# kalj/dealii-cuda

Hardware: AMD Instinct MI355X
Metric: DoFs/s on 1305x Laplace vmult (bmop), p=4 3D uniform (higher is better)
Workload: dtype f64; 1 GPU; bmop: DEGREE_FE=4, DIMENSION=3, MATRIX_FREE_UNIFORM_MESH, hyper_cube(-1,1), 54^3 cells, 10218313 DoFs, 1 z-slab(s); cells_per_dir=54, n_dofs=10218313, n_cells=157464, parallelism=slab1, dof_numbering=caller's (lexicographic), finite=True, clock_ramp_steps=2000

## Files before the change

dealii-cuda_amd/csrc/mfgpu_api.hip:

```cpp
#include <hip/hip_runtime.h>

#include <type_traits>

#include <algorithm>
#include <cmath>
#include <cstdlib>
#include <cstring>
#include <memory>
#include <string>
#include <vector>

#include "mfgpu_kernels.h"

using namespace mfgpu;

struct EventTimer {
  std::vector<Event> ev;
  size_t used = 0;
  double ms = 0.0;
  int begin(hipStream_t st) {
    if (used + 2 > ev.size()) {
      Event e0, e1;
      int rc;
      if ((rc = e0.create(hipEventDefault)) || (rc = e1.create(hipEventDefault))) return rc;
      ev.push_back(std::move(e0));
      ev.push_back(std::move(e1));
    }
    HIP_TRY(hipEventRecord(ev[used].get(), st));
    return 0;
  }
  int end(hipStream_t st) {
    HIP_TRY(hipEventRecord(ev[used + 1].get(), st));
    used += 2;
    return 0;
  }
  int drain(double *total) {
    for (size_t i = 0; i + 1 < used; i += 2) {
      float t = 0.f;
      HIP_TRY(hipEventElapsedTime(&t, ev[i].get(), ev[i + 1].get()));
      ms += t;
    }
    used = 0;
    *total = ms;
    return 0;
  }
  void reset() {
    used = 0;
    ms = 0.0;
  }
};

struct mfgpu_handle {
  Plan plan;
  int dim = 0, n = 0, nd = 0, number_type = MFGPU_F64;
  bool hn = false;
  std::vector<double> S, Dt;
  std::vector<double> sv, sg;
  DeviceArray<uint32_t> d_batch_cell_off, d_batch_dof_off, d_bdofs;
  DeviceArray<uint8_t> d_bflags;
  DeviceArray<uint16_t> d_lmap;
  DeviceArray<uint16_t> d_lmapx;
  DeviceArray<uint16_t> d_perm;
  DeviceArray<uint32_t> d_bdofsp, d_idxp;
  DeviceArray<uint32_t> d_shtab;
  bool shared_records = false;
  size_t record_bytes = 0;
  DeviceArray<uint32_t> d_hnrec;
  DeviceArray<uint32_t> d_hn_slot;
  DeviceArray<void> d_coefp;
  DeviceArray<void> d_coef;
  DeviceArray<void> d_mass, d_massp;
  DeviceArray<uint32_t> d_cmask, d_orphans;
  DeviceArray<void> d_hnw;
  DeviceArray<uint32_t> d_constrained;
  uint32_t n_constrained = 0;
  DeviceArray<void> d_tabsd;
  DeviceArray<void> d_tab2;
  bool twopass = true;
  DeviceArray<uint32_t> d_batch_nint, d_halo_off;
  std::vector<uint32_t> seg_end;
  std::vector<DeviceArray<uint32_t>> d_p2arr, d_p2tiles;
  std::vector<uint32_t> n_p2tiles;
  DeviceArray<uint32_t> d_p2rec, d_p2tab;
  bool p2_shared = false, p2_reverse = false, no_shared_records = false;
  Stream side;
  std::vector<Event> ev_seg;
  Event ev_side;
  bool side_pending = false;
  DeviceArray<void> d_halo;
  DeviceArray<unsigned long long> d_stamps;
  size_t lds = 0, device_bytes = 0;
  PlaneKernel planes = PlaneKernel::none;
  BatchKernel batches = BatchKernel::none;
  enum { kPlain, kMasked, kBatch };
  CellKernel<double> kernels_f64[3];
  CellKernel<float> kernels_f32[3];
  template <typename T>
  CellKernel<T> &kernel(int which) {
    if constexpr (std::is_same<T, double>::value) return kernels_f64[which];
    else return kernels_f32[which];
  }
  uint32_t n_cus = 0, max_workgroups = 0;
  bool prof = false;
  EventTimer t_cells;
  EventTimer t_pass2;
  uint64_t prof_vmults = 0;
};

namespace {

template <typename T>
hipError_t bind_kernel(const mfgpu_handle *h, PlaneKernel pk, BatchKernel bk, bool hn, bool sh, CellKernel<T> *k) {
  const Plan &P = h->plan;
  const auto bind = pk == PlaneKernel::planes3 ? p_bind<T> : pk == PlaneKernel::planes4 ? q_bind<T>
                    : bk == BatchKernel::batches ? apply_bind<T> : bk == BatchKernel::x ? x_bind<T>
                    : bk == BatchKernel::g ? g_bind<T> : bk == BatchKernel::g2 ? g2_bind<T> : nullptr;
  if (!bind) return hipErrorInvalidValue;
  return bind(P.dim, P.n, hn, h->twopass, sh, h->d_mass.get() != nullptr, P.max_batch_dofs, k);
}

template <typename T>
int launch_bound(mfgpu_handle *h, int which, const ApplyArgs<T> &a, uint32_t nbat, hipStream_t st) {
  const CellKernel<T> &k = h->kernel<T>(which);
  if (!k.launch[0]) {
    set_error("cell-loop kernel not bound");
    return MFGPU_EINVAL;
  }
  uint32_t grid = (uint32_t)(k.per_cu < 1 ? 1 : k.per_cu) * h->n_cus;
  if (h->max_workgroups && h->max_workgroups < grid) grid = h->max_workgroups;
  HIP_TRY(k.launch[a.add != 0](a, h->S.data(), h->Dt.data(), k.lds, nbat < grid ? nbat : grid, st));
  return 0;
}

int check_symmetrize(int n, std::vector<double> &S, std::vector<double> &Dt) {
  const int p = n - 1;
  double err = 0, mag = 0;
  for (int r = 0; r < n; ++r)
    for (int c = 0; c < n; ++c) {
      const double s1 = S[r * n + c], s2 = S[(p - r) * n + (p - c)];
      const double d1 = Dt[r * n + c], d2 = -Dt[(p - r) * n + (p - c)];
      err = std::fmax(err, std::fmax(std::fabs(s1 - s2), std::fabs(d1 - d2)));
      mag = std::fmax(mag, std::fmax(std::fabs(s1), std::fabs(d1)));
    }
  if (err > 1e-10 * mag) {
    set_error("shape tables are not symmetric about the cell midpoint (unsupported)");
    return MFGPU_EUNSUPPORTED;
  }
  for (int r = 0; r < n; ++r)
    for (int c = 0; c < n; ++c) {
      const int r2 = p - r, c2 = p - c;
      if (r * n + c < r2 * n + c2) {
        const double s = 0.5 * (S[r * n + c] + S[r2 * n + c2]);
        S[r * n + c] = S[r2 * n + c2] = s;
        const double d = 0.5 * (Dt[r * n + c] - Dt[r2 * n + c2]);
        Dt[r * n + c] = d;
        Dt[r2 * n + c2] = -d;
      } else if (r == r2 && c == c2) {
        Dt[r * n + c] = 0.0;
      }
    }
  return 0;
}

int upload_pass2(mfgpu_handle *h, const uint32_t *priority, uint32_t n_priority) {
  const Plan &P = h->plan;
  std::vector<uint8_t> prio(P.n_dofs, 0);
  for (uint32_t i = 0; i < n_priority; ++i) {
    if (priority[i] >= P.n_dofs) {
      set_error("priority dof out of range");
      return MFGPU_EINVAL;
    }
    prio[priority[i]] = 1;
  }
  const size_t ng = 1 + h->seg_end.size();
  const bool shared = P.sh_p2_use && !h->no_shared_records && n_priority == 0 && ng == 2;
  std::vector<std::vector<uint32_t>> sd(ng), so(ng, std::vector<uint32_t>(1, 0u)), si(ng);
  auto add = [&](uint32_t dof, const uint32_t *slots, uint32_t k, size_t seg) {
    const size_t g = prio[dof & 0x7fffffffu] ? 0 : 1 + seg;
    sd[g].push_back(dof);
    si[g].insert(si[g].end(), slots, slots + k);
    so[g].push_back((uint32_t)si[g].size());
  };
  for (size_t i = 0; i < P.sdofs.size(); ++i) {
    size_t seg = 0;
    if (shared && P.s_off[i + 1] > P.s_off[i]) continue;
    if (P.s_off[i + 1] > P.s_off[i]) {
      const uint32_t slot = P.s_idx[P.s_off[i + 1] - 1];
      const uint32_t batch = (uint32_t)(std::upper_bound(P.halo_off.begin(), P.halo_off.end(), slot) - P.halo_off.begin()) - 1;
      seg = (size_t)(std::upper_bound(h->seg_end.begin(), h->seg_end.end(), batch) - h->seg_end.begin());
      if (seg >= h->seg_end.size()) seg = h->seg_end.size() - 1;
    }
    add(P.sdofs[i], P.s_idx.data() + P.s_off[i], P.s_off[i + 1] - P.s_off[i], seg);
  }
  const uint32_t zero_slot = P.halo_off.empty() ? 0u : P.halo_off.back();
  for (uint32_t orph : P.orphans) add(orph, &zero_slot, 1, 0);
  std::vector<DeviceArray<uint32_t>> d_arr(ng), d_tiles(ng);
  std::vector<uint32_t> n_tiles(ng, 0u);
  const bool reverse = (size_t)P.halo_off.back() * esize(h->number_type) <= ((size_t)256 << 20);
  DeviceArray<uint32_t> d_rec, d_tab;
  if (shared) {
    int rc;
    if ((rc = d_rec.upload(P.sh_p2rec.data(), P.sh_p2rec.size()))) return rc;
    if ((rc = d_tab.upload(P.sh_p2tab.data(), P.sh_p2tab.size()))) return rc;
  }
  for (size_t g = 0; g < ng; ++g) {
    std::vector<uint32_t> arr, tiles;
    build_pass2_classes(sd[g], so[g], si[g], arr, tiles);
    n_tiles[g] = (uint32_t)(tiles.size() / 4);
    if (reverse) {
      const size_t nt = tiles.size() / 4;
      for (size_t a = 0, b = nt ? nt - 1 : 0; a < b; ++a, --b)
        for (int w = 0; w < 4; ++w) std::swap(tiles[4 * a + w], tiles[4 * b + w]);
    }
    int rc;
    if ((rc = d_arr[g].upload(arr.data(), arr.size()))) return rc;
    if ((rc = d_tiles[g].upload(tiles.data(), tiles.size()))) return rc;
  }
  h->d_p2arr = std::move(d_arr);
  h->d_p2tiles = std::move(d_tiles);
  h->n_p2tiles = std::move(n_tiles);
  h->d_p2rec = std::move(d_rec);
  h->d_p2tab = std::move(d_tab);
  h->p2_shared = shared;
  h->p2_reverse = reverse;
  return 0;
}

template <typename T>
int create_arrays(mfgpu_handle *h, const mfgpu_desc &d) {
  const Plan &P = h->plan;
  const size_t ncell = P.n_cells, nd = (size_t)P.nd;
  size_t &acct = h->device_bytes;
  auto up = [&](auto &arr, const void *src, size_t n) {
    const int rc = arr.upload(src, n);
    acct += arr.bytes();
    return rc;
  };
  int rc;
  if ((rc = up(h->d_batch_cell_off, P.batch_cell_off.data(), P.batch_cell_off.size()))) return rc;
  if ((rc = up(h->d_batch_dof_off, P.batch_dof_off.data(), P.batch_dof_off.size()))) return rc;
  if ((rc = up(h->d_bdofs, P.bdofs.data(), P.bdofs.size()))) return rc;
  if ((rc = up(h->d_bflags, P.bflags.data(), P.bflags.size()))) return rc;
  if ((rc = up(h->d_lmap, P.lmap.data(), P.lmap.size()))) return rc;
  const bool general = h->batches == BatchKernel::g || h->batches == BatchKernel::g2;
  if (h->batches == BatchKernel::x && !h->hn) {
    const int n = P.n, n2 = n * n, PP = n2, CH = 256 / PP, ndl = n2 * n;
    std::vector<uint16_t> perm(512, 0xffff);
    for (int layout = 0; layout < 2; ++layout) {
      uint16_t *lanes = perm.data() + 256 * layout;
      std::vector<int> fill(32, 0), overflow;
      for (int q = 0; q < CH * PP; ++q) {
        const int cell = q / PP, pen = q % PP, a = pen % n, b = pen / n;
        const int base = cell * ndl + (layout == 0 ? a + n2 * b : a + n * b);
        const int r = base & 31;
        if (fill[r] < 8) lanes[32 * fill[r]++ + r] = (uint16_t)q;
        else overflow.push_back(q);
      }
      for (int l = 255; l >= 0 && !overflow.empty(); --l)
        if (lanes[l] == 0xffff) {
          lanes[l] = (uint16_t)overflow.back();
          overflow.pop_back();
        }
    }
    if ((rc = up(h->d_perm, perm.data(), perm.size()))) return rc;
  }
  if (h->batches == BatchKernel::x || general) {
    const size_t n = (size_t)P.n, np = (n + 1) & ~(size_t)1, runs = P.lmap.size() / n;
    std::vector<uint16_t> lx(runs * np, 0);
    for (size_t r = 0; r < runs; ++r)
      for (size_t i = 0; i < n; ++i) lx[r * np + i] = P.lmap[r * n + i];
    if ((rc = up(h->d_lmapx, lx.data(), lx.size()))) return rc;
  }
  if (h->batches == BatchKernel::g2) {
    std::vector<T> sd(2 * (size_t)P.n * P.n);
    for (int i = 0; i < P.n * P.n; ++i) {
      sd[i] = (T)h->S[i];
      sd[P.n * P.n + i] = (T)h->Dt[i];
    }
    if ((rc = up(h->d_tabsd, sd.data(), sd.size() * sizeof(T)))) return rc;
  }
  if (h->planes != PlaneKernel::none) {
    if ((rc = build_plane_records(h->plan, d.constraint_mask))) return rc;
    if (!P.pr_hn.empty()) {
      if ((rc = up(h->d_hnrec, P.pr_hn.data(), P.pr_hn.size()))) return rc;
      if ((rc = up(h->d_hn_slot, P.pr_hn_slot.data(), P.pr_hn_slot.size()))) return rc;
    }
    h->shared_records = P.sh_use && !(d.flags & MFGPU_NO_SHARED_RECORDS) &&
                        kernel_exists(h->planes, P.n, d.number_type, false, true, d.mass_coefficient != nullptr);
    const std::vector<uint32_t> &rd = h->shared_records ? P.sh_dofs : P.pr_dofs;
    const std::vector<uint32_t> &rx = h->shared_records ? P.sh_idx : P.pr_idx;
    if ((rc = up(h->d_bdofsp, rd.data(), rd.size()))) return rc;
    if ((rc = up(h->d_idxp, rx.data(), rx.size()))) return rc;
    if (h->shared_records && (rc = up(h->d_shtab, P.sh_batch.data(), P.sh_batch.size()))) return rc;
    h->record_bytes = h->d_bdofsp.bytes() + h->d_idxp.bytes() + h->d_shtab.bytes();
  }
  if ((rc = up(h->d_orphans, P.orphans.data(), P.orphans.size()))) return rc;
  if (h->twopass) {
    if ((rc = up(h->d_batch_nint, P.batch_nint.data(), P.batch_nint.size()))) return rc;
    if ((rc = up(h->d_halo_off, P.halo_off.data(), P.halo_off.size()))) return rc;
    if (h->planes != PlaneKernel::none && (uint64_t)P.halo_off.back() >= (1ull << 29)) {
      set_error("halo buffer too large for 32-bit byte offsets");
      return MFGPU_EUNSUPPORTED;
    }
    const size_t hb = ((size_t)P.halo_off.back() + 1) * sizeof(T);
    if ((rc = h->d_halo.alloc(hb, true))) return rc;
    acct += hb;
  }
  if (h->hn) {
    std::vector<uint32_t> cm(ncell);
    for (size_t i = 0; i < ncell; ++i) cm[i] = d.constraint_mask[P.cell_order[i]];
    if ((rc = up(h->d_cmask, cm.data(), ncell))) return rc;
    std::vector<T> w((size_t)h->n * h->n);
    for (size_t i = 0; i < w.size(); ++i) w[i] = (T)d.constraint_weights[i];
    if ((rc = up(h->d_hnw, w.data(), w.size() * sizeof(T)))) return rc;
  }
  DeviceArray<T> metric;
  if ((rc = fold_coefficient<T>(metric, d.coefficient, d.quadrature_points, d.JxW, d.inv_jac, P.cell_order.data(), P.dim,
                                (uint32_t)ncell, (uint32_t)nd, general)))
    return rc;
  h->d_coef = std::move(metric);
  acct += h->d_coef.bytes();
  if (d.mass_coefficient) {
    DeviceArray<T> mass;
    if ((rc = fold_mass<T>(mass, d.mass_coefficient, d.JxW, P.cell_order.data(), (uint32_t)ncell, (uint32_t)nd))) return rc;
    h->d_mass = std::move(mass);
    acct += h->d_mass.bytes();
  }
  if (h->planes != PlaneKernel::none) {
    const int n = P.n, NT = p_cells_per_wave(n) * n;
    const size_t nbat = P.n_plane_batches, total = nbat * (size_t)(n * n) * NT;
    const size_t ncell_p = P.batch_cell_off[nbat];
    std::vector<uint32_t> cb(ncell_p), cp(ncell_p);
    for (size_t b = 0; b < nbat; ++b)
      for (uint32_t c = P.batch_cell_off[b]; c < P.batch_cell_off[b + 1]; ++c) {
        cb[c] = (uint32_t)b;
        cp[c] = c - P.batch_cell_off[b];
      }
    DeviceArray<uint32_t> t_cb, t_cp;
    if ((rc = t_cb.upload(cb.data(), ncell_p))) return rc;
    if ((rc = t_cp.upload(cp.data(), ncell_p))) return rc;
    if ((rc = h->d_coefp.alloc(total * sizeof(T), true))) return rc;
    acct += h->d_coefp.bytes();
    HIP_TRY(relayout_coef_launch<T>(h->d_coefp.as<T>(), h->d_coef.as<const T>(), t_cb.get(), t_cp.get(), ncell_p * nd, n,
                                    nullptr));
    if (d.mass_coefficient) {
      if ((rc = h->d_massp.alloc(total * sizeof(T), true))) return rc;
      acct += h->d_massp.bytes();
      HIP_TRY(relayout_coef_launch<T>(h->d_massp.as<T>(), h->d_mass.as<const T>(), t_cb.get(), t_cp.get(), ncell_p * nd,
                                      n, nullptr));
    }
    HIP_TRY(hipDeviceSynchronize());
  }
  int dev = 0;
  hipDeviceProp_t prop;
  HIP_TRY(hipGetDevice(&dev));
  HIP_TRY(hipGetDeviceProperties(&prop, dev));
  h->n_cus = (uint32_t)prop.multiProcessorCount;
  h->max_workgroups = d.max_workgroups;
  if (h->planes != PlaneKernel::none) {
    CellKernel<T> &plain = h->kernel<T>(mfgpu_handle::kPlain), &masked = h->kernel<T>(mfgpu_handle::kMasked);
    HIP_TRY(bind_kernel<T>(h, h->planes, BatchKernel::none, false, h->shared_records, &plain));
    h->lds = plain.lds;
    if (P.n_plain_plane_batches < P.n_plane_batches) {
      HIP_TRY(bind_kernel<T>(h, h->planes, BatchKernel::none, true, false, &masked));
      h->lds = std::max(h->lds, masked.lds);
    }
  }
  if (h->batches == BatchKernel::none) return 0;
  CellKernel<T> &batch = h->kernel<T>(mfgpu_handle::kBatch);
  const hipError_t bind_batch_family = bind_kernel<T>(h, PlaneKernel::none, h->batches, h->hn, false, &batch);
  h->lds = batch.lds;
  if (h->lds > 160 * 1024) {
    set_error("batch needs more than 160 KiB of LDS; lower max_dofs_per_batch");
    return MFGPU_EINVAL;
  }
  HIP_TRY(bind_batch_family);
  return 0;
}

void choose_segments(mfgpu_handle *h, uint32_t request) {
  const Plan &P = h->plan;
  const uint32_t nb = (uint32_t)(P.batch_cell_off.size() - 1);
  h->seg_end.assign(1, nb);
  if (!h->twopass || nb < 2 || request == 1) return;
  const uint32_t npl = P.n_plane_batches, nplain = P.n_plain_plane_batches;
  std::vector<uint32_t> cuts;
  if (npl > 0 && npl < nb) cuts.push_back(npl);
  if (nplain > 0 && nplain < npl) cuts.push_back(nplain);
  if (request > 1) {
    for (uint32_t i = 1; i < request; ++i) cuts.push_back((uint32_t)((uint64_t)nb * i / request));
  }
  if (request == 0 && !P.pr_hn.empty() && nplain == 0 && P.n == 5) cuts.push_back(nb / 2);
  std::sort(cuts.begin(), cuts.end());
  h->seg_end.clear();
  for (uint32_t c : cuts)
    if (c > 0 && c < nb && (h->seg_end.empty() || h->seg_end.back() != c)) h->seg_end.push_back(c);
  h->seg_end.push_back(nb);
}

template <typename T>
int create_typed(mfgpu_handle *h, const mfgpu_desc &d) {
  int rc = create_arrays<T>(h, d);
  if (rc) return rc;
  choose_segments(h, d.cell_loop_segments);
  if (!h->twopass) return 0;
  if (h->seg_end.size() > 1) {
    int prio_least = 0, prio_greatest = 0;
    HIP_TRY(hipDeviceGetStreamPriorityRange(&prio_least, &prio_greatest));
    if ((rc = h->side.create(hipStreamNonBlocking, prio_least))) return rc;
    if ((rc = h->ev_side.create(hipEventDisableTiming))) return rc;
    h->ev_seg.resize(h->seg_end.size() - 1);
    for (Event &e : h->ev_seg)
      if ((rc = e.create(hipEventDisableTiming))) return rc;
  }
  return upload_pass2(h, nullptr, 0);
}

template <typename T>
int launch_pass2_group(mfgpu_handle *h, size_t group, void *dst, const void *src, hipStream_t st, int add) {
  if (h->p2_shared && group == 1)
    HIP_TRY(reduce_owner_batches_launch<T>((T *)dst, (const T *)src, h->d_halo.as<const T>(), h->d_p2rec.get(),
                                           h->d_p2tab.get(), (uint32_t)(h->plan.batch_cell_off.size() - 1),
                                           (uint32_t)p_hs(h->plan.n) * 64u, h->p2_reverse ? 1 : 0, add, st));
  HIP_TRY(reduce_classes_launch<T>((T *)dst, (const T *)src, h->d_halo.as<const T>(), h->d_p2arr[group].get(),
                                   h->d_p2tiles[group].get(), h->n_p2tiles[group], add, st));
  return 0;
}

template <typename T>
int vmult_pass2(mfgpu_handle *h, int phase, void *dst, const void *src, hipStream_t st, int add) {
  if (!h->twopass) return 0;
  if (phase == 0) return launch_pass2_group<T>(h, 0, dst, src, st, add);
  int rc = launch_pass2_group<T>(h, h->seg_end.size(), dst, src, st, add);
  if (!rc && h->side_pending) {
    HIP_TRY(hipStreamWaitEvent(st, h->ev_side.get(), 0));
    h->side_pending = false;
  }
  return rc;
}

template <typename T>
int launch_cells(mfgpu_handle *h, ApplyArgs<T> a, uint32_t b0, uint32_t b1, hipStream_t st) {
  const Plan &P = h->plan;
  const uint32_t npl = P.n_plane_batches, nplain = P.n_plain_plane_batches;
  if (b0 < nplain) {
    a.batch0 = b0;
    a.batch_end = b1 < nplain ? b1 : nplain;
    if (const int rc = launch_bound<T>(h, mfgpu_handle::kPlain, a, a.batch_end - a.batch0, st)) return rc;
    b0 = a.batch_end;
  }
  if (b0 < npl && b0 < b1) {
    a.batch0 = b0;
    a.batch_end = b1 < npl ? b1 : npl;
    if (const int rc = launch_bound<T>(h, mfgpu_handle::kMasked, a, a.batch_end - a.batch0, st)) return rc;
    b0 = a.batch_end;
  }
  if (b0 >= b1) return 0;
  a.batch0 = b0;
  a.batch_end = b1;
  return launch_bound<T>(h, mfgpu_handle::kBatch, a, b1 - b0, st);
}

template <typename T>
ApplyArgs<T> make_args(mfgpu_handle *h, void *dst, const void *src, int add) {
  const Plan &P = h->plan;
  ApplyArgs<T> a;
  a.batch_cell_off = h->d_batch_cell_off.get();
  a.batch_dof_off = h->d_batch_dof_off.get();
  a.bdofs = h->d_bdofs.get();
  a.bflags = h->d_bflags.get();
  a.lmap = h->d_lmap.get();
  a.lmapx = h->d_lmapx.get();
  a.perm = h->d_perm.get();
  a.bdofsp = h->d_bdofsp.get();
  a.idxp = h->d_idxp.get();
  a.shtab = h->shared_records ? h->d_shtab.get() : nullptr;
  a.hnrec = h->d_hnrec.get();
  a.hn_slot = h->d_hn_slot.get();
  a.coefp = h->d_coefp.as<const T>();
  a.coef = h->d_coef.as<const T>();
  a.mass = h->d_mass.as<const T>();
  a.massp = h->d_massp.as<const T>();
  a.cmask = h->d_cmask.get();
  a.hn_weights = h->d_hnw.as<const T>();
  a.tabS = h->d_tabsd.as<const T>();
  a.tabDt = a.tabS ? a.tabS + (size_t)P.n * P.n : nullptr;
  a.batch_nint = h->d_batch_nint.get();
  a.halo_off = h->d_halo_off.get();
  a.halo = h->d_halo.as<T>();
  a.dst = (T *)dst;
  a.src = (const T *)src;
  a.nb_max = P.max_batch_dofs;
  a.add = add;
  a.stamps = h->d_stamps.get();
  a.dbg = 0;
  return a;
}

template <typename T>
int vmult_main(mfgpu_handle *h, void *dst, const void *src, hipStream_t st, int add) {
  const Plan &P = h->plan;
  ApplyArgs<T> a = make_args<T>(h, dst, src, add);
  int rc;
  if (h->prof && (rc = h->t_cells.begin(st))) return rc;
  if (h->twopass) {
    const size_t nseg = h->seg_end.size();
    if (h->side_pending) {
      HIP_TRY(hipStreamWaitEvent(st, h->ev_side.get(), 0));
      h->side_pending = false;
    }
    for (size_t s = 0; s < nseg; ++s) {
      if ((rc = launch_cells<T>(h, a, s ? h->seg_end[s - 1] : 0u, h->seg_end[s], st))) return rc;
      if (s + 1 < nseg) {
        HIP_TRY(hipEventRecord(h->ev_seg[s].get(), st));
        HIP_TRY(hipStreamWaitEvent(h->side.get(), h->ev_seg[s].get(), 0));
        if ((rc = launch_pass2_group<T>(h, 1 + s, dst, src, h->side.get(), add))) return rc;
      }
    }
    if (nseg > 1) {
      HIP_TRY(hipEventRecord(h->ev_side.get(), h->side.get()));
      h->side_pending = true;
    }
  } else {
    for (size_t c = 0; c + 1 < P.color_batch_off.size(); ++c) {
      if (P.color_batch_off[c + 1] == P.color_batch_off[c]) continue;
      if ((rc = launch_cells<T>(h, a, P.color_batch_off[c], P.color_batch_off[c + 1], st))) return rc;
    }
  }
  if (h->prof && (rc = h->t_cells.end(st))) return rc;
  if (!h->twopass)
    HIP_TRY(orphan_launch<T>((T *)dst, (const T *)src, h->d_orphans.get(), (uint32_t)P.orphans.size(), add, st));
  if (h->prof) h->prof_vmults++;
  return 0;
}

template <typename T>
int vmult_typed(mfgpu_handle *h, void *dst, const void *src, hipStream_t st, int add) {
  int rc = vmult_main<T>(h, dst, src, st, add);
  if (rc) return rc;
  const bool timed = h->prof && h->twopass;
  if (timed && (rc = h->t_pass2.begin(st))) return rc;
  rc = vmult_pass2<T>(h, 0, dst, src, st, add);
  if (!rc) rc = vmult_pass2<T>(h, 1, dst, src, st, add);
  if (!rc && timed) rc = h->t_pass2.end(st);
  return rc;
}

}

namespace {
template <typename T>
int inverse_diagonal_typed(mfgpu_handle *h, void *diag, hipStream_t st) {
  const Plan &P = h->plan;
  const bool general = h->batches == BatchKernel::g || h->batches == BatchKernel::g2;
  if (!h->d_tab2.get()) {
    const int nn = h->n * h->n;
    std::vector<T> t2(2 * (size_t)nn);
    for (int i = 0; i < nn; ++i) {
      t2[i] = (T)(general ? h->sv[i] : h->sv[i] * h->sv[i]);
      t2[nn + i] = (T)(general ? h->sg[i] : h->sg[i] * h->sg[i]);
    }
    if (const int rc = h->d_tab2.upload(t2.data(), t2.size() * sizeof(T))) return rc;
    h->device_bytes += h->d_tab2.bytes();
  }
  HIP_TRY(fill_launch<T>((T *)diag, P.n_dofs, T(0), st));
  const uint32_t nb = (uint32_t)(P.batch_cell_off.size() - 1), *cell_off = h->d_batch_cell_off.get();
  const uint32_t *dof_off = h->d_batch_dof_off.get(), *bdofs = h->d_bdofs.get(), *cmask = h->d_cmask.get();
  const uint16_t *lmap = h->d_lmap.get();
  const T *coef = h->d_coef.as<const T>(), *hnw = h->d_hnw.as<const T>(), *tab2 = h->d_tab2.as<const T>();
  if (h->batches == BatchKernel::g2)
    HIP_TRY(diag_general2_launch<T>(P.n, (T *)diag, nb, cell_off, dof_off, bdofs, lmap, coef, cmask, hnw, tab2, st));
  else if (h->batches == BatchKernel::g)
    HIP_TRY(diag_general_launch<T>(P.n, (T *)diag, nb, cell_off, dof_off, bdofs, lmap, coef, cmask, hnw, tab2, st));
  else
    HIP_TRY(diag_launch<T>(P.dim, P.n, (T *)diag, nb, cell_off, dof_off, bdofs, lmap, coef, cmask, hnw, tab2, st));
  if (h->d_mass.get())
    HIP_TRY(diag_mass_launch<T>(P.dim, P.n, (T *)diag, nb, cell_off, dof_off, bdofs, lmap, h->d_mass.as<const T>(), cmask,
                                hnw, tab2, !general, st));
  HIP_TRY(set_values_launch<T>((T *)diag, h->d_constrained.get(), h->n_constrained, T(1), st));
  HIP_TRY(vec_map_launch<T>(4, (T *)diag, nullptr, T(0), T(0), P.n_dofs, st));
  return 0;
}
}


namespace {
int vec_map(int op, void *v, const void *w, double s, double a, size_t n, int nt, void *stream) {
  if ((!v && n) || (!w && n && op <= 3)) {
    set_error("null vector");
    return MFGPU_EINVAL;
  }
  if (nt == MFGPU_F32)
    HIP_TRY(vec_map_launch<float>(op, (float *)v, (const float *)w, (float)s, (float)a, n, (hipStream_t)stream));
  else if (nt == MFGPU_F64)
    HIP_TRY(vec_map_launch<double>(op, (double *)v, (const double *)w, s, a, n, (hipStream_t)stream));
  else
    return MFGPU_EINVAL;
  return 0;
}
int vec_reduce(int op, void *v, const void *x, const void *w, double a, size_t n, int nt, void *stream, double *out) {
  if (!out || (n && (!v || (op != 2 && !w) || (op == 1 && !x)))) {
    set_error("null argument");
    return MFGPU_EINVAL;
  }
  if (nt == MFGPU_F32)
    HIP_TRY(vec_reduce_launch<float>(op, (float *)v, (const float *)x, (const float *)w, (float)a, n, (hipStream_t)stream, out));
  else if (nt == MFGPU_F64)
    HIP_TRY(vec_reduce_launch<double>(op, (double *)v, (const double *)x, (const double *)w, a, n, (hipStream_t)stream, out));
  else
    return MFGPU_EINVAL;
  return 0;
}
}


namespace mfgpu {
int handle_number_type(const mfgpu_handle *h) { return h->number_type; }
int handle_set_priority_dofs(mfgpu_handle *h, const uint32_t *ids, uint32_t n) {
  return h->twopass ? upload_pass2(h, ids, n) : 0;
}
int handle_n_batches(const mfgpu_handle *h) { return (int)h->plan.batch_cell_off.size() - 1; }
bool handle_ranged_ok(const mfgpu_handle *h) { return h->twopass && h->seg_end.size() == 1; }
int handle_batches_touching(const mfgpu_handle *h, const uint32_t *ids, uint32_t n, std::vector<uint8_t> &flags) {
  const Plan &P = h->plan;
  std::vector<uint8_t> mark(P.n_dofs, 0);
  for (uint32_t i = 0; i < n; ++i) {
    if (ids[i] >= P.n_dofs) {
      set_error("interface dof out of range");
      return MFGPU_EINVAL;
    }
    mark[ids[i]] = 1;
  }
  const size_t nb = P.batch_cell_off.size() - 1;
  flags.assign(nb, 0);
  for (size_t b = 0; b < nb; ++b)
    for (uint32_t t = P.batch_dof_off[b]; t < P.batch_dof_off[b + 1]; ++t)
      if (mark[P.bdofs[t] & 0x7fffffffu]) {
        flags[b] = 1;
        break;
      }
  return 0;
}
int handle_cells_range(mfgpu_handle *h, uint32_t b0, uint32_t b1, void *dst, const void *src, void *stream, int add) {
  if (b0 >= b1) return 0;
  hipStream_t st = (hipStream_t)stream;
  if (h->number_type == MFGPU_F64) return launch_cells<double>(h, make_args<double>(h, dst, src, add), b0, b1, st);
  return launch_cells<float>(h, make_args<float>(h, dst, src, add), b0, b1, st);
}
int handle_cells_two_ranges(mfgpu_handle *h, uint32_t b0, uint32_t b1, uint32_t c0, uint32_t c1, void *dst,
                            const void *src, void *stream, int add) {
  const uint32_t nplain = h->plan.n_plain_plane_batches, npl = h->plan.n_plane_batches;
  const bool plain = c1 <= nplain, masked = b0 >= nplain && c1 <= npl;
  if (b0 >= b1 || c0 >= c1 || b1 > c0 || !(plain || masked)) {
    const int rc = handle_cells_range(h, b0, b1, dst, src, stream, add);
    return rc ? rc : handle_cells_range(h, c0, c1, dst, src, stream, add);
  }
  hipStream_t st = (hipStream_t)stream;
  auto run = [&](auto a) -> int {
    a.batch0 = b0;
    a.batch_end = c1;
    a.hole0 = b1;
    a.hole_len = c0 - b1;
    using T = typename std::remove_const<typename std::remove_pointer<decltype(a.src)>::type>::type;
    return launch_bound<T>(h, plain ? mfgpu_handle::kPlain : mfgpu_handle::kMasked, a, (b1 - b0) + (c1 - c0), st);
  };
  return h->number_type == MFGPU_F64 ? run(make_args<double>(h, dst, src, add)) : run(make_args<float>(h, dst, src, add));
}
int handle_pass2_group(mfgpu_handle *h, int group, void *dst, const void *src, void *stream, int add) {
  if (!h->twopass) return 0;
  hipStream_t st = (hipStream_t)stream;
  return h->number_type == MFGPU_F64 ? launch_pass2_group<double>(h, (size_t)group, dst, src, st, add)
                                     : launch_pass2_group<float>(h, (size_t)group, dst, src, st, add);
}
int handle_vmult_phase(mfgpu_handle *h, int phase, void *dst, const void *src, void *stream, int add) {
  hipStream_t st = (hipStream_t)stream;
  if (h->number_type == MFGPU_F64)
    return phase == 0 ? vmult_main<double>(h, dst, src, st, add) : vmult_pass2<double>(h, phase - 1, dst, src, st, add);
  return phase == 0 ? vmult_main<float>(h, dst, src, st, add) : vmult_pass2<float>(h, phase - 1, dst, src, st, add);
}
}

extern "C" {

int mfgpu_create(const mfgpu_desc *desc, mfgpu_handle **out) {
  if (!desc || !out) {
    set_error("null argument");
    return MFGPU_EINVAL;
  }
  const mfgpu_desc &d = *desc;
  if (!valid_number_type(d.number_type)) {
    set_error("number_type must be MFGPU_F64 or MFGPU_F32");
    return MFGPU_EINVAL;
  }
  const bool general = !(d.flags & MFGPU_UNIFORM_J0);
  if (general && (d.flags & MFGPU_COLORED_SCATTER)) {
    set_error("the general-Jacobian path (no MFGPU_UNIFORM_J0) is implemented in two-pass scatter mode only");
    return MFGPU_EUNSUPPORTED;
  }
  if (!d.JxW || !d.inv_jac || !d.shape_values || !d.shape_gradients ||
      (!d.coefficient && !d.quadrature_points)) {
    set_error("JxW, inv_jac, shape tables and coefficient (or quadrature_points) are required");
    return MFGPU_EINVAL;
  }
  const bool hn = (d.flags & MFGPU_HANGING_NODES) != 0;
  if (hn && (!d.constraint_mask || !d.constraint_weights)) {
    set_error("MFGPU_HANGING_NODES needs constraint_mask and constraint_weights");
    return MFGPU_EINVAL;
  }
  std::unique_ptr<mfgpu_handle, decltype(&mfgpu_destroy)> h(new mfgpu_handle(), mfgpu_destroy);
  int rc = choose_kernel_and_plan(d, h->planes, h->batches, h->plan);
  if (rc) return rc;
  h->dim = d.dim;
  h->n = d.degree + 1;
  h->nd = h->plan.nd;
  h->number_type = d.number_type;
  h->hn = hn;
  h->twopass = !(d.flags & MFGPU_COLORED_SCATTER);
  h->no_shared_records = (d.flags & MFGPU_NO_SHARED_RECORDS) != 0;
  const int nn = h->n * h->n;
  std::vector<double> sv(nn), sg(nn);
  for (int i = 0; i < nn; ++i) {
    sv[i] = d.number_type == MFGPU_F64 ? ((const double *)d.shape_values)[i] : ((const float *)d.shape_values)[i];
    sg[i] = d.number_type == MFGPU_F64 ? ((const double *)d.shape_gradients)[i] : ((const float *)d.shape_gradients)[i];
  }
  h->sv = sv;
  h->sg = sg;
  rc = derive_tables(h->n, sv.data(), sg.data(), h->S, h->Dt);
  if (!rc) rc = check_symmetrize(h->n, h->S, h->Dt);
  if (!rc) rc = d.number_type == MFGPU_F64 ? create_typed<double>(h.get(), d) : create_typed<float>(h.get(), d);
  if (!rc && d.n_constrained) {
    h->n_constrained = d.n_constrained;
    rc = h->d_constrained.upload(d.constrained_dofs, d.n_constrained);
    h->device_bytes += h->d_constrained.bytes();
  }
  if (rc) return rc;
  *out = h.release();
  return 0;
}

void mfgpu_destroy(mfgpu_handle *h) {
  if (!h) return;
  if (h->side.get()) hipStreamSynchronize(h->side.get());
  delete h;
}

int mfgpu_vmult(mfgpu_handle *h, void *dst, const void *src, void *stream) {
  if (!h || !dst || !src) {
    set_error("null argument");
    return MFGPU_EINVAL;
  }
  if (dst == src) {
    set_error("vmult: dst and src must not alias");
    return MFGPU_EINVAL;
  }
  return h->number_type == MFGPU_F64 ? vmult_typed<double>(h, dst, src, (hipStream_t)stream, 0)
                                     : vmult_typed<float>(h, dst, src, (hipStream_t)stream, 0);
}

int mfgpu_vmult_add(mfgpu_handle *h, void *dst, const void *src, void *stream) {
  if (!h || !dst || !src) {
    set_error("null argument");
    return MFGPU_EINVAL;
  }
  if (dst == src) {
    set_error("vmult_add: dst and src must not alias");
    return MFGPU_EINVAL;
  }
  return h->number_type == MFGPU_F64 ? vmult_typed<double>(h, dst, src, (hipStream_t)stream, 1)
                                     : vmult_typed<float>(h, dst, src, (hipStream_t)stream, 1);
}

uint32_t mfgpu_n_dofs(const mfgpu_handle *h) { return h ? h->plan.n_dofs : 0; }

size_t mfgpu_memory_consumption(const mfgpu_handle *h) { return h ? h->device_bytes : 0; }

int mfgpu_plan_stats(const mfgpu_handle *h, uint64_t s[8]) {
  if (!h || !s) return MFGPU_EINVAL;
  const Plan &P = h->plan;
  s[0] = P.batch_cell_off.size() - 1;
  s[1] = P.color_batch_off.size() - 1;
  s[2] = P.bdofs.size();
  s[3] = P.max_batch_dofs;
  s[4] = P.max_batch_cells;
  s[5] = P.orphans.size();
  s[6] = P.n_first;
  s[7] = P.n_add;
  if (h->twopass) {
    const uint32_t nb = (uint32_t)s[0], npl = P.n_plane_batches, nplain = P.n_plain_plane_batches;
    const uint32_t edge[4] = {0u, nplain, npl, nb};
    s[1] = 0;
    for (size_t g = 0; g < h->seg_end.size(); ++g) {
      const uint32_t s0 = g ? h->seg_end[g - 1] : 0u, s1 = h->seg_end[g];
      for (int f = 0; f < 3; ++f)
        if (std::max(s0, edge[f]) < std::min(s1, edge[f + 1])) ++s[1];
    }
    s[6] = P.sdofs.size();
    s[7] = P.halo_off.back();
  }
  return 0;
}

int mfgpu_record_stats(const mfgpu_handle *h, uint64_t s[4]) {
  if (!h || !s) return MFGPU_EINVAL;
  const Plan &P = h->plan;
  const size_t n = (size_t)P.n, nb = (size_t)p_kgu((int)n) * 64, nx = ((n * n + 1) / 2) * (p_cells_per_wave((int)n) * n);
  const bool planes = h->planes != PlaneKernel::none;
  s[0] = (h->shared_records ? 1 : 0) | (h->p2_shared ? 2 : 0);
  s[1] = planes ? P.sh_dofs.size() / nb : 0;
  s[2] = planes ? P.sh_idx.size() / nx : 0;
  s[3] = h->record_bytes;
  return 0;
}

const char *mfgpu_kernel_name(const mfgpu_handle *h) {
  if (!h) return "";
  const bool x = h->batches == BatchKernel::x;
  switch (h->planes) {
    case PlaneKernel::planes3: return x ? "apply_planes3+apply_batches_x" : "apply_planes3";
    case PlaneKernel::planes4: return x ? "apply_planes4+apply_batches_x" : "apply_planes4";
    default: break;
  }
  switch (h->batches) {
    case BatchKernel::x: return "apply_batches_x";
    case BatchKernel::g: return "apply_batches_g";
    case BatchKernel::g2: return "apply_batches_g2";
    default: return "apply_batches";
  }
}

int mfgpu_profile_enable(mfgpu_handle *h, int on) {
  if (!h) return MFGPU_EINVAL;
  h->prof = on != 0;
  h->t_cells.reset();
  h->t_pass2.reset();
  h->prof_vmults = 0;
  return 0;
}

int mfgpu_profile_read_pass2(mfgpu_handle *h, double *ms) {
  if (!h || !ms) return MFGPU_EINVAL;
  HIP_TRY(hipDeviceSynchronize());
  return h->t_pass2.drain(ms);
}

int mfgpu_profile_read(mfgpu_handle *h, double *ms, uint64_t *nv) {
  if (!h || !ms || !nv) return MFGPU_EINVAL;
  HIP_TRY(hipDeviceSynchronize());
  if (const int rc = h->t_cells.drain(ms)) return rc;
  *nv = h->prof_vmults;
  return 0;
}

#ifdef MFGPU_STAMPS
int mfgpu_debug_stamps(mfgpu_handle *h, unsigned long long *out, size_t n_batches) {
  if (!h) return MFGPU_EINVAL;
  const size_t nbt = h->plan.batch_cell_off.size() - 1;
  if (!h->d_stamps.get()) return h->d_stamps.alloc(2 * nbt * 16, true);
  if (out && n_batches == nbt) {
    HIP_TRY(hipDeviceSynchronize());
    HIP_TRY(hipMemcpy(out, h->d_stamps.get(), 2 * nbt * 16 * sizeof(unsigned long long), hipMemcpyDeviceToHost));
  }
  return 0;
}
#endif


int mfgpu_compute_inverse_diagonal(mfgpu_handle *h, void *inv_diag, void *stream) {
  if (!h || !inv_diag) {
    set_error("null argument");
    return MFGPU_EINVAL;
  }
  return h->number_type == MFGPU_F64 ? inverse_diagonal_typed<double>(h, inv_diag, (hipStream_t)stream)
                                     : inverse_diagonal_typed<float>(h, inv_diag, (hipStream_t)stream);
}

int mfgpu_set_constrained_values(mfgpu_handle *h, void *vec, double value, void *stream) {
  if (!h || !vec) {
    set_error("null argument");
    return MFGPU_EINVAL;
  }
  if (h->number_type == MFGPU_F64)
    HIP_TRY(set_values_launch<double>((double *)vec, h->d_constrained.get(), h->n_constrained, value, (hipStream_t)stream));
  else
    HIP_TRY(set_values_launch<float>((float *)vec, h->d_constrained.get(), h->n_constrained, (float)value,
                                     (hipStream_t)stream));
  return 0;
}

int mfgpu_vec_sadd(void *v, double s, double a, const void *w, size_t n, int nt, void *stream) {
  return vec_map(0, v, w, s, a, n, nt, stream);
}
int mfgpu_vec_equ(void *v, double a, const void *w, size_t n, int nt, void *stream) {
  return vec_map(1, v, w, 0.0, a, n, nt, stream);
}
int mfgpu_vec_scale(void *v, const void *w, size_t n, int nt, void *stream) {
  return vec_map(2, v, w, 0.0, 0.0, n, nt, stream);
}
int mfgpu_vec_divide(void *v, const void *w, size_t n, int nt, void *stream) {
  return vec_map(3, v, w, 0.0, 0.0, n, nt, stream);
}
int mfgpu_vec_invert(void *v, size_t n, int nt, void *stream) { return vec_map(4, v, nullptr, 0.0, 0.0, n, nt, stream); }
int mfgpu_vec_mul(void *v, double a, size_t n, int nt, void *stream) {
  return vec_map(5, v, nullptr, 0.0, a, n, nt, stream);
}
int mfgpu_vec_dot(const void *v, const void *w, size_t n, int nt, void *stream, double *result) {
  return vec_reduce(0, const_cast<void *>(v), nullptr, w, 0.0, n, nt, stream, result);
}
int mfgpu_vec_l2_norm(const void *v, size_t n, int nt, void *stream, double *result) {
  int rc = vec_reduce(0, const_cast<void *>(v), nullptr, v, 0.0, n, nt, stream, result);
  if (!rc) *result = std::sqrt(*result);
  return rc;
}
int mfgpu_vec_add_and_dot(void *v, double a, const void *x, const void *w, size_t n, int nt, void *stream,
                          double *result) {
  return vec_reduce(1, v, x, w, a, n, nt, stream, result);
}
int mfgpu_vec_all_zero(const void *v, size_t n, int nt, void *stream, int *result) {
  if (!result) return MFGPU_EINVAL;
  double cnt = 0.0;
  int rc = vec_reduce(2, const_cast<void *>(v), nullptr, nullptr, 0.0, n, nt, stream, &cnt);
  if (!rc) *result = cnt == 0.0;
  return rc;
}

int mfgpu_vec_alloc(void **dev, size_t n, int nt) {
  if (!dev) return MFGPU_EINVAL;
  *dev = nullptr;
  if (n == 0) return 0;
  HIP_TRY(hipMalloc(dev, n * esize(nt)));
  HIP_TRY(hipMemset(*dev, 0, n * esize(nt)));
  return 0;
}
int mfgpu_vec_free(void *dev) {
  if (dev) HIP_TRY(hipFree(dev));
  return 0;
}
int mfgpu_vec_fill(void *dev, size_t n, int nt, double value, void *stream) {
  if (!dev && n) return MFGPU_EINVAL;
  if (nt == MFGPU_F32)
    HIP_TRY(fill_launch<float>((float *)dev, n, (float)value, (hipStream_t)stream));
  else
    HIP_TRY(fill_launch<double>((double *)dev, n, value, (hipStream_t)stream));
  return 0;
}
int mfgpu_vec_from_host(void *dev, const void *host, size_t n, int nt) {
  if (n) HIP_TRY(hipMemcpy(dev, host, n * esize(nt), hipMemcpyHostToDevice));
  return 0;
}
int mfgpu_vec_to_host(void *host, const void *dev, size_t n, int nt) {
  if (n) HIP_TRY(hipMemcpy(host, dev, n * esize(nt), hipMemcpyDeviceToHost));
  return 0;
}
int mfgpu_device_synchronize(void) {
  HIP_TRY(hipDeviceSynchronize());
  return 0;
}
int mfgpu_device_memory_info(size_t *free_bytes, size_t *total_bytes) {
  if (!free_bytes || !total_bytes) return MFGPU_EINVAL;
  HIP_TRY(hipMemGetInfo(free_bytes, total_bytes));
  return 0;
}

}
```

dealii-cuda_amd/csrc/mfgpu_internal.h:

```cpp
#ifndef MFGPU_INTERNAL_H
#define MFGPU_INTERNAL_H

#include <cstdint>
#include <string>
#include <vector>

#include "../../include/mfgpu.h"

namespace mfgpu {

void set_error(const std::string &msg);

inline int ipow(int a, int e) {
  int r = 1;
  for (int i = 0; i < e; ++i) r *= a;
  return r;
}

constexpr int p_cells_per_wave(int n) { return 64 / n; }
constexpr int p_ji(int n) { return n == 3 ? 2 : n == 4 ? 5 : n == 5 ? 9 : n == 6 ? 14 : 23; }
constexpr int p_hs(int n) { return n == 3 ? 3 : n == 4 ? 6 : n == 5 ? 9 : n == 6 ? 14 : 18; }
constexpr int p_kgu(int n) { return p_ji(n) + p_hs(n); }
constexpr int p_cell_stride(int n) {
  int s = n * n * n;
  while ((s & 31) != (n & 31)) ++s;
  return s;
}

constexpr int q_plane_stride(int n) { return n >= 6 ? 65 : n == 5 ? 33 : n == 4 ? 17 : 33; }
constexpr int q_cell_stride(int n) { return n * q_plane_stride(n); }
constexpr int p_priv_max(int n) { return n >= 5 ? 384 : n == 4 ? 256 : 192; }
constexpr int kHnOpRounds = 2;
constexpr int p_hn_rows(int n) { return p_priv_max(n) / 64 + 3 * kHnOpRounds * 3 + 2; }

template <typename T>
constexpr size_t q_region_doubles(int n) {
  const size_t t = ((size_t)(p_cells_per_wave(n) + 1) * q_cell_stride(n) * sizeof(T) + 7) / 8;
  const size_t u = (size_t)p_kgu(n) * 64 + p_priv_max(n);
  return t > u ? t : u;
}
template <typename T>
constexpr size_t q_lds_bytes(int n, bool hn) {
  return (q_region_doubles<T>(n) + (hn ? (size_t)n * n : 0)) * 8;
}

constexpr uint8_t kFlagConstrained = 1;
constexpr uint8_t kFlagAdd = 2;

struct Plan {
  int dim = 0, degree = 0, n = 0, nd = 0;
  uint32_t n_dofs = 0, n_cells = 0;
  std::vector<uint32_t> cell_order;
  std::vector<uint32_t> batch_cell_off;
  std::vector<uint32_t> batch_dof_off;
  std::vector<uint32_t> color_batch_off;
  std::vector<uint32_t> bdofs;
  std::vector<uint8_t> bflags;
  std::vector<uint16_t> lmap;
  std::vector<uint32_t> orphans;
  std::vector<uint32_t> batch_nint;
  std::vector<uint32_t> halo_off;
  std::vector<uint32_t> sdofs;
  std::vector<uint32_t> s_off;
  std::vector<uint32_t> s_idx;
  std::vector<uint32_t> chunks;
  std::vector<uint32_t> gstarts;
  uint32_t max_batch_dofs = 0, max_batch_cells = 0;
  uint32_t n_plane_batches = 0;
  uint32_t n_plain_plane_batches = 0;
  std::vector<uint32_t> pr_dofs, pr_idx, pr_hn, pr_hn_slot;
  std::vector<uint32_t> sh_dofs, sh_idx, sh_batch;
  bool sh_use = false;
  std::vector<uint32_t> sh_p2rec, sh_p2tab;
  bool sh_p2_use = false;
  uint64_t n_first = 0, n_add = 0;
};

struct PlanLimits {
  uint32_t max_cells = 0, max_dofs = 0;
  uint32_t interior_max = 0, shared_max = 0, halo_stride = 0;
  bool segregate_masked = false;
  bool masked_planes = false;
  uint32_t private_max = 0;
};

int build_plan(const mfgpu_desc &d, Plan &plan, uint32_t max_chunks = 3, const PlanLimits *limits = nullptr);

struct HnLine {
  uint16_t node[8];
};
void hn_cell_lines(unsigned mask, int n, std::vector<HnLine> (&lines)[3], std::vector<uint16_t> &nodes);

enum class PlaneKernel : uint8_t { none, planes3, planes4 };
enum class BatchKernel : uint8_t { none, batches, x, g, g2 };
int choose_kernel_and_plan(const mfgpu_desc &d, PlaneKernel &pk, BatchKernel &bk, Plan &plan);

constexpr bool planes4_wide(int n) { return n >= 6; }
constexpr bool kernel_exists(PlaneKernel k, int n, int number_type, bool hn, bool sh, bool mass) {
  switch (k) {
    case PlaneKernel::planes3: return n >= 3 && n <= 5 && !(sh && hn);
    case PlaneKernel::planes4:
      return planes4_wide(n) ? n <= 7 && !hn && !sh && !mass
                             : n >= 3 && !sh && !(mass && n == 5 && number_type == MFGPU_F64);
    default: return false;
  }
}
constexpr bool kernel_exists(BatchKernel k, int n, int , bool , bool sh, bool ) {
  return k != BatchKernel::none && n >= 2 && n <= 7 && !sh;
}
int build_plane_records(Plan &plan, const uint32_t *constraint_mask);
constexpr int kShBatchWords = 4;
constexpr double kShareMaxFraction = 0.5;
void share_plane_records(Plan &plan);
constexpr int kP2Header = 16, kP2MaxK = 12, kP2SlotBits = 12;
void share_pass2_records(Plan &plan);

int derive_tables(int n, const double *shape_values, const double *shape_gradients,
                  std::vector<double> &S, std::vector<double> &Dt);

int handle_number_type(const mfgpu_handle *h);
int handle_set_priority_dofs(mfgpu_handle *h, const uint32_t *ids, uint32_t n);
int handle_vmult_phase(mfgpu_handle *h, int phase, void *dst, const void *src, void *stream, int add);
int handle_n_batches(const mfgpu_handle *h);
bool handle_ranged_ok(const mfgpu_handle *h);
int handle_batches_touching(const mfgpu_handle *h, const uint32_t *ids, uint32_t n, std::vector<uint8_t> &flags);
int handle_cells_range(mfgpu_handle *h, uint32_t b0, uint32_t b1, void *dst, const void *src, void *stream, int add);
int handle_cells_two_ranges(mfgpu_handle *h, uint32_t b0, uint32_t b1, uint32_t c0, uint32_t c1, void *dst,
                            const void *src, void *stream, int add);
int handle_pass2_group(mfgpu_handle *h, int group, void *dst, const void *src, void *stream, int add);

}

struct mfgpu_plan {
  mfgpu::Plan plan;
};

#endif
```

dealii-cuda_amd/csrc/mfgpu_kernels.h:

```cpp
#ifndef MFGPU_KERNELS_H
#define MFGPU_KERNELS_H

#include <hip/hip_runtime.h>

#include <type_traits>

#include "mfgpu_device.h"
#include "mfgpu_internal.h"

namespace mfgpu {

template <typename T>
struct ApplyArgs {
  const uint32_t *batch_cell_off;
  const uint32_t *batch_dof_off;
  const uint32_t *bdofs;
  const uint8_t *bflags;
  const uint16_t *lmap;
  const uint16_t *lmapx;
  const uint16_t *perm;
  const uint32_t *bdofsp;
  const uint32_t *idxp;
  const T *coefp;
  const uint32_t *hnrec;
  const uint32_t *hn_slot;
  const T *coef;
  const uint32_t *cmask;
  const T *hn_weights;
  const T *tabS, *tabDt;
  const uint32_t *batch_nint;
  const uint32_t *halo_off;
  T *halo;
  T *dst;
  const T *src;
  uint32_t batch0;
  uint32_t batch_end;
  uint32_t hole0 = 0xffffffffu, hole_len = 0;
  uint32_t nb_max;
  int add;
  unsigned long long *stamps;
  int dbg;
  const uint32_t *shtab = nullptr;
  const T *mass = nullptr;
  const T *massp = nullptr;
};

template <typename T, int n>
struct Tables {
  T S[((n + 1) / 2) * n];
  T Dt[((n + 1) / 2) * n];
};

template <typename T, int n>
inline Tables<T, n> make_tables(const double *S, const double *Dt) {
  Tables<T, n> tab;
  for (int i = 0; i < ((n + 1) / 2) * n; ++i) {
    tab.S[i] = (T)S[i];
    tab.Dt[i] = (T)Dt[i];
  }
  return tab;
}

template <typename T>
struct CellKernel {
  size_t lds = 0;
  int per_cu = 0;
  hipError_t (*launch[2])(const ApplyArgs<T> &a, const double *S, const double *Dt, size_t lds, uint32_t grid,
                          hipStream_t st) = {nullptr, nullptr};
};

template <typename T, int Block, auto K, auto MakeTab>
hipError_t launch_cell_kernel(const ApplyArgs<T> &a, const double *S, const double *Dt, size_t lds, uint32_t grid,
                              hipStream_t st) {
  if constexpr (std::is_null_pointer_v<decltype(MakeTab)>)
    hipLaunchKernelGGL(K, dim3(grid), dim3(Block), lds, st, a);
  else
    hipLaunchKernelGGL(K, dim3(grid), dim3(Block), lds, st, a, MakeTab(S, Dt));
  return hipGetLastError();
}

template <typename T, int Block, auto K0, auto K1, auto MakeTab>
hipError_t bind_cell_kernel(size_t lds, CellKernel<T> *k) {
  k->lds = lds;
  for (const void *f : {(const void *)K1, (const void *)K0})
    if (const hipError_t e = hipFuncSetAttribute(f, hipFuncAttributeMaxDynamicSharedMemorySize, (int)lds)) return e;
  k->launch[0] = launch_cell_kernel<T, Block, K0, MakeTab>;
  k->launch[1] = launch_cell_kernel<T, Block, K1, MakeTab>;
  return hipOccupancyMaxActiveBlocksPerMultiprocessor(&k->per_cu, (const void *)K0, Block, lds);
}

template <typename F>
hipError_t dispatch_flags(F &&f) { return f(); }
template <typename F, typename... B>
hipError_t dispatch_flags(F &&f, bool flag, B... rest) {
  return dispatch_flags(
      [&](auto... c) { return flag ? f(std::true_type{}, c...) : f(std::false_type{}, c...); }, rest...);
}
template <typename F, typename... B>
hipError_t dispatch_instantiation(int n, F &&f, B... flags) {
  auto at = [&](auto N) { return dispatch_flags([&](auto... c) { return f(N, c...); }, flags...); };
  switch (n) {
    case 2: return at(std::integral_constant<int, 2>{});
    case 3: return at(std::integral_constant<int, 3>{});
    case 4: return at(std::integral_constant<int, 4>{});
    case 5: return at(std::integral_constant<int, 5>{});
    case 6: return at(std::integral_constant<int, 6>{});
    case 7: return at(std::integral_constant<int, 7>{});
    default: return hipErrorInvalidValue;
  }
}
template <typename T>
constexpr int number_type_of = sizeof(T) == 8 ? MFGPU_F64 : MFGPU_F32;

#define MFGPU_CELL_LOOP_FAMILY(F)                                                                              \
  template <typename T>                                                                                        \
  hipError_t F##_bind(int dim, int n, bool hn, bool twopass, bool sh, bool mass, uint32_t nb_max, CellKernel<T> *k);
MFGPU_CELL_LOOP_FAMILY(apply)
MFGPU_CELL_LOOP_FAMILY(x)
MFGPU_CELL_LOOP_FAMILY(g)
MFGPU_CELL_LOOP_FAMILY(g2)
MFGPU_CELL_LOOP_FAMILY(p)
MFGPU_CELL_LOOP_FAMILY(q)
#undef MFGPU_CELL_LOOP_FAMILY

void build_pass2_classes(const std::vector<uint32_t> &sdofs, const std::vector<uint32_t> &s_off,
                         const std::vector<uint32_t> &s_idx, std::vector<uint32_t> &arr, std::vector<uint32_t> &tiles);
template <typename T>
hipError_t reduce_classes_launch(T *dst, const T *src, const T *halo, const uint32_t *arr, const uint32_t *tiles,
                                 uint32_t n_tiles, int add, hipStream_t st);
template <typename T>
hipError_t reduce_owner_batches_launch(T *dst, const T *src, const T *halo, const uint32_t *rec, const uint32_t *tab,
                                       uint32_t n_batches, uint32_t hstride, int reverse, int add, hipStream_t st);
template <typename T>
hipError_t relayout_coef_launch(T *out, const T *in, const uint32_t *cell_batch, const uint32_t *cell_pos,
                                size_t total, int n, hipStream_t st);
template <typename T>
hipError_t fold_general_launch(T *M, const T *coef, const T *jxw, const T *jinv, const uint32_t *order,
                               uint32_t n_cells, uint32_t nd, hipStream_t st);
template <typename T>
hipError_t fold_general2_launch(T *M, const T *coef, const T *jxw, const T *jinv, const uint32_t *order,
                                uint32_t n_cells, uint32_t nd, hipStream_t st);
template <typename T>
hipError_t orphan_launch(T *dst, const T *src, const uint32_t *orph, uint32_t n, int add, hipStream_t st);
template <typename T>
hipError_t coefficient_launch(T *coef, const T *qpts, size_t nq, int dim, hipStream_t st);
template <typename T>
hipError_t fold_launch(T *c, const T *coef, const T *jxw, const T *j0, const uint32_t *order,
                       uint32_t n_cells, uint32_t nd, hipStream_t st);
template <typename T>
hipError_t fill_launch(T *v, size_t n, T a, hipStream_t st);
template <typename T>
int fold_mass(DeviceArray<T> &out, const void *mass_coefficient, const void *JxW, const uint32_t *cell_order,
              uint32_t n_cells, uint32_t nd);
template <typename T>
int fold_coefficient(DeviceArray<T> &out, const void *coefficient, const void *quadrature_points, const void *JxW,
                     const void *inv_jac, const uint32_t *cell_order, int dim, uint32_t n_cells, uint32_t nd,
                     bool general);

template <typename T>
hipError_t diag_launch(int dim, int n, T *diag, uint32_t n_batches, const uint32_t *batch_cell_off,
                       const uint32_t *batch_dof_off, const uint32_t *bdofs, const uint16_t *lmap, const T *coef,
                       const uint32_t *cmask, const T *hn_weights, const T *tab2, hipStream_t st);
template <typename T>
hipError_t diag_general_launch(int n, T *diag, uint32_t n_batches, const uint32_t *batch_cell_off,
                               const uint32_t *batch_dof_off, const uint32_t *bdofs, const uint16_t *lmap,
                               const T *metric, const uint32_t *cmask, const T *hn_weights, const T *tab,
                               hipStream_t st);
template <typename T>
hipError_t diag_general2_launch(int n, T *diag, uint32_t n_batches, const uint32_t *batch_cell_off,
                                const uint32_t *batch_dof_off, const uint32_t *bdofs, const uint16_t *lmap,
                                const T *metric, const uint32_t *cmask, const T *hn_weights, const T *tab,
                                hipStream_t st);
template <typename T>
hipError_t diag_mass_launch(int dim, int n, T *diag, uint32_t n_batches, const uint32_t *batch_cell_off,
                            const uint32_t *batch_dof_off, const uint32_t *bdofs, const uint16_t *lmap, const T *mass,
                            const uint32_t *cmask, const T *hn_weights, const T *tab, bool squared, hipStream_t st);
template <typename T>
hipError_t set_values_launch(T *v, const uint32_t *idx, uint32_t n, T value, hipStream_t st);
template <typename T>
hipError_t vec_map_launch(int op, T *v, const T *w, T s, T a, size_t n, hipStream_t st);
template <typename T>
hipError_t vec_reduce_launch(int op, T *v, const T *x, const T *w, T a, size_t n, hipStream_t st, double *out);

}
#endif
```

dealii-cuda_amd/csrc/mfgpu_kernels_p.hip:

```cpp
#include <hip/hip_runtime.h>

#include "mfgpu_cell.h"
#include "mfgpu_kernels.h"
#include "mfgpu_planes.h"

namespace mfgpu {

#define MFGPU_PIN_VMEM() __builtin_amdgcn_sched_barrier(0x380)

template <int n, typename T, bool ADD, bool HN, bool SH = false, bool MASS = false>
__global__ void __launch_bounds__(64) __attribute__((amdgpu_waves_per_eu(1, 1)))
apply_planes3(const ApplyArgs<T> A, const TablesEO<T, n> tab) {
  constexpr int n2 = n * n;
  constexpr int CW = p_cells_per_wave(n);
  constexpr int NT = CW * n;
  constexpr int KGU = p_kgu(n);
  constexpr int JI = p_ji(n);
  constexpr int HS = KGU - JI;
  constexpr int SA = p_cell_stride(n);
  constexpr int NIW = (n2 + 1) / 2;
  extern __shared__ __attribute__((aligned(16))) unsigned char smem_raw[];
  constexpr int PRIV = HN ? p_priv_max(n) : 0;
  double *ua = reinterpret_cast<double *>(smem_raw);
  T *Aw = reinterpret_cast<T *>(ua + KGU * 64 + PRIV + (HN ? n2 : 0));
  T *Bw = Aw + (CW + 1) * SA;
  double *Wl = ua + KGU * 64 + PRIV;

  const int lane = threadIdx.x;
  if (HN) {
    if (lane < n2) Wl[lane] = (double)A.hn_weights[lane];
  }
  const int lc = lane / n, k = lane - lc * n;
  const bool lane_on = lane < NT;
  const int tk = lane_on ? lane : NT - 1;

  uint32_t b, bstride, bend;
  {
    const uint32_t nbt = A.batch_end - A.batch0 - A.hole_len, G = gridDim.x;
    if (G >= 8 && nbt >= G) {
      const uint32_t xcd = blockIdx.x & 7u, slot = blockIdx.x >> 3;
      const uint32_t q = G >> 3, rem = G & 7u;
      const uint32_t wlo = xcd * q + (xcd < rem ? xcd : rem);
      const uint32_t w = q + (xcd < rem ? 1u : 0u);
      b = A.batch0 + (uint32_t)((uint64_t)nbt * wlo / G) + slot;
      bend = A.batch0 + (uint32_t)((uint64_t)nbt * (wlo + w) / G);
      bstride = w;
    } else {
      b = A.batch0 + blockIdx.x;
      bend = A.batch_end - A.hole_len;
      bstride = G;
    }
  }
  if (b >= bend) return;
  const uint32_t hole0 = A.hole0, hole_len = A.hole_len;
  auto next_of = [&](uint32_t x) {
    const uint32_t l = (x >= hole0 ? x - hole_len : x) + bstride;
    return l < bend ? (l >= hole0 ? l + hole_len : l) : x;
  };
  if (b >= hole0) b += hole_len;
  static_assert(kernel_exists(PlaneKernel::planes3, n, number_type_of<T>, HN, SH, MASS), "no such instantiation");
  struct Meta {
    uint32_t base, drec, irec;
  };
  auto meta_request = [&](uint32_t bb) -> uint32_t {
    return A.shtab[(size_t)bb * kShBatchWords + (lane & (kShBatchWords - 1))];
  };
  auto meta_of = [&](uint32_t v) -> Meta {
    return Meta{(uint32_t)__builtin_amdgcn_readlane((int)v, 0), (uint32_t)__builtin_amdgcn_readlane((int)v, 1),
                (uint32_t)__builtin_amdgcn_readlane((int)v, 2)};
  };

  auto load_dofs = [&](uint32_t rec, uint32_t (&g)[KGU]) {
    const uint32_t *p = A.bdofsp + (size_t)rec * (KGU * 64) + lane;
#pragma unroll
    for (int j = 0; j < KGU; ++j) g[j] = SH ? p[j * 64] : nt_load(p + j * 64);
  };
  auto src_at = [&](uint32_t base, uint32_t g) -> T {
    const T *const sp = SH ? A.src + base : A.src;
    return *reinterpret_cast<const T *>(reinterpret_cast<const char *>(sp) + (uint32_t)(g * (uint32_t)sizeof(T)));
  };
  auto dst_at = [&](uint32_t base, uint32_t g) -> T * {
    T *const dp = SH ? A.dst + base : A.dst;
    return reinterpret_cast<T *>(reinterpret_cast<char *>(dp) + (uint32_t)(g * (uint32_t)sizeof(T)));
  };
  auto load_ix = [&](uint32_t rec, uint32_t (&ix)[NIW]) {
    const uint32_t *p = A.idxp + (size_t)rec * (NIW * NT) + tk;
#pragma unroll
    for (int w = 0; w < NIW; ++w) ix[w] = SH ? p[w * NT] : nt_load(p + w * NT);
  };
  auto stage_src = [&](const uint32_t (&g)[KGU], const T (&sv)[KGU]) {
#pragma unroll
    for (int j = 0; j < KGU; ++j) {
      double v = (double)sv[j];
      if (j >= JI) {
        const unsigned long long keep = (unsigned long long)(long long)~((int)g[j] >> 31);
        v = __longlong_as_double((long long)((unsigned long long)__double_as_longlong(v) & keep));
      }
      ua[lane + j * 64] = v;
    }
  };
  auto ixb = [&](const uint32_t (&ix)[NIW], int i) -> uint32_t {
    return (i & 1) ? (ix[i >> 1] >> 16) : (ix[i >> 1] & 0xffffu);
  };
  auto scatter_slot = [&](int j, uint32_t bb, uint32_t base, uint32_t g, T r, T oldv) {
    if (j < JI) {
      *dst_at(base, g) = ADD ? oldv + r : r;
    } else {
      T *const hp = A.halo + (size_t)bb * (HS * 64) + lane;
      hp[(j - JI) * 64] = r;
    }
  };

  uint32_t b1 = next_of(b), b2 = next_of(b1);
  uint32_t Gp[KGU], Gc[KGU], Gn[KGU], Gnn[KGU];
  uint32_t IXc[NIW], IXn[NIW];
  constexpr int CR = PRIV / 64, HROWS = HN ? p_hn_rows(n) : 1;
  uint32_t Hc[HROWS], Hn[HROWS];
  auto load_hn = [&](uint32_t bb, uint32_t (&H)[HROWS]) {
    const uint32_t slot = A.hn_slot[bb];
    if (slot != 0xffffffffu) {
      const uint32_t *p = A.hnrec + (size_t)slot * (HROWS * 64) + lane;
#pragma unroll
      for (int w = 0; w < HROWS; ++w) H[w] = nt_load(p + w * 64);
    } else {
#pragma unroll
      for (int w = 0; w < HROWS; ++w) H[w] = 0u;
    }
  };
  T Cc[n2];
  T Mm[MASS ? n2 : 1];
  T SVn[KGU], R[KGU], old[KGU];
  Meta Mp{0u, 0u, 0u}, Mc = Mp, M1 = Mp, M2 = Mp;
  uint32_t Mv = 0u;
  if (SH) {
    Mc = meta_of(meta_request(b));
    M1 = meta_of(meta_request(b1));
    M2 = meta_of(meta_request(b2));
    Mp = Mc;
  }
  load_dofs(SH ? Mc.drec : b, Gc);
  load_dofs(SH ? M1.drec : b1, Gn);
  load_ix(SH ? Mc.irec : b, IXc);
  if (HN) load_hn(b, Hc);
  constexpr uint32_t kDummyIx = 8u * (uint32_t)(KGU * 64 - 1) * 0x10001u;
#pragma unroll
  for (int w = 0; w < NIW; ++w) IXc[w] = lane_on ? IXc[w] : kDummyIx;
  {
    const T *p = A.coefp + (size_t)b * (n2 * NT) + tk;
#pragma unroll
    for (int r = 0; r < n2; ++r) Cc[r] = nt_load(p + r * NT);
  }
  if (MASS) {
    const T *p = A.massp + (size_t)b * (n2 * NT) + tk;
#pragma unroll
    for (int r = 0; r < n2; ++r) Mm[r] = nt_load(p + r * NT);
  }
#pragma unroll
  for (int j = 0; j < KGU; ++j) {
    SVn[j] = src_at(Mc.base, Gc[j]);
    Gp[j] = Gc[j];
    R[j] = T(0);
    old[j] = T(0);
  }
  stage_src(Gc, SVn);
  WaveSync::sync();

  const int pxy = lc * SA + n2 * k;
  const int pyz = lc * SA + k;
  uint32_t bp = b;

  while (true) {
    const bool has_next = b1 != b;
    constexpr int kH2 = HN ? HROWS - 2 : 0, kH1 = HN ? HROWS - 1 : 0;
    const uint32_t hn_ncopy = HN ? (uint32_t)__builtin_amdgcn_readfirstlane(Hc[kH2] & 0xffffu) : 0u;
    auto hn_count = [&](int dir) -> uint32_t {
      const uint32_t w = dir == 0 ? Hc[kH2] >> 16 : dir == 1 ? Hc[kH1] & 0xffffu : Hc[kH1] >> 16;
      return (uint32_t)__builtin_amdgcn_readfirstlane(w);
    };
    auto hn_pass = [&](int dir, bool transposed, const double (&Wr)[n2]) {
      const uint32_t count = hn_count(dir);
#pragma unroll
      for (int r = 0; r < kHnOpRounds; ++r) {
        if ((uint32_t)(r * 64) >= count) break;
        const bool on = (uint32_t)(r * 64 + lane) < count;
        const uint32_t *ww = &Hc[CR + (dir * kHnOpRounds + r) * 3];
        double v[n], o[n];
        uint32_t pos[n];
#pragma unroll
        for (int t = 0; t < n; ++t) {
          pos[t] = on ? (ww[t >> 1] >> (16 * (t & 1))) & 0xffffu : (uint32_t)(KGU * 64 + PRIV - 1);
          v[t] = ua[pos[t]];
        }
#pragma unroll
        for (int i = 0; i < n; ++i) {
          double acc = 0.0;
#pragma unroll
          for (int k2 = 0; k2 < n; ++k2) acc = fma(transposed ? Wr[k2 * n + i] : Wr[i * n + k2], v[k2], acc);
          o[i] = acc;
        }
        if (on) {
#pragma unroll
          for (int i = 0; i < n; ++i) ua[pos[i]] = o[i];
        }
      }
    };
    if (HN && hn_ncopy) {
      double Wr[n2];
#pragma unroll
      for (int i = 0; i < n2; ++i) Wr[i] = Wl[i];
      double cv[CR > 0 ? CR : 1];
#pragma unroll
      for (int r = 0; r < CR; ++r) cv[r] = (uint32_t)(r * 64 + lane) < hn_ncopy ? ua[Hc[r] & 0xffffu] : 0.0;
#pragma unroll
      for (int r = 0; r < CR; ++r)
        if ((uint32_t)(r * 64 + lane) < hn_ncopy) ua[Hc[r] >> 16] = cv[r];
      WaveSync::sync();
      hn_pass(0, false, Wr);
      WaveSync::sync();
      hn_pass(1, false, Wr);
      WaveSync::sync();
      hn_pass(2, false, Wr);
      WaveSync::sync();
    }
    STAMP(0);
    RSTAMP(8);
    WGSTAMP(10);
    load_dofs(SH ? M2.drec : b2, Gnn);
    load_ix(SH ? M1.irec : b1, IXn);
    if (SH) Mv = meta_request(next_of(b2));
    if (HN) load_hn(b1, Hn);
    if (ADD) {
#pragma unroll
      for (int j = 0; j < JI; ++j) old[j] = *dst_at(Mp.base, Gp[j]);
    }
    STAMP(1);
    auto hookA = [&](int) {};
    auto hookB = [&](int s) {
      MFGPU_PIN_VMEM();
#pragma unroll
      for (int j = (KGU * s) / (5 * n); j < (KGU * (s + 1)) / (5 * n); ++j)
        scatter_slot(j, bp, Mp.base, Gp[j], R[j], old[j]);
#pragma unroll
      for (int j = (KGU * s) / (5 * n); j < (KGU * (s + 1)) / (5 * n); ++j)
        SVn[j] = src_at(M1.base, Gn[j]);
      MFGPU_PIN_VMEM();
    };
    const T *const cnext = A.coefp + (size_t)b1 * (n2 * NT) + tk;
    const T *const mnext = MASS ? A.massp + (size_t)b1 * (n2 * NT) + tk : nullptr;
    auto hookC = [&](int s) {
      MFGPU_PIN_VMEM();
#pragma unroll
      for (int r = (n2 * s) / (2 * n); r < (n2 * (s + 1)) / (2 * n); ++r)
        Cc[r] = nt_load(cnext + r * NT);
      if (MASS) {
#pragma unroll
        for (int r = (n2 * s) / (2 * n); r < (n2 * (s + 1)) / (2 * n); ++r)
          Mm[r] = nt_load(mnext + r * NT);
      }
      MFGPU_PIN_VMEM();
    };

    {
      T u[n2];
#pragma unroll
      for (int x = 0; x < n; ++x)
#pragma unroll
        for (int y = 0; y < n; ++y)
          u[x + n * y] = (T) * reinterpret_cast<const double *>(reinterpret_cast<const char *>(ua) + ixb(IXc, x + n * y));
#pragma unroll
      for (int x = 0; x < n; ++x) {
        T in[n], out[n];
        get_line<n, 1>(u, x, in);
        eo_apply<n, 0>(tab, in, out);
        set_line<n, 1>(u, x, out);
        hookA(x);
      }
#pragma unroll
      for (int y = 0; y < n; ++y) {
        T in[n], a[n], bb[n];
        get_line<n, 0>(u, y, in);
        eo_apply<n, 0>(tab, in, a);
        eo_apply<n, 2>(tab, a, bb);
#pragma unroll
        for (int x = 0; x < n; ++x) {
          Aw[pxy + x + n * y] = a[x];
          Bw[pxy + x + n * y] = bb[x];
        }
        hookA(n + y);
      }
    }
    WaveSync::sync();
    STAMP(2);
#pragma unroll
    for (int j = 0; j < KGU + PRIV / 64; ++j) ua[lane + j * 64] = 0.0;

    {
      T nx[n];
#pragma unroll
      for (int z = 0; z < n; ++z) nx[z] = Bw[pyz + n2 * z];
#pragma unroll
      for (int y = 0; y < n; ++y) {
        T in[n], g[n], o[n];
#pragma unroll
        for (int z = 0; z < n; ++z) in[z] = nx[z];
#pragma unroll
        for (int z = 0; z < n; ++z) nx[z] = y + 1 < n ? Bw[pyz + n * (y + 1) + n2 * z] : Aw[pyz + n2 * z];
        eo_apply<n, 0>(tab, in, g);
#pragma unroll
        for (int z = 0; z < n; ++z) g[z] *= Cc[y + n * z];
        eo_apply<n, 1>(tab, g, o);
#pragma unroll
        for (int z = 0; z < n; ++z) Bw[pyz + n * y + n2 * z] = o[z];
        hookB(y);
      }
      T v[n2], r[n2];
#pragma unroll
      for (int y = 0; y < n; ++y) {
        T in[n], o[n];
#pragma unroll
        for (int z = 0; z < n; ++z) in[z] = nx[z];
        if (y + 1 < n) {
#pragma unroll
          for (int z = 0; z < n; ++z) nx[z] = Aw[pyz + n * (y + 1) + n2 * z];
        }
        eo_apply<n, 0>(tab, in, o);
        set_line<n, 1>(v, y, o);
        hookB(n + y);
      }
#pragma unroll
      for (int y = 0; y < n; ++y) {
        T in[n], g[n], o[n];
        get_line<n, 1>(v, y, in);
        eo_apply<n, 2>(tab, in, g);
#pragma unroll
        for (int z = 0; z < n; ++z) g[z] *= Cc[y + n * z];
        eo_apply<n, 3>(tab, g, o);
        set_line<n, 1>(r, y, o);
        hookB(2 * n + y);
      }
#pragma unroll
      for (int z = 0; z < n; ++z) {
        T in[n], g[n], o[n];
        get_line<n, 0>(v, z, in);
        eo_apply<n, 2>(tab, in, g);
#pragma unroll
        for (int y = 0; y < n; ++y) g[y] *= Cc[y + n * z];
        eo_apply<n, 3>(tab, g, o);
#pragma unroll
        for (int y = 0; y < n; ++y) r[y + n * z] += MASS ? fma(Mm[y + n * z], in[y], o[y]) : o[y];
        hookB(3 * n + z);
      }
#pragma unroll
      for (int y = 0; y < n; ++y) {
        T in[n], o[n];
        get_line<n, 1>(r, y, in);
        eo_apply<n, 1>(tab, in, o);
#pragma unroll
        for (int z = 0; z < n; ++z) Aw[pyz + n * y + n2 * z] = o[z];
        hookB(4 * n + y);
      }
    }
    WaveSync::sync();
    STAMP(3);

    {
      T o[n2];
      T nr[n], nt[n];
#pragma unroll
      for (int x = 0; x < n; ++x) {
        nr[x] = Aw[pxy + x];
        nt[x] = Bw[pxy + x];
      }
#pragma unroll
      for (int y = 0; y < n; ++y) {
        T rp[n], tp[n], w[n], ol[n];
#pragma unroll
        for (int x = 0; x < n; ++x) {
          rp[x] = nr[x];
          tp[x] = nt[x];
        }
        if (y + 1 < n) {
#pragma unroll
          for (int x = 0; x < n; ++x) {
            nr[x] = Aw[pxy + x + n * (y + 1)];
            nt[x] = Bw[pxy + x + n * (y + 1)];
          }
        }
        eo_apply<n, 3>(tab, tp, w);
#pragma unroll
        for (int x = 0; x < n; ++x) w[x] += rp[x];
        eo_apply<n, 1>(tab, w, ol);
        set_line<n, 0>(o, y, ol);
        hookC(y);
      }
#pragma unroll
      for (int x = 0; x < n; ++x) {
        T in[n], out[n];
        get_line<n, 1>(o, x, in);
        eo_apply<n, 1>(tab, in, out);
#pragma unroll
        for (int y = 0; y < n; ++y)
          lds_add(reinterpret_cast<double *>(reinterpret_cast<char *>(ua) + ixb(IXc, x + n * y)), (double)out[y]);
        hookC(n + x);
      }
    }
    WaveSync::sync();
    STAMP(4);

    if (HN && hn_ncopy) {
      double Wr[n2];
#pragma unroll
      for (int i = 0; i < n2; ++i) Wr[i] = Wl[i];
      hn_pass(2, true, Wr);
      WaveSync::sync();
      hn_pass(1, true, Wr);
      WaveSync::sync();
      hn_pass(0, true, Wr);
      WaveSync::sync();
      double cv[CR > 0 ? CR : 1];
#pragma unroll
      for (int r = 0; r < CR; ++r) cv[r] = (uint32_t)(r * 64 + lane) < hn_ncopy ? ua[Hc[r] >> 16] : 0.0;
#pragma unroll
      for (int r = 0; r < CR; ++r)
        if ((uint32_t)(r * 64 + lane) < hn_ncopy) lds_add(ua + (Hc[r] & 0xffffu), cv[r]);
      WaveSync::sync();
    }
#pragma unroll
    for (int j = 0; j < KGU; ++j) R[j] = (T)ua[lane + j * 64];
    WaveSync::sync();
    STAMP(5);
    stage_src(Gn, SVn);
    STAMP(6);
    bp = b;
    if (SH) Mp = Mc;
#pragma unroll
    for (int j = 0; j < KGU; ++j) Gp[j] = Gc[j];
    STAMP(7);
    RSTAMP(9);
    if (!has_next) break;
    WaveSync::sync();
    b = b1;
    b1 = b2;
    b2 = next_of(b2);
    if (SH) {
      Mc = M1;
      M1 = M2;
      M2 = meta_of(Mv);
    }
#pragma unroll
    for (int j = 0; j < KGU; ++j) {
      Gc[j] = Gn[j];
      Gn[j] = Gnn[j];
    }
#pragma unroll
    for (int w = 0; w < NIW; ++w) IXc[w] = lane_on ? IXn[w] : kDummyIx;
    if (HN) {
#pragma unroll
      for (int w = 0; w < HROWS; ++w) Hc[w] = Hn[w];
    }
  }
  if (ADD) {
#pragma unroll
    for (int j = 0; j < JI; ++j) old[j] = *dst_at(Mp.base, Gp[j]);
  }
#pragma unroll
  for (int j = 0; j < KGU; ++j) scatter_slot(j, bp, Mp.base, Gp[j], R[j], old[j]);
}

template <int n, typename T>
static size_t p_lds_bytes(bool hn) {
  return ((size_t)p_kgu(n) * 64 + (hn ? (size_t)p_priv_max(n) + n * n : 0)) * sizeof(double) +
         (size_t)2 * (p_cells_per_wave(n) + 1) * p_cell_stride(n) * sizeof(T);
}

template <typename T>
hipError_t p_bind(int, int n, bool hn, bool, bool sh, bool mass, uint32_t, CellKernel<T> *k) {
  return dispatch_instantiation(n, [&](auto N, auto HN, auto SH, auto MASS) {
    constexpr int n_ = N;
    if constexpr (kernel_exists(PlaneKernel::planes3, n_, number_type_of<T>, HN, SH, MASS))
      return bind_cell_kernel<T, 64, apply_planes3<n_, T, false, HN, SH, MASS>, apply_planes3<n_, T, true, HN, SH, MASS>,
                              make_tables_eo<T, n_>>(p_lds_bytes<n_, T>(HN), k);
    else
      return hipErrorInvalidValue;
  }, hn, sh, mass);
}
template hipError_t p_bind<double>(int, int, bool, bool, bool, bool, uint32_t, CellKernel<double> *);
template hipError_t p_bind<float>(int, int, bool, bool, bool, bool, uint32_t, CellKernel<float> *);

template <typename T>
__global__ void relayout_coef_kernel(T *out, const T *in, const uint32_t *cell_batch, const uint32_t *cell_pos,
                                     size_t total, int n) {
  const size_t i = (size_t)blockIdx.x * blockDim.x + threadIdx.x;
  if (i >= total) return;
  const int n2 = n * n, nd = n2 * n, NT = (64 / n) * n;
  const size_t cell = i / nd;
  const int q = (int)(i - cell * nd);
  const int x = q % n, r = q / n;
  out[((size_t)cell_batch[cell] * n2 + r) * NT + cell_pos[cell] * n + x] = in[i];
}

template <typename T>
hipError_t relayout_coef_launch(T *out, const T *in, const uint32_t *cell_batch, const uint32_t *cell_pos,
                                size_t total, int n, hipStream_t st) {
  if (total == 0) return hipSuccess;
  hipLaunchKernelGGL(relayout_coef_kernel<T>, dim3((unsigned)((total + 255) / 256)), dim3(256), 0, st, out, in,
                     cell_batch, cell_pos, total, n);
  return hipGetLastError();
}
template hipError_t relayout_coef_launch<double>(double *, const double *, const uint32_t *, const uint32_t *, size_t,
                                                 int, hipStream_t);
template hipError_t relayout_coef_launch<float>(float *, const float *, const uint32_t *, const uint32_t *, size_t, int,
                                                hipStream_t);

}
```

dealii-cuda_amd/csrc/mfgpu_plan.cpp:

```cpp
#include <algorithm>
#include <cassert>
#include <cmath>
#include <cstring>
#include <numeric>
#include <unordered_map>

#include "mfgpu_internal.h"

namespace mfgpu {

static thread_local std::string g_err;
void set_error(const std::string &msg) { g_err = msg; }
const char *last_error() { return g_err.c_str(); }

int derive_tables(int n, const double *sv, const double *sg, std::vector<double> &S,
                  std::vector<double> &Dt) {
  std::vector<long double> A(n * n), B(n * n);
  for (int i = 0; i < n * n; ++i) {
    A[i] = sv[i];
    B[i] = sg[i];
  }
  for (int c = 0; c < n; ++c) {
    int piv = c;
    for (int r = c + 1; r < n; ++r)
// ... 419 lines not shown
      std::vector<uint32_t> second(batches[b].begin() + half, batches[b].end());
      batches[b].resize(half);
      batches.insert(batches.begin() + b + 1, std::move(second));
      batch_masked.insert(batch_masked.begin() + b + 1, batch_masked[b]);
    }
  }

  std::vector<uint64_t> dof_colors(N, 0);
  std::vector<uint32_t> bcolor(nb, 0);
  uint32_t ncolors = 0;
  for (uint32_t b = 0; b < nb; ++b) {
    uint64_t forbidden = 0;
    for (uint32_t g : bd[b]) forbidden |= dof_colors[g];
    uint32_t c = 0;
    while (c < 64 && (forbidden >> c) & 1) ++c;
    if (c >= 64) {
      set_error("more than 64 batch colours needed");
      return MFGPU_EUNSUPPORTED;
    }
    bcolor[b] = c;
    ncolors = std::max(ncolors, c + 1);
    for (uint32_t g : bd[b]) dof_colors[g] |= (1ull << c);
  }
  const bool colored = (d.flags & MFGPU_COLORED_SCATTER) != 0;
  std::vector<uint32_t> order(nb);
  std::iota(order.begin(), order.end(), 0u);
  if (colored) {
    std::stable_sort(order.begin(), order.end(),
                     [&](uint32_t a, uint32_t b2) { return bcolor[a] < bcolor[b2]; });
    P.color_batch_off.assign(ncolors + 1, 0);
    for (uint32_t b = 0; b < nb; ++b) P.color_batch_off[bcolor[b] + 1]++;
    for (uint32_t c = 0; c < ncolors; ++c) P.color_batch_off[c + 1] += P.color_batch_off[c];
  } else {
    P.color_batch_off.assign({0u, nb});
  }

  std::vector<uint32_t> rank_of(nb);
  for (uint32_t k = 0; k < nb; ++k) rank_of[order[k]] = k;
  std::vector<uint32_t> shared_ids;
  for (uint32_t g = 0; g < N; ++g)
    if (shared_flag[g]) shared_ids.push_back(g);
  const size_t ns = shared_ids.size();
  std::vector<uint32_t> sid(N, NONE), t_off(ns + 1, 0);
  for (size_t i = 0; i < ns; ++i) {
    sid[shared_ids[i]] = (uint32_t)i;
    t_off[i + 1] = t_off[i] + ntouch[shared_ids[i]];
  }
  std::vector<uint32_t> touchers(t_off[ns]);
  {
    std::vector<uint32_t> fill(t_off.begin(), t_off.end() - 1);
    for (uint32_t k = 0; k < nb; ++k)
      for (size_t t = nint[order[k]]; t < bd[order[k]].size(); ++t) touchers[fill[sid[bd[order[k]][t]]]++] = k;
  }
  auto seq_less = [&](uint32_t a, uint32_t b2) {
    const uint32_t la = t_off[a + 1] - t_off[a], lb = t_off[b2 + 1] - t_off[b2];
    const uint32_t *pa = &touchers[t_off[a]], *pb = &touchers[t_off[b2]];
    for (uint32_t i = 0; i < la && i < lb; ++i)
      if (pa[i] != pb[i]) return pa[i] < pb[i];
    if (la != lb) return la < lb;
    return a < b2;
  };
  auto same_group = [&](uint32_t a, uint32_t b2) {
    const uint32_t la = t_off[a + 1] - t_off[a], lb = t_off[b2 + 1] - t_off[b2];
    return la == lb && std::equal(&touchers[t_off[a]], &touchers[t_off[a]] + la, &touchers[t_off[b2]]);
  };
  std::vector<uint32_t> sorder(ns);
  std::iota(sorder.begin(), sorder.end(), 0u);
  std::sort(sorder.begin(), sorder.end(), seq_less);
  std::vector<uint32_t> spos(N, NONE);
  for (size_t i = 0; i < ns; ++i) spos[shared_ids[sorder[i]]] = (uint32_t)i;
  for (uint32_t b = 0; b < nb; ++b)
    std::sort(bd[b].begin() + nint[b], bd[b].end(), [&](uint32_t x, uint32_t y) { return spos[x] < spos[y]; });

  P.cell_order.clear();
  P.cell_order.reserve(nc);
  P.batch_cell_off.assign(1, 0);
  P.batch_dof_off.assign(1, 0);
  P.bdofs.clear();
  P.bflags.clear();
  P.lmap.assign((size_t)nc * nd, 0);
  std::vector<uint8_t> touched(N, 0);
  std::vector<uint16_t> pos_in_batch(N, 0);
  P.max_batch_dofs = P.max_batch_cells = 0;
  P.n_first = P.n_add = 0;
  P.batch_nint.clear();
  P.halo_off.assign(1, 0);
  for (uint32_t k = 0; k < nb; ++k) {
    const uint32_t b = order[k];
    const std::vector<uint32_t> &v = bd[b];
    P.batch_nint.push_back(nint[b]);
    P.halo_off.push_back(P.halo_off.back() +
                         (interior_max && (!batch_masked[b] || masked_planes) ? limits->halo_stride
                                                                              : (uint32_t)(v.size() - nint[b])));
    for (uint32_t g : v) {
      uint8_t f = 0;
      if (constrained[g]) f |= kFlagConstrained;
      if (touched[g]) {
        f |= kFlagAdd;
        ++P.n_add;
      } else {
        touched[g] = 1;
        ++P.n_first;
      }
      P.bdofs.push_back(g | (constrained[g] ? 0x80000000u : 0u));
      P.bflags.push_back(f);
    }
    for (size_t t = 0; t < v.size(); ++t) pos_in_batch[v[t]] = (uint16_t)t;
    for (uint32_t c : batches[b]) {
      const size_t pos = P.cell_order.size();
      P.cell_order.push_back(c);
      for (uint32_t i = 0; i < nd; ++i) P.lmap[pos * nd + i] = pos_in_batch[l2g[(uint64_t)c * nd + i]];
    }
    P.batch_cell_off.push_back((uint32_t)P.cell_order.size());
    P.batch_dof_off.push_back((uint32_t)P.bdofs.size());
    P.max_batch_dofs = std::max<uint32_t>(P.max_batch_dofs, (uint32_t)v.size());
    P.max_batch_cells = std::max<uint32_t>(P.max_batch_cells, (uint32_t)batches[b].size());
  }
  P.n_plane_batches = P.n_plain_plane_batches = 0;
  if (interior_max) {
    for (uint32_t k = 0; k < nb; ++k) {
      P.n_plain_plane_batches += batch_masked[order[k]] ? 0u : 1u;
      P.n_plane_batches += (batch_masked[order[k]] && !masked_planes) ? 0u : 1u;
    }
    if (masked_planes && P.n_plain_plane_batches < P.n_plane_batches) P.n_plain_plane_batches = 0;
  }
  P.orphans.clear();
  for (uint32_t g = 0; g < N; ++g)
    if (!touched[g]) P.orphans.push_back(g | (constrained[g] ? 0x80000000u : 0u));
  {
    P.sdofs.resize(ns);
    for (size_t i = 0; i < ns; ++i) {
      const uint32_t g = shared_ids[sorder[i]];
      P.sdofs[i] = g | (constrained[g] ? 0x80000000u : 0u);
    }
    P.s_off.assign(ns + 1, 0);
    for (size_t i = 0; i < ns; ++i) P.s_off[i + 1] = P.s_off[i] + ntouch[P.sdofs[i] & 0x7fffffffu];
    P.s_idx.assign(P.s_off[ns], 0);
    std::vector<uint32_t> fill(P.s_off.begin(), P.s_off.end() - 1);
    for (uint32_t k = 0; k < nb; ++k) {
      const uint32_t ni = P.batch_nint[k];
      const uint32_t d0 = P.batch_dof_off[k], d1 = P.batch_dof_off[k + 1];
      for (uint32_t t = d0 + ni; t < d1; ++t) {
        const uint32_t g = P.bdofs[t] & 0x7fffffffu;
        P.s_idx[fill[spos[g]]++] = P.halo_off[k] + (t - d0 - ni);
      }
    }
    P.chunks.clear();
    P.gstarts.clear();
    for (size_t i = 0; i < ns;) {
      size_t j = i + 1;
      while (j < ns && same_group(sorder[i], sorder[j])) ++j;
      const uint32_t k = P.s_off[i + 1] - P.s_off[i], tstart = (uint32_t)P.gstarts.size();
      for (uint32_t t = 0; t < k; ++t) P.gstarts.push_back(P.s_idx[P.s_off[i] + t]);
      for (size_t o = i; o < j; o += 64) {
        const uint32_t cnt = (uint32_t)std::min<size_t>(64, j - o);
        P.chunks.push_back((uint32_t)o);
        P.chunks.push_back(cnt | (k << 16));
        P.chunks.push_back(tstart);
        P.chunks.push_back((uint32_t)(o - i));
      }
      i = j;
    }
  }
  return 0;
}

int build_plane_records(Plan &P, const uint32_t *constraint_mask) {
  const int n = P.n, n2 = n * n, NT = p_cells_per_wave(n) * n, NIW = (n2 + 1) / 2;
  const int JI = p_ji(n) * 64, NB = p_kgu(n) * 64;
  const size_t nbat = P.n_plane_batches;
  const uint32_t dummy = 8u * (uint32_t)(NB - 1);
  std::vector<uint32_t> &bd = P.pr_dofs, &ix = P.pr_idx;
  bd.assign((size_t)NB * nbat, 0u);
  ix.assign((size_t)NIW * NT * nbat, dummy | (dummy << 16));
  std::vector<uint32_t> slot_of;
  const int HROWS = p_hn_rows(n), CR = p_priv_max(n) / 64;
  std::vector<uint32_t> &hnrec = P.pr_hn;
  hnrec.clear();
  P.pr_hn_slot.assign(nbat, 0xffffffffu);
  std::vector<HnLine> lines[3];
  std::vector<uint16_t> pnodes;
  std::vector<uint32_t> priv_pos((size_t)P.nd);
  for (size_t b = 0; b < nbat; ++b) {
    const uint32_t c0 = P.batch_cell_off[b], nc = P.batch_cell_off[b + 1] - c0;
    const uint32_t d0 = P.batch_dof_off[b], nbd = P.batch_dof_off[b + 1] - d0, ni = P.batch_nint[b];
    if ((int)nc * n > NT || (int)ni > JI || (int)(nbd - ni) >= NB - JI || nbd == ni) {
      set_error("internal: batch does not fit the plane kernel's dof-list slots");
      return MFGPU_EINVAL;
    }
    slot_of.assign(nbd, 0u);
    for (uint32_t t = 0; t < nbd; ++t) slot_of[t] = t < ni ? t : (uint32_t)JI + (t - ni);
    for (int t = 0; t < NB; ++t) {
      uint32_t src_t;
      if (t < JI) src_t = (uint32_t)t < ni ? (uint32_t)t : ni;
      else src_t = std::min<uint32_t>(ni + (uint32_t)(t - JI), nbd - 1);
      bd[b * NB + t] = P.bdofs[d0 + src_t];
    }
    bool hnb = false;
    if (constraint_mask && b >= P.n_plain_plane_batches)
      for (uint32_t c = 0; c < nc; ++c) hnb = hnb || constraint_mask[P.cell_order[c0 + c]] != 0;
    uint32_t next_priv = (uint32_t)NB;
    std::vector<uint32_t> copies, ops_d[3];
    for (uint32_t c = 0; c < nc; ++c) {
      const unsigned mask = hnb ? constraint_mask[P.cell_order[c0 + c]] : 0u;
      std::fill(priv_pos.begin(), priv_pos.end(), 0xffffffffu);
      if (mask) {
        hn_cell_lines(mask, n, lines, pnodes);
        for (uint16_t node : pnodes) {
          if (next_priv >= (uint32_t)NB + (uint32_t)p_priv_max(n)) {
            set_error("internal: batch exceeds the plane kernel's private hanging-node entries");
            return MFGPU_EINVAL;
          }
          priv_pos[node] = next_priv;
          copies.push_back((next_priv << 16) | slot_of[P.lmap[(size_t)(c0 + c) * P.nd + node]]);
          ++next_priv;
        }
        for (int dir = 0; dir < 3; ++dir)
          for (const HnLine &L : lines[dir]) {
            uint32_t w[3] = {0u, 0u, 0u};
            for (int t = 0; t < n; ++t) w[t >> 1] |= priv_pos[L.node[t]] << (16 * (t & 1));
            ops_d[dir].insert(ops_d[dir].end(), w, w + 3);
          }
      }
      for (int k = 0; k < n; ++k)
        for (int i = 0; i < n2; ++i) {
          const int node = i + n2 * k;
          const uint32_t pos = priv_pos[node] != 0xffffffffu ? priv_pos[node] : slot_of[P.lmap[(size_t)(c0 + c) * P.nd + node]];
          const uint32_t off = 8u * pos;
          uint32_t &w = ix[(b * NIW + i / 2) * NT + c * n + k];
          w = (i & 1) ? ((w & 0xffffu) | (off << 16)) : ((w & 0xffff0000u) | off);
        }
    }
    if (hnb) {
      P.pr_hn_slot[b] = (uint32_t)(hnrec.size() / ((size_t)HROWS * 64));
      hnrec.resize(hnrec.size() + (size_t)HROWS * 64, 0u);
      uint32_t *rec = hnrec.data() + (size_t)P.pr_hn_slot[b] * HROWS * 64;
      for (size_t e = 0; e < copies.size(); ++e) rec[e] = copies[e];
      for (int dir = 0; dir < 3; ++dir) {
        const size_t nops = ops_d[dir].size() / 3;
        if (nops > (size_t)kHnOpRounds * 64) {
          set_error("internal: more hanging-node lines in a batch than the plane kernel's record holds");
          return MFGPU_EINVAL;
        }
        for (size_t e = 0; e < nops; ++e)
          for (int w = 0; w < 3; ++w)
            rec[(size_t)(CR + (dir * kHnOpRounds + (int)(e / 64)) * 3 + w) * 64 + e % 64] = ops_d[dir][e * 3 + w];
      }
      const uint32_t h0 = (uint32_t)copies.size() | ((uint32_t)(ops_d[0].size() / 3) << 16);
      const uint32_t h1 = (uint32_t)(ops_d[1].size() / 3) | ((uint32_t)(ops_d[2].size() / 3) << 16);
      for (int l = 0; l < 64; ++l) {
        rec[(size_t)(HROWS - 2) * 64 + l] = h0;
        rec[(size_t)(HROWS - 1) * 64 + l] = h1;
      }
    }
  }
  share_plane_records(P);
  share_pass2_records(P);
  return 0;
}

namespace {
uint64_t hash_words(const uint32_t *w, size_t n) {
  uint64_t h = 1469598103934665603ull;
  for (size_t i = 0; i < n; ++i) h = (h ^ w[i]) * 1099511628211ull;
  return h;
}

uint32_t intern_record(std::vector<uint32_t> &table, std::unordered_multimap<uint64_t, uint32_t> &seen,
                       const uint32_t *rec, size_t len) {
  const uint64_t h = hash_words(rec, len);
  const auto range = seen.equal_range(h);
  for (auto it = range.first; it != range.second; ++it)
    if (!std::memcmp(table.data() + (size_t)it->second * len, rec, len * sizeof(uint32_t))) return it->second;
  const uint32_t id = (uint32_t)(table.size() / len);
  table.insert(table.end(), rec, rec + len);
  seen.emplace(h, id);
  return id;
}
}

void share_plane_records(Plan &P) {
  const int n = P.n, NT = p_cells_per_wave(n) * n, NIW = (n * n + 1) / 2;
  const size_t NB = (size_t)p_kgu(n) * 64, NX = (size_t)NIW * NT, nbat = P.n_plane_batches;
  P.sh_dofs.clear();
  P.sh_idx.clear();
  P.sh_batch.assign(nbat * kShBatchWords, 0u);
  std::unordered_multimap<uint64_t, uint32_t> seen_d, seen_x;
  std::vector<uint32_t> rel(NB);
  for (size_t b = 0; b < nbat; ++b) {
    const uint32_t *g = P.pr_dofs.data() + b * NB;
    uint32_t base = 0x7fffffffu;
    for (size_t t = 0; t < NB; ++t) base = std::min(base, g[t] & 0x7fffffffu);
    for (size_t t = 0; t < NB; ++t) rel[t] = g[t] - base;
    uint32_t *e = P.sh_batch.data() + b * kShBatchWords;
    e[0] = base;
    e[1] = intern_record(P.sh_dofs, seen_d, rel.data(), NB);
    e[2] = intern_record(P.sh_idx, seen_x, P.pr_idx.data() + b * NX, NX);
  }
  const size_t shared = P.sh_dofs.size() + P.sh_idx.size() + P.sh_batch.size();
  const size_t expanded = P.pr_dofs.size() + P.pr_idx.size();
  P.sh_use = nbat > 0 && P.pr_hn.empty() && (double)shared <= kShareMaxFraction * (double)expanded;
}

void share_pass2_records(Plan &P) {
  P.sh_p2rec.clear();
  P.sh_p2tab.clear();
  P.sh_p2_use = false;
  const size_t nb = P.batch_cell_off.size() - 1;
  const uint32_t hs = (uint32_t)p_hs(P.n) * 64u;
  if (nb == 0 || P.n_plane_batches != nb || P.halo_off.size() != nb + 1 || hs > (1u << kP2SlotBits)) return;
  for (size_t b = 0; b <= nb; ++b)
    if (P.halo_off[b] != (uint64_t)b * hs) return;
  std::vector<std::vector<uint32_t>> owned(nb);
  size_t expanded = 0;
  for (size_t i = 0; i < P.sdofs.size(); ++i) {
    const uint32_t k = P.s_off[i + 1] - P.s_off[i];
    expanded += 1 + (k ? k : 1);
    if (k == 0) continue;
    if (k > (uint32_t)kP2MaxK) return;
    const uint32_t owner = P.s_idx[P.s_off[i]] / hs;
    for (uint32_t t = 0; t < k; ++t) {
      const uint32_t tb = P.s_idx[P.s_off[i] + t] / hs;
      if (tb >= nb || tb < owner || tb - owner >= (1u << (32 - kP2SlotBits))) return;
    }
    owned[owner].push_back((uint32_t)i);
  }
  P.sh_p2tab.assign(2 * nb, 0u);
  std::unordered_multimap<uint64_t, std::pair<uint32_t, uint32_t>> seen;
  std::vector<uint32_t> rec;
  for (size_t b = 0; b < nb; ++b) {
    std::vector<uint32_t> &m = owned[b];
    auto k_of = [&](uint32_t i) { return P.s_off[i + 1] - P.s_off[i]; };
    std::stable_sort(m.begin(), m.end(), [&](uint32_t x, uint32_t y) { return k_of(x) > k_of(y); });
    const uint32_t base = P.sh_batch[b * kShBatchWords], ne = (uint32_t)m.size(), kmax = ne ? k_of(m[0]) : 0u;
    auto pad = [](uint32_t x) { return (x + 63u) & ~63u; };
    const uint32_t e0 = pad(ne);
    rec.assign(kP2Header, 0u);
    rec[0] = ne;
    rec[1] = e0;
    rec[2] = kmax;
    rec.resize(kP2Header + 2 * (size_t)e0, 0u);
    for (uint32_t e = 0; e < e0; ++e) rec[kP2Header + e] = e < ne ? P.sdofs[m[e]] - base : 0xffffffffu;
    for (uint32_t e = 0; e < ne; ++e) rec[kP2Header + e0 + e] = k_of(m[e]);
    for (uint32_t t = 0; t < kmax; ++t) {
      uint32_t cnt = 0;
      while (cnt < ne && k_of(m[cnt]) > t) ++cnt;
      rec[3 + t] = (uint32_t)rec.size();
      rec.resize(rec.size() + pad(cnt), 0u);
      for (uint32_t e = 0; e < cnt; ++e) {
        const uint32_t slot = P.s_idx[P.s_off[m[e]] + t], tb = slot / hs;
        rec[rec[3 + t] + e] = ((tb - (uint32_t)b) << kP2SlotBits) | (slot - tb * hs);
      }
    }
    const uint64_t h = hash_words(rec.data(), rec.size());
    uint32_t off = 0xffffffffu;
    const auto range = seen.equal_range(h);
    for (auto it = range.first; it != range.second && off == 0xffffffffu; ++it)
      if (it->second.second == rec.size() &&
          !std::memcmp(P.sh_p2rec.data() + it->second.first, rec.data(), rec.size() * sizeof(uint32_t)))
        off = it->second.first;
    if (off == 0xffffffffu) {
      off = (uint32_t)P.sh_p2rec.size();
      P.sh_p2rec.insert(P.sh_p2rec.end(), rec.begin(), rec.end());
      seen.emplace(h, std::make_pair(off, (uint32_t)rec.size()));
    }
    P.sh_p2tab[2 * b] = base;
    P.sh_p2tab[2 * b + 1] = off;
  }
  const size_t shared = P.sh_p2rec.size() + P.sh_p2tab.size();
  P.sh_p2_use = (double)shared <= kShareMaxFraction * (double)expanded;
}

int choose_kernel_and_plan(const mfgpu_desc &d, PlaneKernel &pk, BatchKernel &bk, Plan &plan) {
  const bool general = !(d.flags & MFGPU_UNIFORM_J0), hn = (d.flags & MFGPU_HANGING_NODES) != 0;
  const bool colored = (d.flags & MFGPU_COLORED_SCATTER) != 0;
  if (d.kernel > MFGPU_KERNEL_PLANES_2W) {
    set_error("unknown mfgpu_desc.kernel");
    return MFGPU_EINVAL;
  }
  const bool pk_ok = d.dim == 3 && !general && !colored && d.degree >= 2 && d.degree <= 6 &&
                     d.n_dofs < (1u << 29);
  const bool xk_ok = d.dim == 3 && !general && !colored;
  const bool want_planes = d.kernel == MFGPU_KERNEL_PLANES || d.kernel == MFGPU_KERNEL_PLANES_2W;
  if ((want_planes && !pk_ok) || (d.kernel == MFGPU_KERNEL_PENCILS_X && !xk_ok) ||
      (d.kernel == MFGPU_KERNEL_PENCILS && general)) {
    set_error("mfgpu_desc.kernel: this kernel family does not cover the description (see include/mfgpu.h)");
    return MFGPU_EUNSUPPORTED;
  }
  const bool planes4 = d.kernel == MFGPU_KERNEL_PLANES_2W || d.degree >= 5 ||
                       (d.kernel == MFGPU_KERNEL_AUTO && d.degree == 3 && d.number_type == MFGPU_F64);
  const PlaneKernel plane_kind = planes4 ? PlaneKernel::planes4 : PlaneKernel::planes3;
  const bool mass = d.mass_coefficient != nullptr;
  auto plane_kernel_exists = [&](bool with_hn) {
    return kernel_exists(plane_kind, d.degree + 1, d.number_type, with_hn, false, mass);
  };
  const bool mass_without_planes = mass && pk_ok && !plane_kernel_exists(false);
  if (mass_without_planes && want_planes) {
    set_error("mfgpu_desc.kernel: this plane kernel has no mass-term instantiation at this degree (apply_planes4w at "
              "p = 5, 6; apply_planes4 at p = 4 in double); use MFGPU_KERNEL_AUTO or MFGPU_KERNEL_PENCILS_X");
    return MFGPU_EUNSUPPORTED;
  }
  bool planes = pk_ok && !mass_without_planes && (want_planes || (d.kernel == MFGPU_KERNEL_AUTO &&
                                     (d.degree >= 4 || (d.degree == 3 && (hn || d.number_type == MFGPU_F64)))));
  bool pencils_x = xk_ok && !planes && d.kernel != MFGPU_KERNEL_PENCILS;
  PlanLimits lim;
  if (planes) {
    lim.max_cells = (uint32_t)p_cells_per_wave(d.degree + 1);
    lim.max_dofs = (uint32_t)p_kgu(d.degree + 1) * 64u - 1u;
    lim.interior_max = (uint32_t)p_ji(d.degree + 1) * 64u;
    lim.halo_stride = (uint32_t)p_hs(d.degree + 1) * 64u;
    lim.shared_max = lim.halo_stride - 1u;
    lim.segregate_masked = hn;
    lim.masked_planes = hn && plane_kernel_exists(true);
    lim.private_max = (uint32_t)p_priv_max(d.degree + 1);
  }
  int rc = build_plan(d, plan, (pencils_x && d.degree == 3) ? 4u : 3u, planes ? &lim : nullptr);
  if (rc == MFGPU_EUNSUPPORTED && planes && d.kernel == MFGPU_KERNEL_AUTO && xk_ok) {
    planes = false;
    pencils_x = true;
    plan = Plan();
    rc = build_plan(d, plan, d.degree == 3 ? 4u : 3u, nullptr);
  }
  if (!rc && planes) {
    const uint32_t nbat = (uint32_t)plan.batch_cell_off.size() - 1;
    pencils_x = plan.n_plane_batches < nbat;
    if (plan.n_plane_batches == 0) planes = false;
  }
  pk = planes ? plane_kind : PlaneKernel::none;
  bk = pencils_x ? BatchKernel::x : general ? (d.dim == 2 ? BatchKernel::g2 : BatchKernel::g)
                                   : planes ? BatchKernel::none : BatchKernel::batches;
  assert(rc || (pk != PlaneKernel::none) == (plan.n_plane_batches > 0));
  return rc;
}

}

extern "C" {

const char *mfgpu_last_error(void) { return mfgpu::last_error(); }

int mfgpu_plan_create(const mfgpu_desc *desc, mfgpu_plan **out) {
  if (!desc || !out) {
    mfgpu::set_error("null argument");
    return MFGPU_EINVAL;
  }
  mfgpu_plan *p = new mfgpu_plan();
  mfgpu::PlaneKernel pk;
  mfgpu::BatchKernel bk;
  mfgpu_desc d = *desc;
  d.mass_coefficient = nullptr;
  int rc = mfgpu::choose_kernel_and_plan(d, pk, bk, p->plan);
  if (!rc && pk != mfgpu::PlaneKernel::none) rc = mfgpu::build_plane_records(p->plan, desc->constraint_mask);
  if (rc) {
    delete p;
    return rc;
  }
  *out = p;
  return 0;
}

void mfgpu_plan_destroy(mfgpu_plan *p) { delete p; }

size_t mfgpu_desc_size(void) { return sizeof(mfgpu_desc); }

int mfgpu_suggest_renumbering(const mfgpu_desc *desc, uint32_t *new_index) {
  if (!desc || !new_index) {
    mfgpu::set_error("null argument");
    return MFGPU_EINVAL;
  }
  mfgpu::Plan P;
  mfgpu::PlaneKernel pk;
  mfgpu::BatchKernel bk;
  mfgpu_desc d = *desc;
  d.mass_coefficient = nullptr;
  int rc = mfgpu::choose_kernel_and_plan(d, pk, bk, P);
  if (rc) return rc;
  const uint32_t NONE = 0xffffffffu;
  std::fill(new_index, new_index + desc->n_dofs, NONE);
  uint32_t next = 0;
  const size_t nb = P.batch_cell_off.size() - 1;
  for (size_t b = 0; b < nb; ++b) {
    const uint32_t d0 = P.batch_dof_off[b];
    const uint32_t ni = P.batch_nint.empty() ? P.batch_dof_off[b + 1] - d0 : P.batch_nint[b];
    for (uint32_t t = 0; t < ni; ++t) {
      const uint32_t g = P.bdofs[d0 + t] & 0x7fffffffu;
      if (new_index[g] == NONE) new_index[g] = next++;
    }
  }
  for (uint32_t e : P.sdofs) {
    const uint32_t g = e & 0x7fffffffu;
    if (new_index[g] == NONE) new_index[g] = next++;
  }
  for (uint32_t g = 0; g < desc->n_dofs; ++g)
    if (new_index[g] == NONE) new_index[g] = next++;
  if (next != desc->n_dofs) {
    mfgpu::set_error("internal: renumbering is not a permutation");
    return MFGPU_EINVAL;
  }
  return 0;
}

int64_t mfgpu_plan_array_u32(const mfgpu_plan *p, int what, const uint32_t **ptr) {
  if (!p || !ptr) return MFGPU_EINVAL;
  const std::vector<uint32_t> *v = nullptr;
  switch (what) {
    case 0: v = &p->plan.batch_cell_off; break;
    case 1: v = &p->plan.batch_dof_off; break;
    case 2: v = &p->plan.color_batch_off; break;
    case 3: v = &p->plan.cell_order; break;
    case 4: v = &p->plan.bdofs; break;
    case 5: v = &p->plan.orphans; break;
    case 6: v = &p->plan.batch_nint; break;
    case 7: v = &p->plan.halo_off; break;
    case 8: v = &p->plan.sdofs; break;
    case 9: v = &p->plan.s_off; break;
    case 10: v = &p->plan.s_idx; break;
    case 11: v = &p->plan.chunks; break;
    case 12: v = &p->plan.gstarts; break;
    case 13: v = &p->plan.pr_dofs; break;
    case 14: v = &p->plan.pr_idx; break;
    case 15: v = &p->plan.pr_hn; break;
    case 16: v = &p->plan.pr_hn_slot; break;
    case 17: v = &p->plan.sh_dofs; break;
    case 18: v = &p->plan.sh_idx; break;
    case 19: v = &p->plan.sh_batch; break;
    case 20: v = &p->plan.sh_p2rec; break;
    case 21: v = &p->plan.sh_p2tab; break;
    default: mfgpu::set_error("bad array id"); return MFGPU_EINVAL;
  }
  *ptr = v->data();
  return (int64_t)v->size();
}

int mfgpu_plan_shares_records(const mfgpu_plan *p) {
  return p ? (p->plan.sh_use ? 1 : 0) | (p->plan.sh_p2_use ? 2 : 0) : 0;
}

int64_t mfgpu_plan_lmap(const mfgpu_plan *p, const uint16_t **ptr) {
  if (!p || !ptr) return MFGPU_EINVAL;
  *ptr = p->plan.lmap.data();
  return (int64_t)p->plan.lmap.size();
}

int64_t mfgpu_plan_bflags(const mfgpu_plan *p, const uint8_t **ptr) {
  if (!p || !ptr) return MFGPU_EINVAL;
  *ptr = p->plan.bflags.data();
  return (int64_t)p->plan.bflags.size();
}

}
```

dealii-cuda_amd/pymfgpu/__init__.py:

```python
from __future__ import annotations

import ctypes as C
import os

import numpy as np

_HERE = os.path.dirname(os.path.abspath(__file__))
LIB_PATH = os.environ.get("MFGPU_LIB") or os.path.join(os.path.dirname(_HERE), "lib", "libmfgpu.so")

F64, F32 = 0, 1
OK, EINVAL = 0, -1
UNIFORM_J0, HANGING_NODES, COLORED_SCATTER, NO_SHARED_RECORDS = 1, 2, 1 << 8, 1 << 9
KERNEL_AUTO, KERNEL_PENCILS, KERNEL_PENCILS_X, KERNEL_PLANES, KERNEL_PLANES_2W = 0, 1, 2, 3, 4


class MfgpuError(RuntimeError):
    pass


class Desc(C.Structure):
    _fields_ = [
        ("dim", C.c_int32), ("degree", C.c_int32), ("number_type", C.c_int32), ("flags", C.c_uint32),
        ("n_dofs", C.c_uint32), ("n_cells", C.c_uint32),
        ("loc2glob", C.c_void_p), ("constraint_mask", C.c_void_p),
        ("JxW", C.c_void_p), ("inv_jac", C.c_void_p), ("coefficient", C.c_void_p),
        ("quadrature_points", C.c_void_p), ("shape_values", C.c_void_p), ("shape_gradients", C.c_void_p),
        ("constraint_weights", C.c_void_p), ("constrained_dofs", C.c_void_p),
        ("n_constrained", C.c_uint32), ("max_cells_per_batch", C.c_uint32), ("max_dofs_per_batch", C.c_uint32),
        ("kernel", C.c_uint32), ("cell_loop_segments", C.c_uint32), ("max_workgroups", C.c_uint32),
        ("mass_coefficient", C.c_void_p),
    ]


SYMBOLS = [
    "mfgpu_create", "mfgpu_vmult", "mfgpu_vmult_add", "mfgpu_n_dofs", "mfgpu_memory_consumption",
    "mfgpu_destroy", "mfgpu_last_error", "mfgpu_plan_stats", "mfgpu_kernel_name", "mfgpu_compute_inverse_diagonal", "mfgpu_set_constrained_values",
    "mfgpu_vec_sadd", "mfgpu_vec_equ", "mfgpu_vec_scale", "mfgpu_vec_divide", "mfgpu_vec_invert", "mfgpu_vec_mul",
    "mfgpu_vec_dot", "mfgpu_vec_l2_norm", "mfgpu_vec_add_and_dot", "mfgpu_vec_all_zero", "mfgpu_profile_enable", "mfgpu_profile_read", "mfgpu_profile_read_pass2",
    "mfgpu_plan_create", "mfgpu_plan_destroy", "mfgpu_plan_array_u32", "mfgpu_plan_lmap", "mfgpu_plan_bflags",
    "mfgpu_plan_shares_records", "mfgpu_record_stats",
    "mfgpu_vec_alloc", "mfgpu_vec_free", "mfgpu_vec_fill", "mfgpu_vec_from_host", "mfgpu_vec_to_host",
    "mfgpu_device_synchronize", "mfgpu_device_memory_info", "mfgpu_mesh_create_uniform", "mfgpu_mesh_create_adaptive", "mfgpu_mesh_create_ball", "mfgpu_mesh_create_from_leaves",
    "mfgpu_mesh_cell_levels", "mfgpu_mesh_destroy",
    "mfgpu_mesh_desc", "mfgpu_mesh_dof_coords", "mfgpu_mesh_interface_dofs",
    "mfgpu_dist_unique_id", "mfgpu_dist_create", "mfgpu_dist_connect_local", "mfgpu_dist_attach", "mfgpu_dist_schedule",
    "mfgpu_vmult_dist_begin", "mfgpu_vmult_dist_end", "mfgpu_vmult_dist", "mfgpu_dist_destroy",
    "mfgpu_transfer_create", "mfgpu_transfer_create_from_meshes", "mfgpu_transfer_prolongate",
    "mfgpu_transfer_restrict_and_add", "mfgpu_transfer_memory_consumption", "mfgpu_transfer_destroy",
    "mfgpu_mesh_transfer_patches", "mfgpu_suggest_renumbering", "mfgpu_mesh_renumber",
    "mfgpu_level_create", "mfgpu_level_operator", "mfgpu_level_vmult_interface_down", "mfgpu_level_vmult_interface_up",
    "mfgpu_level_destroy", "mfgpu_index_pairs_create", "mfgpu_vec_copy_pairs", "mfgpu_index_pairs_destroy",
    "mfgpu_mesh_create_adaptive_mg", "mfgpu_mg_hierarchy_create", "mfgpu_mg_n_levels", "mfgpu_mg_level_mesh",
    "mfgpu_mg_edge_dofs", "mfgpu_mg_copy_pairs", "mfgpu_mg_transfer_arrays", "mfgpu_mg_hierarchy_destroy",
    "mfgpu_integrator_create", "mfgpu_integrator_rhs", "mfgpu_integrator_l2_error", "mfgpu_integrator_error_points",
    "mfgpu_integrator_destroy",
    "mfgpu_vec_convert", "mfgpu_vec_copy_pairs_convert", "mfgpu_vec_chebyshev_start", "mfgpu_vec_chebyshev_update",
    "mfgpu_desc_size",
]

_lib = None


def lib():
    global _lib
    if _lib is None:
        if not os.path.exists(LIB_PATH):
            raise MfgpuError(f"{LIB_PATH} not found: build it with __graft_entry__.build() "
                             "(make -C dealii-cuda_amd); there is no fallback path")
        L = C.CDLL(LIB_PATH)
        L.mfgpu_last_error.restype = C.c_char_p
        L.mfgpu_create.argtypes = [C.POINTER(Desc), C.POINTER(C.c_void_p)]
        L.mfgpu_desc_size.argtypes = []
        L.mfgpu_desc_size.restype = C.c_size_t
        L.mfgpu_vmult.argtypes = [C.c_void_p, C.c_void_p, C.c_void_p, C.c_void_p]
        L.mfgpu_vmult_add.argtypes = [C.c_void_p, C.c_void_p, C.c_void_p, C.c_void_p]
        L.mfgpu_n_dofs.argtypes = [C.c_void_p]
        L.mfgpu_n_dofs.restype = C.c_uint32
        L.mfgpu_memory_consumption.argtypes = [C.c_void_p]
        L.mfgpu_memory_consumption.restype = C.c_size_t
        L.mfgpu_destroy.argtypes = [C.c_void_p]
        L.mfgpu_destroy.restype = None
        L.mfgpu_plan_stats.argtypes = [C.c_void_p, C.POINTER(C.c_uint64)]
        L.mfgpu_device_memory_info.argtypes = [C.POINTER(C.c_size_t), C.POINTER(C.c_size_t)]
        L.mfgpu_kernel_name.argtypes = [C.c_void_p]
        L.mfgpu_kernel_name.restype = C.c_char_p
        L.mfgpu_compute_inverse_diagonal.argtypes = [C.c_void_p, C.c_void_p, C.c_void_p]
        L.mfgpu_set_constrained_values.argtypes = [C.c_void_p, C.c_void_p, C.c_double, C.c_void_p]
        vp, d, z, i = C.c_void_p, C.c_double, C.c_size_t, C.c_int
        L.mfgpu_vec_sadd.argtypes = [vp, d, d, vp, z, i, vp]
        L.mfgpu_vec_equ.argtypes = [vp, d, vp, z, i, vp]
        L.mfgpu_vec_scale.argtypes = [vp, vp, z, i, vp]
        L.mfgpu_vec_divide.argtypes = [vp, vp, z, i, vp]
        L.mfgpu_vec_invert.argtypes = [vp, z, i, vp]
        L.mfgpu_vec_mul.argtypes = [vp, d, z, i, vp]
        L.mfgpu_vec_dot.argtypes = [vp, vp, z, i, vp, C.POINTER(d)]
        L.mfgpu_vec_l2_norm.argtypes = [vp, z, i, vp, C.POINTER(d)]
        L.mfgpu_vec_add_and_dot.argtypes = [vp, d, vp, vp, z, i, vp, C.POINTER(d)]
        L.mfgpu_vec_all_zero.argtypes = [vp, z, i, vp, C.POINTER(i)]
        L.mfgpu_profile_enable.argtypes = [C.c_void_p, C.c_int]
        L.mfgpu_profile_read.argtypes = [C.c_void_p, C.POINTER(C.c_double), C.POINTER(C.c_uint64)]
        L.mfgpu_profile_read_pass2.argtypes = [C.c_void_p, C.POINTER(C.c_double)]
        L.mfgpu_plan_create.argtypes = [C.POINTER(Desc), C.POINTER(C.c_void_p)]
        L.mfgpu_plan_destroy.argtypes = [C.c_void_p]
        L.mfgpu_plan_destroy.restype = None
        L.mfgpu_plan_array_u32.argtypes = [C.c_void_p, C.c_int, C.POINTER(C.c_void_p)]
        L.mfgpu_plan_array_u32.restype = C.c_int64
        L.mfgpu_plan_lmap.argtypes = [C.c_void_p, C.POINTER(C.c_void_p)]
        L.mfgpu_plan_lmap.restype = C.c_int64
        L.mfgpu_plan_bflags.argtypes = [C.c_void_p, C.POINTER(C.c_void_p)]
        L.mfgpu_plan_bflags.restype = C.c_int64
        L.mfgpu_plan_shares_records.argtypes = [C.c_void_p]
        L.mfgpu_record_stats.argtypes = [C.c_void_p, C.POINTER(C.c_uint64)]
        L.mfgpu_vec_alloc.argtypes = [C.POINTER(C.c_void_p), C.c_size_t, C.c_int]
        L.mfgpu_vec_free.argtypes = [C.c_void_p]
        L.mfgpu_vec_fill.argtypes = [C.c_void_p, C.c_size_t, C.c_int, C.c_double, C.c_void_p]
        L.mfgpu_vec_from_host.argtypes = [C.c_void_p, C.c_void_p, C.c_size_t, C.c_int]
        L.mfgpu_vec_to_host.argtypes = [C.c_void_p, C.c_void_p, C.c_size_t, C.c_int]
        L.mfgpu_mesh_create_uniform.argtypes = [C.c_int, C.c_int, C.POINTER(C.c_uint32), C.c_double, C.c_double,
                                                C.c_uint32, C.c_uint32, C.c_int, C.POINTER(C.c_void_p)]
        L.mfgpu_mesh_create_adaptive.argtypes = [C.c_int, C.c_int, C.c_int, C.c_int, C.POINTER(C.c_void_p)]
        L.mfgpu_mesh_create_ball.argtypes = [C.c_int, C.c_int, C.c_int, C.c_int, C.POINTER(C.c_void_p)]
        L.mfgpu_mesh_create_from_leaves.argtypes = [C.c_int, C.c_int, C.c_void_p, C.c_uint32, C.c_int, C.POINTER(C.c_void_p)]
        L.mfgpu_mesh_cell_levels.argtypes = [C.c_void_p, C.POINTER(C.c_void_p)]
        L.mfgpu_mesh_cell_levels.restype = C.c_int64
        L.mfgpu_mesh_destroy.argtypes = [C.c_void_p]
        L.mfgpu_mesh_destroy.restype = None
        L.mfgpu_mesh_desc.argtypes = [C.c_void_p, C.POINTER(Desc)]
        L.mfgpu_mesh_dof_coords.argtypes = [C.c_void_p, C.POINTER(C.c_void_p)]
        L.mfgpu_mesh_dof_coords.restype = C.c_int64
        L.mfgpu_mesh_interface_dofs.argtypes = [C.c_void_p, C.c_int, C.POINTER(C.c_void_p)]
        L.mfgpu_mesh_interface_dofs.restype = C.c_int64
        L.mfgpu_transfer_create.argtypes = [C.c_int, C.c_int, C.c_int, C.c_uint32, C.c_void_p, C.c_void_p, C.c_uint32,
                                            C.c_uint32, C.c_void_p, C.c_uint32, C.c_void_p, C.POINTER(C.c_void_p)]
        L.mfgpu_transfer_create_from_meshes.argtypes = [C.c_void_p, C.c_void_p, C.POINTER(C.c_void_p)]
        L.mfgpu_transfer_prolongate.argtypes = [C.c_void_p, C.c_void_p, C.c_void_p, C.c_void_p]
        L.mfgpu_transfer_restrict_and_add.argtypes = [C.c_void_p, C.c_void_p, C.c_void_p, C.c_void_p]
        L.mfgpu_transfer_memory_consumption.argtypes = [C.c_void_p]
        L.mfgpu_transfer_memory_consumption.restype = C.c_size_t
        L.mfgpu_mesh_transfer_patches.argtypes = [C.c_void_p, C.c_void_p, C.c_void_p, C.c_void_p]
        L.mfgpu_mesh_transfer_patches.restype = C.c_int64
        L.mfgpu_suggest_renumbering.argtypes = [C.POINTER(Desc), C.c_void_p]
        L.mfgpu_mesh_renumber.argtypes = [C.c_void_p, C.c_void_p]
        L.mfgpu_level_create.argtypes = [C.POINTER(Desc), C.c_void_p, C.c_uint32, C.POINTER(C.c_void_p)]
        L.mfgpu_level_operator.argtypes = [C.c_void_p]
        L.mfgpu_level_operator.restype = C.c_void_p
        L.mfgpu_level_vmult_interface_down.argtypes = [C.c_void_p, C.c_void_p, C.c_void_p, C.c_void_p]
        L.mfgpu_level_vmult_interface_up.argtypes = [C.c_void_p, C.c_void_p, C.c_void_p, C.c_void_p]
        L.mfgpu_mesh_create_adaptive_mg.argtypes = [C.c_int, C.c_int, C.c_int, C.c_int, C.POINTER(C.c_void_p)]
        L.mfgpu_mg_hierarchy_create.argtypes = [C.c_void_p, C.POINTER(C.c_void_p)]
        L.mfgpu_mg_n_levels.argtypes = [C.c_void_p]
        L.mfgpu_mg_level_mesh.argtypes = [C.c_void_p, C.c_int]
        L.mfgpu_mg_level_mesh.restype = C.c_void_p
        L.mfgpu_mg_edge_dofs.argtypes = [C.c_void_p, C.c_int, C.POINTER(C.c_void_p)]
        L.mfgpu_mg_edge_dofs.restype = C.c_int64
        L.mfgpu_mg_copy_pairs.argtypes = [C.c_void_p, C.c_int, C.POINTER(C.c_void_p), C.POINTER(C.c_void_p)]
        L.mfgpu_mg_copy_pairs.restype = C.c_int64
        L.mfgpu_mg_transfer_arrays.argtypes = [C.c_void_p, C.c_int, C.POINTER(C.c_void_p), C.POINTER(C.c_void_p)]
        L.mfgpu_mg_transfer_arrays.restype = C.c_int64
        L.mfgpu_mg_hierarchy_destroy.argtypes = [C.c_void_p]
        L.mfgpu_mg_hierarchy_destroy.restype = None
        L.mfgpu_index_pairs_create.argtypes = [C.c_void_p, C.c_void_p, C.c_uint32, C.POINTER(C.c_void_p)]
        L.mfgpu_vec_copy_pairs.argtypes = [C.c_void_p, C.c_void_p, C.c_void_p, C.c_int, C.c_void_p]
        L.mfgpu_index_pairs_destroy.argtypes = [C.c_void_p]
        L.mfgpu_index_pairs_destroy.restype = None
        L.mfgpu_level_destroy.argtypes = [C.c_void_p]
        L.mfgpu_level_destroy.restype = None
        L.mfgpu_transfer_destroy.argtypes = [C.c_void_p]
        L.mfgpu_transfer_destroy.restype = None
        L.mfgpu_integrator_create.argtypes = [C.POINTER(Desc), C.POINTER(C.c_void_p)]
        L.mfgpu_integrator_rhs.argtypes = [C.c_void_p, C.c_void_p, C.c_void_p, C.c_void_p, C.c_void_p]
        L.mfgpu_integrator_l2_error.argtypes = [C.c_void_p, C.c_void_p, C.c_void_p, C.c_void_p, C.c_void_p,
                                                C.POINTER(C.c_double)]
        L.mfgpu_integrator_error_points.argtypes = [C.c_void_p, C.c_void_p, C.c_void_p]
        L.mfgpu_integrator_destroy.argtypes = [C.c_void_p]
        L.mfgpu_integrator_destroy.restype = None
        L.mfgpu_vec_convert.argtypes = [vp, i, vp, i, z, vp]
        L.mfgpu_vec_copy_pairs_convert.argtypes = [vp, vp, i, vp, i, vp]
        L.mfgpu_vec_chebyshev_start.argtypes = [vp, vp, vp, vp, vp, vp, d, i, z, i, vp]
        L.mfgpu_vec_chebyshev_update.argtypes = [vp, vp, vp, vp, vp, d, d, z, i, vp]
        _lib = L
    return _lib


def _check(rc):
    if rc != 0:
        raise MfgpuError(f"mfgpu error {rc}: {lib().mfgpu_last_error().decode()}")


def np_dtype(number_type):
    return np.float64 if number_type == F64 else np.float32


def _view(ptr, count, dtype):
    if count <= 0 or not ptr:
        return np.zeros(0, dtype=dtype)
    buf = (C.c_char * (count * np.dtype(dtype).itemsize)).from_address(ptr)
    return np.frombuffer(buf, dtype=dtype, count=count)


class Mesh:

    def __init__(self, handle, keep=None):
        self._h = handle
        self._keep = keep
        self.desc = Desc()
        _check(lib().mfgpu_mesh_desc(self._h, C.byref(self.desc)))

    @classmethod
    def uniform(cls, dim, degree, n_per_dir, lo=-1.0, hi=1.0, slab=(0, 0), number_type=F64):
        if np.isscalar(n_per_dir):
            n_per_dir = [int(n_per_dir)] * dim
        arr = (C.c_uint32 * 3)(*(list(n_per_dir) + [1] * (3 - len(n_per_dir))))
        h = C.c_void_p()
        _check(lib().mfgpu_mesh_create_uniform(dim, degree, arr, lo, hi, slab[0], slab[1], number_type, C.byref(h)))
        return cls(h)

    @classmethod
    def adaptive(cls, dim, degree, n_ref, number_type=F64):
        h = C.c_void_p()
        _check(lib().mfgpu_mesh_create_adaptive(dim, degree, n_ref, number_type, C.byref(h)))
        return cls(h)

    @classmethod
    def adaptive_mg(cls, dim, degree, n_ref, number_type=F64):
        h = C.c_void_p()
        _check(lib().mfgpu_mesh_create_adaptive_mg(dim, degree, n_ref, number_type, C.byref(h)))
        return cls(h)

    @classmethod
    def ball(cls, dim, degree, n_ref, number_type=F64):
        h = C.c_void_p()
        _check(lib().mfgpu_mesh_create_ball(dim, degree, n_ref, number_type, C.byref(h)))
        return cls(h)

    @classmethod
    def from_leaves(cls, dim, degree, leaves, number_type=F64):
        lv = np.ascontiguousarray(leaves, dtype=np.uint32).reshape(-1, 4)
        h = C.c_void_p()
        _check(lib().mfgpu_mesh_create_from_leaves(dim, degree, lv.ctypes.data, len(lv), number_type, C.byref(h)))
        return cls(h)

    def cell_levels(self):
        p = C.c_void_p()
        cnt = lib().mfgpu_mesh_cell_levels(self._h, C.byref(p))
        return _view(p.value, cnt, np.uint32).reshape(-1, 4).copy()

    def __del__(self):
        if getattr(self, "_h", None) and _lib is not None and getattr(self, "_owner", None) is None:
            _lib.mfgpu_mesh_destroy(self._h)
            self._h = None

    @property
    def n_dofs(self):
        return int(self.desc.n_dofs)

    @property
    def n_cells(self):
        return int(self.desc.n_cells)

    @property
    def nd(self):
        return (self.desc.degree + 1) ** self.desc.dim

    def arrays(self):
        d = self.desc
        dt = np_dtype(d.number_type)
        nd, nc, n = self.nd, d.n_cells, d.degree + 1
        out = dict(
            loc2glob=_view(d.loc2glob, nc * nd, np.uint32).reshape(nc, nd),
            JxW=_view(d.JxW, nc * nd, dt).reshape(nc, nd),
            inv_jac=(_view(d.inv_jac, nc, dt) if d.flags & UNIFORM_J0
                     else _view(d.inv_jac, nc * nd * d.dim * d.dim, dt).reshape(nc, nd, d.dim, d.dim)),
            quadrature_points=_view(d.quadrature_points, nc * nd * d.dim, dt).reshape(nc, nd, d.dim),
            shape_values=_view(d.shape_values, n * n, dt),
            shape_gradients=_view(d.shape_gradients, n * n, dt),
            constraint_weights=_view(d.constraint_weights, n * n, np.float64),
            constrained_dofs=_view(d.constrained_dofs, d.n_constrained, np.uint32),
            constraint_mask=_view(d.constraint_mask, nc, np.uint32) if d.constraint_mask else None,
        )
        return out

    def set_mass_coefficient(self, c):
        if c is None:
            self._mass, self.desc.mass_coefficient = None, None
            return
        self._mass = np.ascontiguousarray(c, dtype=np_dtype(self.desc.number_type)).reshape(-1)
        assert self._mass.size == self.n_cells * self.nd
        self.desc.mass_coefficient = self._mass.ctypes.data

    def dof_coords(self):
        p = C.c_void_p()
        cnt = lib().mfgpu_mesh_dof_coords(self._h, C.byref(p))
        return _view(p.value, cnt, np.float64).reshape(-1, self.desc.dim)

    def suggest_renumbering(self):
        out = np.zeros(self.n_dofs, dtype=np.uint32)
        _check(lib().mfgpu_suggest_renumbering(C.byref(self.desc), out.ctypes.data))
        return out

    def renumber(self, new_index):
        ni = np.ascontiguousarray(new_index, dtype=np.uint32)
        assert ni.size == self.n_dofs
        _check(lib().mfgpu_mesh_renumber(self._h, ni.ctypes.data))
        _check(lib().mfgpu_mesh_desc(self._h, C.byref(self.desc)))

    def transfer_patches(self, fine: "Mesh"):
        p, dim = self.desc.degree, self.desc.dim
        cd = np.zeros((self.n_cells, (p + 1) ** dim), dtype=np.uint32)
        fd = np.zeros((self.n_cells, (2 * p + 1) ** dim), dtype=np.uint32)
        rc = lib().mfgpu_mesh_transfer_patches(self._h, fine._h, cd.ctypes.data, fd.ctypes.data)
        if rc < 0:
            _check(int(rc))
        return cd, fd

    def interface_dofs(self, which):
        p = C.c_void_p()
        cnt = lib().mfgpu_mesh_interface_dofs(self._h, which, C.byref(p))
        return _view(p.value, cnt, np.uint32).copy()


def make_desc(dim, degree, n_dofs, loc2glob, JxW, inv_jac, coefficient, constrained,
              shape_values, shape_gradients, number_type=F64, constraint_mask=None,
              constraint_weights=None, quadrature_points=None, max_cells_per_batch=0, max_dofs_per_batch=0,
              colored=False, kernel=0, cell_loop_segments=0, max_workgroups=0, mass_coefficient=None):
    dt = np_dtype(number_type)
    keep = []

    def ptr(a, dtype):
        if a is None:
            return None
        a = np.ascontiguousarray(a, dtype=dtype)
        keep.append(a)
        return a.ctypes.data

    d = Desc()
    d.dim, d.degree, d.number_type = dim, degree, number_type
    l2g = np.ascontiguousarray(loc2glob, dtype=np.uint32)
    d.n_dofs = int(n_dofs)
    d.n_cells = l2g.size // ((degree + 1) ** dim)
    uniform = np.asarray(inv_jac).size == d.n_cells
    assert uniform or np.asarray(inv_jac).size == l2g.size * dim * dim
    d.flags = ((UNIFORM_J0 if uniform else 0) | (HANGING_NODES if constraint_mask is not None else 0)
               | (COLORED_SCATTER if colored else 0))
    d.loc2glob = ptr(l2g, np.uint32)
    d.constraint_mask = ptr(constraint_mask, np.uint32)
    d.JxW = ptr(JxW, dt)
    d.inv_jac = ptr(inv_jac, dt)
    d.coefficient = ptr(coefficient, dt)
    d.quadrature_points = ptr(quadrature_points, dt)
    d.shape_values = ptr(shape_values, dt)
    d.shape_gradients = ptr(shape_gradients, dt)
    d.constraint_weights = ptr(constraint_weights, np.float64)
    c = np.ascontiguousarray(constrained, dtype=np.uint32)
    d.constrained_dofs = ptr(c, np.uint32)
    d.n_constrained = c.size
    d.max_cells_per_batch = max_cells_per_batch
    d.max_dofs_per_batch = max_dofs_per_batch
    d.kernel = kernel
    d.cell_loop_segments = cell_loop_segments
    d.max_workgroups = max_workgroups
    d.mass_coefficient = ptr(mass_coefficient, dt)
    return d, keep


class Plan:

    def __init__(self, desc: Desc, keep=None):
        self._keep = keep
        self.nd = (desc.degree + 1) ** desc.dim
        h = C.c_void_p()
        _check(lib().mfgpu_plan_create(C.byref(desc), C.byref(h)))
        self._h = h

    def __del__(self):
        if getattr(self, "_h", None) and _lib is not None:
            _lib.mfgpu_plan_destroy(self._h)
            self._h = None

    def _u32(self, what):
        p = C.c_void_p()
        cnt = lib().mfgpu_plan_array_u32(self._h, what, C.byref(p))
        if cnt < 0:
            _check(int(cnt))
        return _view(p.value, cnt, np.uint32).copy()

    batch_cell_off = property(lambda s: s._u32(0))
    batch_dof_off = property(lambda s: s._u32(1))
    color_batch_off = property(lambda s: s._u32(2))
    cell_order = property(lambda s: s._u32(3))
    bdofs = property(lambda s: s._u32(4) & np.uint32(0x7fffffff))
    bdofs_constrained = property(lambda s: (s._u32(4) >> np.uint32(31)).astype(bool))
    orphans = property(lambda s: s._u32(5))
    batch_nint = property(lambda s: s._u32(6))
    halo_off = property(lambda s: s._u32(7))
    sdofs = property(lambda s: s._u32(8))
    s_off = property(lambda s: s._u32(9))
    s_idx = property(lambda s: s._u32(10))
    chunks = property(lambda s: s._u32(11).reshape(-1, 4))
    gstarts = property(lambda s: s._u32(12))
    pr_dofs = property(lambda s: s._u32(13))
    pr_idx = property(lambda s: s._u32(14))
    pr_hn = property(lambda s: s._u32(15))
    pr_hn_slot = property(lambda s: s._u32(16))
    sh_dofs = property(lambda s: s._u32(17))
    sh_idx = property(lambda s: s._u32(18))
    sh_batch = property(lambda s: s._u32(19).reshape(-1, 4))
    shares_records = property(lambda s: bool(lib().mfgpu_plan_shares_records(s._h) & 1))
    sh_p2rec = property(lambda s: s._u32(20))
    sh_p2tab = property(lambda s: s._u32(21).reshape(-1, 2))
    shares_pass2_records = property(lambda s: bool(lib().mfgpu_plan_shares_records(s._h) & 2))

    @property
    def lmap(self):
        p = C.c_void_p()
        cnt = lib().mfgpu_plan_lmap(self._h, C.byref(p))
        return _view(p.value, cnt, np.uint16).reshape(-1, self.nd).copy()

    @property
    def bflags(self):
        p = C.c_void_p()
        cnt = lib().mfgpu_plan_bflags(self._h, C.byref(p))
        return _view(p.value, cnt, np.uint8).copy()


class DeviceVector:

    def __init__(self, n, number_type=F64):
        self.n, self.number_type = int(n), number_type
        p = C.c_void_p()
        _check(lib().mfgpu_vec_alloc(C.byref(p), self.n, number_type))
        self.ptr = p.value

    def __del__(self):
        if getattr(self, "ptr", None) and _lib is not None:
            _lib.mfgpu_vec_free(self.ptr)
            self.ptr = None

    def fill(self, value, stream=None):
        _check(lib().mfgpu_vec_fill(self.ptr, self.n, self.number_type, float(value), stream))

    def from_host(self, a):
        a = np.ascontiguousarray(a, dtype=np_dtype(self.number_type))
        assert a.size == self.n
        _check(lib().mfgpu_vec_from_host(self.ptr, a.ctypes.data, self.n, self.number_type))

    def to_host(self):
        a = np.empty(self.n, dtype=np_dtype(self.number_type))
        _check(lib().mfgpu_vec_to_host(a.ctypes.data, self.ptr, self.n, self.number_type))
        return a

    def swap(self, other):
        self.ptr, other.ptr = other.ptr, self.ptr
        self.n, other.n = other.n, self.n

    def _a(self, other=None):
        if other is not None:
            assert other.n == self.n and other.number_type == self.number_type
        return self.n, self.number_type

    def sadd(self, s, a, w, stream=None):
        _check(lib().mfgpu_vec_sadd(self.ptr, float(s), float(a), w.ptr, *self._a(w), stream))

    def add(self, a, w, stream=None):
        self.sadd(1.0, a, w, stream)

    def equ(self, a, w, stream=None):
        _check(lib().mfgpu_vec_equ(self.ptr, float(a), w.ptr, *self._a(w), stream))

    def scale(self, w, stream=None):
        _check(lib().mfgpu_vec_scale(self.ptr, w.ptr, *self._a(w), stream))

    def divide(self, w, stream=None):
        _check(lib().mfgpu_vec_divide(self.ptr, w.ptr, *self._a(w), stream))

    def invert(self, stream=None):
        _check(lib().mfgpu_vec_invert(self.ptr, *self._a(), stream))

    def mul(self, a, stream=None):
        _check(lib().mfgpu_vec_mul(self.ptr, float(a), *self._a(), stream))

    def dot(self, w, stream=None):
        r = C.c_double()
        _check(lib().mfgpu_vec_dot(self.ptr, w.ptr, *self._a(w), stream, C.byref(r)))
        return r.value

    def l2_norm(self, stream=None):
        r = C.c_double()
        _check(lib().mfgpu_vec_l2_norm(self.ptr, *self._a(), stream, C.byref(r)))
        return r.value

    def add_and_dot(self, a, x, w, stream=None):
        r = C.c_double()
        self._a(x)
        _check(lib().mfgpu_vec_add_and_dot(self.ptr, float(a), x.ptr, w.ptr, *self._a(w), stream, C.byref(r)))
        return r.value

    def all_zero(self, stream=None):
        r = C.c_int()
        _check(lib().mfgpu_vec_all_zero(self.ptr, *self._a(), stream, C.byref(r)))
        return bool(r.value)


class Operator:

    def __init__(self, desc: Desc, keep=None):
        self._keep = keep
        self.number_type = desc.number_type
        h = C.c_void_p()
        _check(lib().mfgpu_create(C.byref(desc), C.byref(h)))
        self._h = h

    def __del__(self):
        self.clear()

    def clear(self):
        if getattr(self, "_h", None) and _lib is not None:
            _lib.mfgpu_destroy(self._h)
            self._h = None

    def n(self):
        return int(lib().mfgpu_n_dofs(self._h))

    m = n

    def vmult(self, dst, src, stream=None):
        _check(lib().mfgpu_vmult(self._h, _ptr(dst), _ptr(src), stream))

    def vmult_add(self, dst, src, stream=None):
        _check(lib().mfgpu_vmult_add(self._h, _ptr(dst), _ptr(src), stream))

    def memory_consumption(self):
        return int(lib().mfgpu_memory_consumption(self._h))

    def plan_stats(self):
        s = (C.c_uint64 * 8)()
        _check(lib().mfgpu_plan_stats(self._h, s))
        keys = ["n_batches", "n_launches", "batch_dofs", "max_batch_dofs", "max_batch_cells", "n_orphans",
                "first_touch_or_shared_dofs", "rmw_adds_or_halo_slots"]
        out = dict(zip(keys, [int(v) for v in s]))
        r = (C.c_uint64 * 4)()
        _check(lib().mfgpu_record_stats(self._h, r))
        out.update(index_records="shared" if r[0] & 1 else "expanded",
                   pass2_records="shared" if r[0] & 2 else "expanded", distinct_dof_records=int(r[1]),
                   distinct_index_records=int(r[2]), index_record_bytes=int(r[3]))
        return out

    def kernel_name(self):
        return lib().mfgpu_kernel_name(self._h).decode()

    def compute_inverse_diagonal(self, inv_diag, stream=None):
        _check(lib().mfgpu_compute_inverse_diagonal(self._h, _ptr(inv_diag), stream))

    def set_constrained_values(self, vec, value, stream=None):
        _check(lib().mfgpu_set_constrained_values(self._h, _ptr(vec), float(value), stream))

    def profile_enable(self, on=True):
        _check(lib().mfgpu_profile_enable(self._h, int(on)))

    def profile_read(self):
        ms, nv = C.c_double(), C.c_uint64()
        _check(lib().mfgpu_profile_read(self._h, C.byref(ms), C.byref(nv)))
        return ms.value, int(nv.value)

    def profile_read_pass2(self):
        ms = C.c_double()
        _check(lib().mfgpu_profile_read_pass2(self._h, C.byref(ms)))
        return ms.value


class Integrator:

    def __init__(self, desc: Desc, keep=None):
        self._keep = keep
        self.dim, self.degree, self.n_cells = int(desc.dim), int(desc.degree), int(desc.n_cells)
        h = C.c_void_p()
        _check(lib().mfgpu_integrator_create(C.byref(desc), C.byref(h)))
        self._h = h

    def __del__(self):
        if getattr(self, "_h", None) and _lib is not None:
            _lib.mfgpu_integrator_destroy(self._h)
            self._h = None

    @property
    def n_error_points(self):
        return (self.degree + 2) ** self.dim

    def rhs(self, dst, f=None, u_b=None, stream=None):
        _check(lib().mfgpu_integrator_rhs(self._h, _ptr(dst), None if f is None else _ptr(f),
                                          None if u_b is None else _ptr(u_b), stream))

    def l2_error(self, u, exact=None, per_cell=None, stream=None):
        r = C.c_double()
        _check(lib().mfgpu_integrator_l2_error(self._h, _ptr(u), None if exact is None else _ptr(exact),
                                               None if per_cell is None else _ptr(per_cell), stream, C.byref(r)))
        return r.value

    def error_points(self):
        v = DeviceVector(self.n_cells * self.n_error_points * self.dim)
        _check(lib().mfgpu_integrator_error_points(self._h, v.ptr, None))
        return v.to_host().reshape(self.n_cells, self.n_error_points, self.dim)


class MgHierarchy:

    def __init__(self, mesh: "Mesh"):
        h = C.c_void_p()
        _check(lib().mfgpu_mg_hierarchy_create(mesh._h, C.byref(h)))
        self._h = h
        self.n_levels = int(lib().mfgpu_mg_n_levels(h))

    def level_mesh(self, level):
        m = Mesh.__new__(Mesh)
        m._owner = self
        m._h = C.c_void_p(lib().mfgpu_mg_level_mesh(self._h, level))
        m.desc = Desc()
        _check(lib().mfgpu_mesh_desc(m._h, C.byref(m.desc)))
        return m

    def edge_dofs(self, level):
        p = C.c_void_p()
        n = lib().mfgpu_mg_edge_dofs(self._h, level, C.byref(p))
        return _view(p.value, n, np.uint32).copy()

    def copy_pairs(self, level):
        a, b = C.c_void_p(), C.c_void_p()
        n = lib().mfgpu_mg_copy_pairs(self._h, level, C.byref(a), C.byref(b))
        return _view(a.value, n, np.uint32).copy(), _view(b.value, n, np.uint32).copy()

    def transfer_arrays(self, level, nd, nfd):
        a, b = C.c_void_p(), C.c_void_p()
        n = lib().mfgpu_mg_transfer_arrays(self._h, level, C.byref(a), C.byref(b))
        return _view(a.value, n * nd, np.uint32).reshape(n, nd).copy(), _view(b.value, n * nfd, np.uint32).reshape(n, nfd).copy()

    def __del__(self):
        if getattr(self, "_h", None) and _lib is not None:
            _lib.mfgpu_mg_hierarchy_destroy(self._h)
            self._h = None


class Level:

    def __init__(self, desc: Desc, edge_dofs, keep=None):
        self._keep = keep
        e = np.ascontiguousarray(edge_dofs, dtype=np.uint32)
        h = C.c_void_p()
        _check(lib().mfgpu_level_create(C.byref(desc), e.ctypes.data if e.size else None, e.size, C.byref(h)))
        self._h = h
        self.number_type = desc.number_type

    def vmult(self, dst, src, stream=None):
        _check(lib().mfgpu_vmult(lib().mfgpu_level_operator(self._h), _ptr(dst), _ptr(src), stream))

    def compute_inverse_diagonal(self, inv_diag, stream=None):
        _check(lib().mfgpu_compute_inverse_diagonal(lib().mfgpu_level_operator(self._h), _ptr(inv_diag), stream))

    def vmult_interface_down(self, dst, src, stream=None):
        _check(lib().mfgpu_level_vmult_interface_down(self._h, _ptr(dst), _ptr(src), stream))

    def vmult_interface_up(self, dst, src, stream=None):
        _check(lib().mfgpu_level_vmult_interface_up(self._h, _ptr(dst), _ptr(src), stream))

    def __del__(self):
        if getattr(self, "_h", None) and _lib is not None:
            _lib.mfgpu_level_destroy(self._h)
            self._h = None


class Transfer:

    def __init__(self, handle):
        self._h = handle

    @classmethod
    def from_arrays(cls, dim, degree, coarse_cell_dofs, fine_patch_dofs, n_coarse_dofs, n_fine_dofs, coarse_dirichlet,
                    number_type=F64, prolongation_1d=None):
        cd = np.ascontiguousarray(coarse_cell_dofs, dtype=np.uint32)
        fd = np.ascontiguousarray(fine_patch_dofs, dtype=np.uint32)
        di = np.ascontiguousarray(coarse_dirichlet, dtype=np.uint32)
        p1 = None if prolongation_1d is None else np.ascontiguousarray(prolongation_1d, dtype=np.float64)
        n_cells = cd.size // ((degree + 1) ** dim)
        assert fd.size == n_cells * (2 * degree + 1) ** dim
        h = C.c_void_p()
        _check(lib().mfgpu_transfer_create(dim, degree, number_type, n_cells, cd.ctypes.data, fd.ctypes.data, n_coarse_dofs,
                                           n_fine_dofs, di.ctypes.data if di.size else None, di.size,
                                           None if p1 is None else p1.ctypes.data, C.byref(h)))
        return cls(h)

    @classmethod
    def from_meshes(cls, coarse: "Mesh", fine: "Mesh"):
        h = C.c_void_p()
        _check(lib().mfgpu_transfer_create_from_meshes(coarse._h, fine._h, C.byref(h)))
        return cls(h)

    def prolongate(self, dst_fine, src_coarse, stream=None):
        _check(lib().mfgpu_transfer_prolongate(self._h, _ptr(dst_fine), _ptr(src_coarse), stream))

    def restrict_and_add(self, dst_coarse, src_fine, stream=None):
        _check(lib().mfgpu_transfer_restrict_and_add(self._h, _ptr(dst_coarse), _ptr(src_fine), stream))

    def memory_consumption(self):
        return int(lib().mfgpu_transfer_memory_consumption(self._h))

    def __del__(self):
        if getattr(self, "_h", None) and _lib is not None:
            _lib.mfgpu_transfer_destroy(self._h)
            self._h = None


def _ptr(v):
    if isinstance(v, DeviceVector):
        return v.ptr
    if hasattr(v, "data_ptr"):
        return v.data_ptr()
    return int(v)


class IndexPairs:

    def __init__(self, dst_idx, src_idx):
        a = np.ascontiguousarray(dst_idx, dtype=np.uint32)
        b = np.ascontiguousarray(src_idx, dtype=np.uint32)
        assert a.size == b.size
        h = C.c_void_p()
        _check(lib().mfgpu_index_pairs_create(a.ctypes.data if a.size else None, b.ctypes.data if b.size else None,
                                              a.size, C.byref(h)))
        self._h = h

    def copy(self, dst, src, number_type=F64, stream=None):
        _check(lib().mfgpu_vec_copy_pairs(self._h, _ptr(dst), _ptr(src), number_type, stream))

    def __del__(self):
        if getattr(self, "_h", None) and _lib is not None:
            _lib.mfgpu_index_pairs_destroy(self._h)
            self._h = None


def vec_convert(dst, dst_type, src, src_type, n, stream=None, check=True):
    rc = lib().mfgpu_vec_convert(_ptr(dst), dst_type, _ptr(src), src_type, n, stream)
    return _check(rc) if check else rc


def copy_pairs_convert(pairs: "IndexPairs", dst, dst_type, src, src_type, stream=None, check=True):
    rc = lib().mfgpu_vec_copy_pairs_convert(pairs._h, _ptr(dst), dst_type, _ptr(src), src_type, stream)
    return _check(rc) if check else rc


def chebyshev_start(x, upd, r, b, t, dinv, f, zero_start, n, number_type, stream=None, check=True):
    rc = lib().mfgpu_vec_chebyshev_start(_ptr(x), _ptr(upd), _ptr(r), _ptr(b), None if t is None else _ptr(t),
                                         _ptr(dinv), float(f), 1 if zero_start else 0, n, number_type, stream)
    return _check(rc) if check else rc


def chebyshev_update(x, upd, r, t, dinv, f1, f2, n, number_type, stream=None, check=True):
    rc = lib().mfgpu_vec_chebyshev_update(_ptr(x), _ptr(upd), _ptr(r), _ptr(t), _ptr(dinv), float(f1), float(f2), n,
                                          number_type, stream)
    return _check(rc) if check else rc


def synchronize():
    _check(lib().mfgpu_device_synchronize())


def device_memory_info():
    f, t = C.c_size_t(), C.c_size_t()
    _check(lib().mfgpu_device_memory_info(C.byref(f), C.byref(t)))
    return f.value, t.value


def dist_unique_id() -> bytes:
    buf = C.create_string_buffer(128)
    _check(lib().mfgpu_dist_unique_id(buf))
    return buf.raw


class Dist:

    def __init__(self, mesh: "Mesh", rank: int, world: int, unique_id=None):
        lo = np.ascontiguousarray(mesh.interface_dofs(0), dtype=np.uint32)
        up = np.ascontiguousarray(mesh.interface_dofs(1), dtype=np.uint32)
        con = np.ascontiguousarray(mesh.arrays()["constrained_dofs"], dtype=np.uint32)
        self._keep = (lo, up, con)
        self.number_type = mesh.desc.number_type
        d = C.c_void_p()
        L = lib()
        L.mfgpu_dist_create.argtypes = [C.c_char_p, C.c_int, C.c_int, C.c_void_p, C.c_uint32, C.c_void_p, C.c_uint32,
                                        C.c_void_p, C.c_uint32, C.c_uint32, C.c_int, C.c_void_p]
        _check(L.mfgpu_dist_create(unique_id, rank, world, lo.ctypes.data if lo.size else None, lo.size,
                                   up.ctypes.data if up.size else None, up.size, con.ctypes.data if con.size else None,
                                   con.size, mesh.n_dofs, self.number_type, C.byref(d)))
        self._d = d
        for f in ("mfgpu_dist_connect_local", "mfgpu_dist_attach"):
            getattr(L, f).argtypes = [C.c_void_p, C.c_void_p]
        L.mfgpu_vmult_dist_begin.argtypes = [C.c_void_p, C.c_void_p, C.c_void_p, C.c_void_p, C.c_void_p]
        L.mfgpu_vmult_dist.argtypes = [C.c_void_p, C.c_void_p, C.c_void_p, C.c_void_p, C.c_void_p]
        L.mfgpu_vmult_dist_end.argtypes = [C.c_void_p, C.c_void_p, C.c_void_p, C.c_void_p]
        L.mfgpu_dist_destroy.argtypes = [C.c_void_p]

    def __del__(self):
        if getattr(self, "_d", None) and _lib is not None:
            _lib.mfgpu_dist_destroy(self._d)
            self._d = None

    def connect_local(self, upper: "Dist"):
        _check(lib().mfgpu_dist_connect_local(self._d, upper._d))

    def attach(self, op: "Operator"):
        _check(lib().mfgpu_dist_attach(self._d, op._h))

    def schedule(self):
        info = (C.c_uint32 * 4)()
        lib().mfgpu_dist_schedule.argtypes = [C.c_void_p, C.c_void_p]
        _check(lib().mfgpu_dist_schedule(self._d, info))
        return bool(info[0]), int(info[1]), int(info[2]), int(info[3])

    def vmult_begin(self, op, dst, src, stream=None):
        _check(lib().mfgpu_vmult_dist_begin(op._h, self._d, _ptr(dst), _ptr(src), stream))

    def vmult_end(self, op, dst, stream=None):
        _check(lib().mfgpu_vmult_dist_end(op._h, self._d, _ptr(dst), stream))

    def vmult(self, op, dst, src, stream=None):
        _check(lib().mfgpu_vmult_dist(op._h, self._d, _ptr(dst), _ptr(src), stream))
```

include/mfgpu.h:

```cpp
#ifndef MFGPU_H
#define MFGPU_H

#include <stddef.h>
#include <stdint.h>

#ifdef __cplusplus
extern "C" {
#endif

#define MFGPU_OK 0
#define MFGPU_EINVAL (-1)
#define MFGPU_EHIP (-2)
#define MFGPU_ENOMEM (-3)
#define MFGPU_EUNSUPPORTED (-4)

#define MFGPU_F64 0
#define MFGPU_F32 1

#define MFGPU_UNIFORM_J0 (1u << 0)
#define MFGPU_HANGING_NODES (1u << 1)

#define MFGPU_COLORED_SCATTER (1u << 8)

#define MFGPU_NO_SHARED_RECORDS (1u << 9)

typedef struct mfgpu_handle mfgpu_handle;

typedef struct mfgpu_desc {
  int32_t dim;
  int32_t degree;
  int32_t number_type;
  uint32_t flags;
  uint32_t n_dofs;
  uint32_t n_cells;
  const uint32_t *loc2glob;
  const uint32_t *constraint_mask;
  const void *JxW;
  const void *inv_jac;
  const void *coefficient;
  const void *quadrature_points;
  const void *shape_values;
  const void *shape_gradients;
  const double *constraint_weights;
  const uint32_t *constrained_dofs;
  uint32_t n_constrained;
  uint32_t max_cells_per_batch;
  uint32_t max_dofs_per_batch;
  uint32_t kernel;
  uint32_t cell_loop_segments;
  uint32_t max_workgroups;
  const void *mass_coefficient;
} mfgpu_desc;

size_t mfgpu_desc_size(void);

#define MFGPU_KERNEL_AUTO 0
#define MFGPU_KERNEL_PENCILS 1
#define MFGPU_KERNEL_PENCILS_X 2
#define MFGPU_KERNEL_PLANES 3
#define MFGPU_KERNEL_PLANES_2W 4


int mfgpu_create(const mfgpu_desc *desc, mfgpu_handle **out);

int mfgpu_vmult(mfgpu_handle *h, void *dst_dev, const void *src_dev, void *stream);

int mfgpu_vmult_add(mfgpu_handle *h, void *dst_dev, const void *src_dev, void *stream);

uint32_t mfgpu_n_dofs(const mfgpu_handle *h);

size_t mfgpu_memory_consumption(const mfgpu_handle *h);

void mfgpu_destroy(mfgpu_handle *h);

const char *mfgpu_last_error(void);

int mfgpu_plan_stats(const mfgpu_handle *h, uint64_t stats[8]);

int mfgpu_record_stats(const mfgpu_handle *h, uint64_t stats[4]);

const char *mfgpu_kernel_name(const mfgpu_handle *h);

int mfgpu_profile_enable(mfgpu_handle *h, int on);
int mfgpu_profile_read(mfgpu_handle *h, double *kernel_ms_total, uint64_t *n_vmults);
int mfgpu_profile_read_pass2(mfgpu_handle *h, double *pass2_ms_total);

typedef struct mfgpu_plan mfgpu_plan;
int mfgpu_plan_create(const mfgpu_desc *desc, mfgpu_plan **out);
void mfgpu_plan_destroy(mfgpu_plan *p);
int64_t mfgpu_plan_array_u32(const mfgpu_plan *p, int what, const uint32_t **ptr);
int mfgpu_plan_shares_records(const mfgpu_plan *p);
int64_t mfgpu_plan_lmap(const mfgpu_plan *p, const uint16_t **ptr);
int64_t mfgpu_plan_bflags(const mfgpu_plan *p, const uint8_t **ptr);

int mfgpu_suggest_renumbering(const mfgpu_desc *desc, uint32_t *new_index );

int mfgpu_compute_inverse_diagonal(mfgpu_handle *h, void *inv_diag, void *stream);
int mfgpu_set_constrained_values(mfgpu_handle *h, void *vec, double value, void *stream);

int mfgpu_vec_sadd(void *v, double s, double a, const void *w, size_t n, int number_type, void *stream);
int mfgpu_vec_equ(void *v, double a, const void *w, size_t n, int number_type, void *stream);
int mfgpu_vec_scale(void *v, const void *w, size_t n, int number_type, void *stream);
int mfgpu_vec_divide(void *v, const void *w, size_t n, int number_type, void *stream);
int mfgpu_vec_invert(void *v, size_t n, int number_type, void *stream);
int mfgpu_vec_mul(void *v, double a, size_t n, int number_type, void *stream);
int mfgpu_vec_dot(const void *v, const void *w, size_t n, int number_type, void *stream, double *result);
int mfgpu_vec_l2_norm(const void *v, size_t n, int number_type, void *stream, double *result);
int mfgpu_vec_add_and_dot(void *v, double a, const void *x, const void *w, size_t n, int number_type,
                          void *stream, double *result);
int mfgpu_vec_all_zero(const void *v, size_t n, int number_type, void *stream, int *result);

int mfgpu_vec_alloc(void **dev, size_t n, int number_type);
int mfgpu_vec_free(void *dev);
int mfgpu_vec_fill(void *dev, size_t n, int number_type, double value, void *stream);
int mfgpu_vec_from_host(void *dev, const void *host, size_t n, int number_type);
int mfgpu_vec_to_host(void *host, const void *dev, size_t n, int number_type);
int mfgpu_device_synchronize(void);
int mfgpu_device_memory_info(size_t *free_bytes, size_t *total_bytes);

typedef struct mfgpu_dist mfgpu_dist;
int mfgpu_dist_unique_id(void *id128);
int mfgpu_dist_create(const void *id128, int rank, int world, const uint32_t *lower_ids, uint32_t n_lower,
                      const uint32_t *upper_ids, uint32_t n_upper, const uint32_t *constrained_dofs,
                      uint32_t n_constrained, uint32_t n_dofs, int number_type, mfgpu_dist **out);
int mfgpu_dist_connect_local(mfgpu_dist *lower_rank, mfgpu_dist *upper_rank);
int mfgpu_dist_attach(mfgpu_dist *d, mfgpu_handle *h);
int mfgpu_dist_schedule(const mfgpu_dist *d, uint32_t info[4]);
int mfgpu_vmult_dist_begin(mfgpu_handle *h, mfgpu_dist *d, void *dst_dev, const void *src_dev, void *stream);
int mfgpu_vmult_dist_end(mfgpu_handle *h, mfgpu_dist *d, void *dst_dev, void *stream);
int mfgpu_vmult_dist(mfgpu_handle *h, mfgpu_dist *d, void *dst_dev, const void *src_dev, void *stream);
void mfgpu_dist_destroy(mfgpu_dist *d);

typedef struct mfgpu_transfer mfgpu_transfer;
int mfgpu_transfer_create(int dim, int degree, int number_type, uint32_t n_coarse_cells,
                          const uint32_t *coarse_cell_dofs ,
                          const uint32_t *fine_patch_dofs  , uint32_t n_coarse_dofs,
                          uint32_t n_fine_dofs, const uint32_t *coarse_dirichlet, uint32_t n_coarse_dirichlet,
                          const double *prolongation_1d ,
                          mfgpu_transfer **out);
int mfgpu_transfer_prolongate(mfgpu_transfer *t, void *dst_fine_dev, const void *src_coarse_dev, void *stream);
int mfgpu_transfer_restrict_and_add(mfgpu_transfer *t, void *dst_coarse_dev, const void *src_fine_dev, void *stream);
size_t mfgpu_transfer_memory_consumption(const mfgpu_transfer *t);
void mfgpu_transfer_destroy(mfgpu_transfer *t);

typedef struct mfgpu_level mfgpu_level;
int mfgpu_level_create(const mfgpu_desc *desc, const uint32_t *edge_dofs, uint32_t n_edge, mfgpu_level **out);
mfgpu_handle *mfgpu_level_operator(mfgpu_level *level);
int mfgpu_level_vmult_interface_down(mfgpu_level *level, void *dst_dev, const void *src_dev, void *stream);
int mfgpu_level_vmult_interface_up(mfgpu_level *level, void *dst_dev, const void *src_dev, void *stream);
void mfgpu_level_destroy(mfgpu_level *level);

typedef struct mfgpu_index_pairs mfgpu_index_pairs;
int mfgpu_index_pairs_create(const uint32_t *dst_idx, const uint32_t *src_idx, uint32_t n, mfgpu_index_pairs **out);
int mfgpu_vec_copy_pairs(const mfgpu_index_pairs *p, void *dst_dev, const void *src_dev, int number_type, void *stream);
void mfgpu_index_pairs_destroy(mfgpu_index_pairs *p);

int mfgpu_vec_convert(void *dst, int dst_type, const void *src, int src_type, size_t n, void *stream);
int mfgpu_vec_copy_pairs_convert(const mfgpu_index_pairs *p, void *dst, int dst_type, const void *src, int src_type,
                                 void *stream);
int mfgpu_vec_chebyshev_start(void *x, void *upd, void *r, const void *b, const void *t, const void *dinv, double f,
                              int zero_start, size_t n, int number_type, void *stream);
int mfgpu_vec_chebyshev_update(void *x, void *upd, void *r, const void *t, const void *dinv, double f1, double f2,
                               size_t n, int number_type, void *stream);

typedef struct mfgpu_integrator mfgpu_integrator;
int mfgpu_integrator_create(const mfgpu_desc *desc, mfgpu_integrator **out);
int mfgpu_integrator_rhs(mfgpu_integrator *it, void *rhs, const void *f_qp, const void *u_b, void *stream);
int mfgpu_integrator_l2_error(mfgpu_integrator *it, const void *u, const void *exact, void *per_cell, void *stream,
                              double *l2);
int mfgpu_integrator_error_points(mfgpu_integrator *it, void *points, void *stream);
void mfgpu_integrator_destroy(mfgpu_integrator *it);

typedef struct mfgpu_mesh mfgpu_mesh;

int mfgpu_mesh_create_uniform(int dim, int degree, const uint32_t *n_per_dir, double lo, double hi,
                              uint32_t slab_begin, uint32_t slab_end, int number_type,
                              mfgpu_mesh **out);
int mfgpu_mesh_create_adaptive(int dim, int degree, int n_ref, int number_type, mfgpu_mesh **out);
int mfgpu_mesh_create_ball(int dim, int degree, int n_ref, int number_type, mfgpu_mesh **out);
int mfgpu_transfer_create_from_meshes(const mfgpu_mesh *coarse, const mfgpu_mesh *fine, mfgpu_transfer **out);
int64_t mfgpu_mesh_transfer_patches(const mfgpu_mesh *coarse, const mfgpu_mesh *fine, uint32_t *coarse_cell_dofs,
                                    uint32_t *fine_patch_dofs);
int mfgpu_mesh_renumber(mfgpu_mesh *m, const uint32_t *new_index);
int mfgpu_mesh_create_adaptive_mg(int dim, int degree, int n_ref, int number_type, mfgpu_mesh **out);
typedef struct mfgpu_mg_hierarchy mfgpu_mg_hierarchy;
int mfgpu_mg_hierarchy_create(const mfgpu_mesh *adaptive, mfgpu_mg_hierarchy **out);
int mfgpu_mg_n_levels(const mfgpu_mg_hierarchy *h);
const mfgpu_mesh *mfgpu_mg_level_mesh(const mfgpu_mg_hierarchy *h, int level);
int64_t mfgpu_mg_edge_dofs(const mfgpu_mg_hierarchy *h, int level, const uint32_t **ptr);
int64_t mfgpu_mg_copy_pairs(const mfgpu_mg_hierarchy *h, int level, const uint32_t **active_dofs, const uint32_t **level_dofs);
int64_t mfgpu_mg_transfer_arrays(const mfgpu_mg_hierarchy *h, int level, const uint32_t **coarse_cell_dofs,
                                 const uint32_t **fine_patch_dofs);
void mfgpu_mg_hierarchy_destroy(mfgpu_mg_hierarchy *h);
int mfgpu_mesh_create_from_leaves(int dim, int degree, const uint32_t *leaves, uint32_t n_leaves,
                                  int number_type, mfgpu_mesh **out);
int64_t mfgpu_mesh_cell_levels(const mfgpu_mesh *m, const uint32_t **ptr);
void mfgpu_mesh_destroy(mfgpu_mesh *m);
int mfgpu_mesh_desc(const mfgpu_mesh *m, mfgpu_desc *desc);
int64_t mfgpu_mesh_dof_coords(const mfgpu_mesh *m, const double **ptr);
int64_t mfgpu_mesh_interface_dofs(const mfgpu_mesh *m, int which, const uint32_t **ptr);

#ifdef __cplusplus
}
#endif
#endif
```

Baseline: 80.43 billion DoFs/s.

## Carry shared-face partial sums across consecutive plane batches in registers

Adds a chained variant of the planes3 kernel (n=5, shared records, no hanging nodes). Consecutive batches handled by the same workgroup pass the partial results for their shared DoF plane through one extra register slot instead of writing them to the halo buffer. Those DoFs are then dropped from the pass-2 reduction. The host builds a batch order, a set of links and new dof/index/pass-2 records for a given grid size, and uses the chained path only when the whole range runs at that grid. The aim is less halo traffic and less pass-2 work. In exchange the kernel uses an extra register and LDS slot, and the records and pass-2 tables become more complex.

Result: no change. 80.31 billion DoFs/s (-0.2%).

```diff
diff --git a/dealii-cuda_amd/csrc/mfgpu_api.hip b/dealii-cuda_amd/csrc/mfgpu_api.hip
--- a/dealii-cuda_amd/csrc/mfgpu_api.hip
+++ b/dealii-cuda_amd/csrc/mfgpu_api.hip
@@ -83,6 +83,10 @@
   std::vector<uint32_t> n_p2tiles;
   DeviceArray<uint32_t> d_p2rec, d_p2tab;
   bool p2_shared = false, p2_reverse = false, no_shared_records = false;
+  bool carry = false, cells_chained = false;
+  uint32_t chain_grid = 0, chain_run = 0;
+  uint64_t chain_links = 0, chain_carried = 0;
+  DeviceArray<uint32_t> d_ch_dofs, d_ch_idx, d_ch_tab, d_ch_p2rec, d_ch_p2tab;
   Stream side;
   std::vector<Event> ev_seg;
   Event ev_side;
@@ -92,9 +96,9 @@
   size_t lds = 0, device_bytes = 0;
   PlaneKernel planes = PlaneKernel::none;
   BatchKernel batches = BatchKernel::none;
-  enum { kPlain, kMasked, kBatch };
-  CellKernel<double> kernels_f64[3];
-  CellKernel<float> kernels_f32[3];
+  enum { kPlain, kMasked, kBatch, kChained };
+  CellKernel<double> kernels_f64[4];
+  CellKernel<float> kernels_f32[4];
   template <typename T>
   CellKernel<T> &kernel(int which) {
     if constexpr (std::is_same<T, double>::value) return kernels_f64[which];
@@ -120,15 +124,21 @@
 }
 
 template <typename T>
+uint32_t grid_of(mfgpu_handle *h, int which, uint32_t nbat) {
+  const CellKernel<T> &k = h->kernel<T>(which);
+  uint32_t grid = (uint32_t)(k.per_cu < 1 ? 1 : k.per_cu) * h->n_cus;
+  if (h->max_workgroups && h->max_workgroups < grid) grid = h->max_workgroups;
+  return nbat < grid ? nbat : grid;
+}
+
+template <typename T>
 int launch_bound(mfgpu_handle *h, int which, const ApplyArgs<T> &a, uint32_t nbat, hipStream_t st) {
   const CellKernel<T> &k = h->kernel<T>(which);
   if (!k.launch[0]) {
     set_error("cell-loop kernel not bound");
     return MFGPU_EINVAL;
   }
-  uint32_t grid = (uint32_t)(k.per_cu < 1 ? 1 : k.per_cu) * h->n_cus;
-  if (h->max_workgroups && h->max_workgroups < grid) grid = h->max_workgroups;
-  HIP_TRY(k.launch[a.add != 0](a, h->S.data(), h->Dt.data(), k.lds, nbat < grid ? nbat : grid, st));
+  HIP_TRY(k.launch[a.add != 0](a, h->S.data(), h->Dt.data(), k.lds, grid_of<T>(h, which, nbat), st));
   return 0;
 }
 
@@ -365,6 +375,27 @@
       HIP_TRY(bind_kernel<T>(h, h->planes, BatchKernel::none, true, false, &masked));
       h->lds = std::max(h->lds, masked.lds);
     }
+    const uint32_t nb = (uint32_t)(P.batch_cell_off.size() - 1);
+    const bool mass = d.mass_coefficient != nullptr;
+    if (h->shared_records && P.sh_p2_use && !(d.flags & MFGPU_NO_CARRY) && P.n_plain_plane_batches == nb &&
+        h->planes == PlaneKernel::planes3 && kernel_exists(h->planes, P.n, d.number_type, false, true, mass, true)) {
+      CellKernel<T> &chained = h->kernel<T>(mfgpu_handle::kChained);
+      HIP_TRY(p_bind_chained<T>(P.n, mass, &chained));
+      Chain c;
+      if (!build_chain(P, grid_of<T>(h, mfgpu_handle::kChained, nb), (uint32_t)kChainRun, c) && !c.links.empty()) {
+        if ((rc = up(h->d_ch_dofs, c.dofs.data(), c.dofs.size()))) return rc;
+        if ((rc = up(h->d_ch_idx, c.idx.data(), c.idx.size()))) return rc;
+        if ((rc = up(h->d_ch_tab, c.tab.data(), c.tab.size()))) return rc;
+        if ((rc = up(h->d_ch_p2rec, c.p2rec.data(), c.p2rec.size()))) return rc;
+        if ((rc = up(h->d_ch_p2tab, c.p2tab.data(), c.p2tab.size()))) return rc;
+        h->carry = true;
+        h->chain_grid = c.grid;
+        h->chain_run = c.run;
+        h->chain_links = c.links.size();
+        h->chain_carried = c.carried;
+        h->lds = std::max(h->lds, chained.lds);
+      }
+    }
   }
   if (h->batches == BatchKernel::none) return 0;
   CellKernel<T> &batch = h->kernel<T>(mfgpu_handle::kBatch);
@@ -419,8 +450,10 @@
 template <typename T>
 int launch_pass2_group(mfgpu_handle *h, size_t group, void *dst, const void *src, hipStream_t st, int add) {
   if (h->p2_shared && group == 1)
-    HIP_TRY(reduce_owner_batches_launch<T>((T *)dst, (const T *)src, h->d_halo.as<const T>(), h->d_p2rec.get(),
-                                           h->d_p2tab.get(), (uint32_t)(h->plan.batch_cell_off.size() - 1),
+    HIP_TRY(reduce_owner_batches_launch<T>((T *)dst, (const T *)src, h->d_halo.as<const T>(),
+                                           (h->cells_chained ? h->d_ch_p2rec : h->d_p2rec).get(),
+                                           (h->cells_chained ? h->d_ch_p2tab : h->d_p2tab).get(),
+                                           (uint32_t)(h->plan.batch_cell_off.size() - 1),
                                            (uint32_t)p_hs(h->plan.n) * 64u, h->p2_reverse ? 1 : 0, add, st));
   HIP_TRY(reduce_classes_launch<T>((T *)dst, (const T *)src, h->d_halo.as<const T>(), h->d_p2arr[group].get(),
                                    h->d_p2tiles[group].get(), h->n_p2tiles[group], add, st));
@@ -443,6 +476,16 @@
 int launch_cells(mfgpu_handle *h, ApplyArgs<T> a, uint32_t b0, uint32_t b1, hipStream_t st) {
   const Plan &P = h->plan;
   const uint32_t npl = P.n_plane_batches, nplain = P.n_plain_plane_batches;
+  h->cells_chained = h->carry && h->p2_shared && b0 == 0 && b1 == P.batch_cell_off.size() - 1 && a.hole_len == 0 &&
+                     grid_of<T>(h, mfgpu_handle::kChained, b1) == h->chain_grid;
+  if (h->cells_chained) {
+    a.bdofsp = h->d_ch_dofs.get();
+    a.idxp = h->d_ch_idx.get();
+    a.shtab = h->d_ch_tab.get();
+    a.batch0 = 0;
+    a.batch_end = b1;
+    return launch_bound<T>(h, mfgpu_handle::kChained, a, b1, st);
+  }
   if (b0 < nplain) {
     a.batch0 = b0;
     a.batch_end = b1 < nplain ? b1 : nplain;
@@ -656,6 +699,7 @@
     return rc ? rc : handle_cells_range(h, c0, c1, dst, src, stream, add);
   }
   hipStream_t st = (hipStream_t)stream;
+  h->cells_chained = false;
   auto run = [&](auto a) -> int {
     a.batch0 = b0;
     a.batch_end = c1;
@@ -812,6 +856,15 @@
   return 0;
 }
 
+int mfgpu_carry_stats(const mfgpu_handle *h, uint64_t s[4]) {
+  if (!h || !s) return MFGPU_EINVAL;
+  s[0] = h->carry && h->p2_shared ? 1 : 0;
+  s[1] = h->carry ? h->chain_run : 0;
+  s[2] = h->carry ? h->chain_links : 0;
+  s[3] = h->carry ? h->chain_carried : 0;
+  return 0;
+}
+
 const char *mfgpu_kernel_name(const mfgpu_handle *h) {
   if (!h) return "";
   const bool x = h->batches == BatchKernel::x;
diff --git a/dealii-cuda_amd/csrc/mfgpu_internal.h b/dealii-cuda_amd/csrc/mfgpu_internal.h
--- a/dealii-cuda_amd/csrc/mfgpu_internal.h
+++ b/dealii-cuda_amd/csrc/mfgpu_internal.h
@@ -96,10 +96,11 @@
 int choose_kernel_and_plan(const mfgpu_desc &d, PlaneKernel &pk, BatchKernel &bk, Plan &plan);
 
 constexpr bool planes4_wide(int n) { return n >= 6; }
-constexpr bool kernel_exists(PlaneKernel k, int n, int number_type, bool hn, bool sh, bool mass) {
+constexpr bool kernel_exists(PlaneKernel k, int n, int number_type, bool hn, bool sh, bool mass, bool ch = false) {
   switch (k) {
-    case PlaneKernel::planes3: return n >= 3 && n <= 5 && !(sh && hn);
+    case PlaneKernel::planes3: return n >= 3 && n <= 5 && !(sh && hn) && (!ch || (n == 5 && sh && !hn && !mass));
     case PlaneKernel::planes4:
+      if (ch) return false;
       return planes4_wide(n) ? n <= 7 && !hn && !sh && !mass
                              : n >= 3 && !sh && !(mass && n == 5 && number_type == MFGPU_F64);
     default: return false;
@@ -114,6 +115,15 @@
 void share_plane_records(Plan &plan);
 constexpr int kP2Header = 16, kP2MaxK = 12, kP2SlotBits = 12;
 void share_pass2_records(Plan &plan);
+
+struct Chain {
+  uint32_t grid = 0, run = 0;
+  std::vector<uint32_t> order, links, eligible;
+  std::vector<uint32_t> dofs, idx, tab, p2rec, p2tab;
+  uint64_t carried = 0;
+};
+constexpr int kChainRun = 6;
+int build_chain(const Plan &plan, uint32_t G, uint32_t run, Chain &chain);
 
 int derive_tables(int n, const double *shape_values, const double *shape_gradients,
                   std::vector<double> &S, std::vector<double> &Dt);
@@ -133,6 +143,7 @@
 
 struct mfgpu_plan {
   mfgpu::Plan plan;
+  mfgpu::Chain chain;
 };
 
 #endif
diff --git a/dealii-cuda_amd/csrc/mfgpu_kernels.h b/dealii-cuda_amd/csrc/mfgpu_kernels.h
--- a/dealii-cuda_amd/csrc/mfgpu_kernels.h
+++ b/dealii-cuda_amd/csrc/mfgpu_kernels.h
@@ -122,6 +122,8 @@
 MFGPU_CELL_LOOP_FAMILY(p)
 MFGPU_CELL_LOOP_FAMILY(q)
 #undef MFGPU_CELL_LOOP_FAMILY
+template <typename T>
+hipError_t p_bind_chained(int n, bool mass, CellKernel<T> *k);
 
 void build_pass2_classes(const std::vector<uint32_t> &sdofs, const std::vector<uint32_t> &s_off,
                          const std::vector<uint32_t> &s_idx, std::vector<uint32_t> &arr, std::vector<uint32_t> &tiles);
diff --git a/dealii-cuda_amd/csrc/mfgpu_kernels_p.hip b/dealii-cuda_amd/csrc/mfgpu_kernels_p.hip
--- a/dealii-cuda_amd/csrc/mfgpu_kernels_p.hip
+++ b/dealii-cuda_amd/csrc/mfgpu_kernels_p.hip
@@ -8,14 +8,14 @@
 
 #define MFGPU_PIN_VMEM() __builtin_amdgcn_sched_barrier(0x380)
 
-template <int n, typename T, bool ADD, bool HN, bool SH = false, bool MASS = false>
+template <int n, typename T, bool ADD, bool HN, bool SH = false, bool MASS = false, bool CH = false>
 __global__ void __launch_bounds__(64) __attribute__((amdgpu_waves_per_eu(1, 1)))
 apply_planes3(const ApplyArgs<T> A, const TablesEO<T, n> tab) {
   constexpr int n2 = n * n;
   constexpr int CW = p_cells_per_wave(n);
   constexpr int NT = CW * n;
-  constexpr int KGU = p_kgu(n);
-  constexpr int JI = p_ji(n);
+  constexpr int KGU = p_kgu(n) + (CH ? 1 : 0);
+  constexpr int JI = p_ji(n) + (CH ? 1 : 0);
   constexpr int HS = KGU - JI;
   constexpr int SA = p_cell_stride(n);
   constexpr int NIW = (n2 + 1) / 2;
@@ -58,7 +58,7 @@
     return l < bend ? (l >= hole0 ? l + hole_len : l) : x;
   };
   if (b >= hole0) b += hole_len;
-  static_assert(kernel_exists(PlaneKernel::planes3, n, number_type_of<T>, HN, SH, MASS), "no such instantiation");
+  static_assert(kernel_exists(PlaneKernel::planes3, n, number_type_of<T>, HN, SH, MASS, CH), "no such instantiation");
   struct Meta {
     uint32_t base, drec, irec;
   };
@@ -69,6 +69,8 @@
     return Meta{(uint32_t)__builtin_amdgcn_readlane((int)v, 0), (uint32_t)__builtin_amdgcn_readlane((int)v, 1),
                 (uint32_t)__builtin_amdgcn_readlane((int)v, 2)};
   };
+  auto word3_of = [&](uint32_t v) -> uint32_t { return CH ? (uint32_t)__builtin_amdgcn_readlane((int)v, 3) : 0u; };
+  auto batch_at = [&](uint32_t word3, uint32_t pos) -> uint32_t { return CH ? word3 & 0xffffffu : pos; };
 
   auto load_dofs = [&](uint32_t rec, uint32_t (&g)[KGU]) {
     const uint32_t *p = A.bdofsp + (size_t)rec * (KGU * 64) + lane;
@@ -132,12 +134,19 @@
   T SVn[KGU], R[KGU], old[KGU];
   Meta Mp{0u, 0u, 0u}, Mc = Mp, M1 = Mp, M2 = Mp;
   uint32_t Mv = 0u;
+  uint32_t Wp = 0u, Wc = 0u, W1 = 0u, W2 = 0u;
   if (SH) {
     Mc = meta_of(meta_request(b));
     M1 = meta_of(meta_request(b1));
     M2 = meta_of(meta_request(b2));
     Mp = Mc;
   }
+  if (CH) {
+    Wc = word3_of(meta_request(b));
+    W1 = word3_of(meta_request(b1));
+    W2 = word3_of(meta_request(b2));
+    Wp = Wc;
+  }
   load_dofs(SH ? Mc.drec : b, Gc);
   load_dofs(SH ? M1.drec : b1, Gn);
   load_ix(SH ? Mc.irec : b, IXc);
@@ -146,12 +155,12 @@
 #pragma unroll
   for (int w = 0; w < NIW; ++w) IXc[w] = lane_on ? IXc[w] : kDummyIx;
   {
-    const T *p = A.coefp + (size_t)b * (n2 * NT) + tk;
+    const T *p = A.coefp + (size_t)batch_at(Wc, b) * (n2 * NT) + tk;
 #pragma unroll
     for (int r = 0; r < n2; ++r) Cc[r] = nt_load(p + r * NT);
   }
   if (MASS) {
-    const T *p = A.massp + (size_t)b * (n2 * NT) + tk;
+    const T *p = A.massp + (size_t)batch_at(Wc, b) * (n2 * NT) + tk;
 #pragma unroll
     for (int r = 0; r < n2; ++r) Mm[r] = nt_load(p + r * NT);
   }
@@ -239,14 +248,14 @@
       MFGPU_PIN_VMEM();
 #pragma unroll
       for (int j = (KGU * s) / (5 * n); j < (KGU * (s + 1)) / (5 * n); ++j)
-        scatter_slot(j, bp, Mp.base, Gp[j], R[j], old[j]);
+        scatter_slot(j, batch_at(Wp, bp), Mp.base, Gp[j], R[j], old[j]);
 #pragma unroll
       for (int j = (KGU * s) / (5 * n); j < (KGU * (s + 1)) / (5 * n); ++j)
         SVn[j] = src_at(M1.base, Gn[j]);
       MFGPU_PIN_VMEM();
     };
-    const T *const cnext = A.coefp + (size_t)b1 * (n2 * NT) + tk;
-    const T *const mnext = MASS ? A.massp + (size_t)b1 * (n2 * NT) + tk : nullptr;
+    const T *const cnext = A.coefp + (size_t)batch_at(W1, b1) * (n2 * NT) + tk;
+    const T *const mnext = MASS ? A.massp + (size_t)batch_at(W1, b1) * (n2 * NT) + tk : nullptr;
     auto hookC = [&](int s) {
       MFGPU_PIN_VMEM();
 #pragma unroll
@@ -425,14 +434,18 @@
         if ((uint32_t)(r * 64 + lane) < hn_ncopy) lds_add(ua + (Hc[r] & 0xffffu), cv[r]);
       WaveSync::sync();
     }
+    const T carry = R[KGU - 1];
 #pragma unroll
     for (int j = 0; j < KGU; ++j) R[j] = (T)ua[lane + j * 64];
+    if (CH)
+      R[JI - 1] = (uint32_t)lane < (Wc >> 24) ? carry + R[JI - 1] : R[JI - 1];
     WaveSync::sync();
     STAMP(5);
     stage_src(Gn, SVn);
     STAMP(6);
     bp = b;
     if (SH) Mp = Mc;
+    if (CH) Wp = Wc;
 #pragma unroll
     for (int j = 0; j < KGU; ++j) Gp[j] = Gc[j];
     STAMP(7);
@@ -447,6 +460,11 @@
       M1 = M2;
       M2 = meta_of(Mv);
     }
+    if (CH) {
+      Wc = W1;
+      W1 = W2;
+      W2 = word3_of(Mv);
+    }
 #pragma unroll
     for (int j = 0; j < KGU; ++j) {
       Gc[j] = Gn[j];
@@ -464,28 +482,39 @@
     for (int j = 0; j < JI; ++j) old[j] = *dst_at(Mp.base, Gp[j]);
   }
 #pragma unroll
-  for (int j = 0; j < KGU; ++j) scatter_slot(j, bp, Mp.base, Gp[j], R[j], old[j]);
+  for (int j = 0; j < KGU; ++j) scatter_slot(j, batch_at(Wp, bp), Mp.base, Gp[j], R[j], old[j]);
 }
 
 template <int n, typename T>
-static size_t p_lds_bytes(bool hn) {
-  return ((size_t)p_kgu(n) * 64 + (hn ? (size_t)p_priv_max(n) + n * n : 0)) * sizeof(double) +
+static size_t p_lds_bytes(bool hn, bool ch) {
+  return ((size_t)(p_kgu(n) + (ch ? 1 : 0)) * 64 + (hn ? (size_t)p_priv_max(n) + n * n : 0)) * sizeof(double) +
          (size_t)2 * (p_cells_per_wave(n) + 1) * p_cell_stride(n) * sizeof(T);
 }
 
+template <typename T>
+static hipError_t p_bind_switches(int n, bool hn, bool sh, bool mass, bool ch, CellKernel<T> *k) {
+  return dispatch_instantiation(n, [&](auto N, auto HN, auto SH, auto MASS, auto CH) {
+    constexpr int n_ = N;
+    if constexpr (kernel_exists(PlaneKernel::planes3, n_, number_type_of<T>, HN, SH, MASS, CH))
+      return bind_cell_kernel<T, 64, apply_planes3<n_, T, false, HN, SH, MASS, CH>,
+                              apply_planes3<n_, T, true, HN, SH, MASS, CH>, make_tables_eo<T, n_>>(
+          p_lds_bytes<n_, T>(HN, CH), k);
+    else
+      return hipErrorInvalidValue;
+  }, hn, sh, mass, ch);
+}
 template <typename T>
 hipError_t p_bind(int, int n, bool hn, bool, bool sh, bool mass, uint32_t, CellKernel<T> *k) {
-  return dispatch_instantiation(n, [&](auto N, auto HN, auto SH, auto MASS) {
-    constexpr int n_ = N;
-    if constexpr (kernel_exists(PlaneKernel::planes3, n_, number_type_of<T>, HN, SH, MASS))
-      return bind_cell_kernel<T, 64, apply_planes3<n_, T, false, HN, SH, MASS>, apply_planes3<n_, T, true, HN, SH, MASS>,
-                              make_tables_eo<T, n_>>(p_lds_bytes<n_, T>(HN), k);
-    else
-      return hipErrorInvalidValue;
-  }, hn, sh, mass);
+  return p_bind_switches<T>(n, hn, sh, mass, false, k);
+}
+template <typename T>
+hipError_t p_bind_chained(int n, bool mass, CellKernel<T> *k) {
+  return p_bind_switches<T>(n, false, true, mass, true, k);
 }
 template hipError_t p_bind<double>(int, int, bool, bool, bool, bool, uint32_t, CellKernel<double> *);
 template hipError_t p_bind<float>(int, int, bool, bool, bool, bool, uint32_t, CellKernel<float> *);
+template hipError_t p_bind_chained<double>(int, bool, CellKernel<double> *);
+template hipError_t p_bind_chained<float>(int, bool, CellKernel<float> *);
 
 template <typename T>
 __global__ void relayout_coef_kernel(T *out, const T *in, const uint32_t *cell_batch, const uint32_t *cell_pos,
diff --git a/dealii-cuda_amd/csrc/mfgpu_plan.cpp b/dealii-cuda_amd/csrc/mfgpu_plan.cpp
--- a/dealii-cuda_amd/csrc/mfgpu_plan.cpp
+++ b/dealii-cuda_amd/csrc/mfgpu_plan.cpp
@@ -745,35 +745,37 @@
   P.sh_use = nbat > 0 && P.pr_hn.empty() && (double)shared <= kShareMaxFraction * (double)expanded;
 }
 
-void share_pass2_records(Plan &P) {
-  P.sh_p2rec.clear();
-  P.sh_p2tab.clear();
-  P.sh_p2_use = false;
+namespace {
+bool owner_batch_records(const Plan &P, const std::vector<uint32_t> &sdofs, const std::vector<uint32_t> &s_off,
+                         const std::vector<uint32_t> &s_idx, std::vector<uint32_t> &p2rec, std::vector<uint32_t> &p2tab,
+                         size_t &expanded) {
+  p2rec.clear();
+  p2tab.clear();
   const size_t nb = P.batch_cell_off.size() - 1;
   const uint32_t hs = (uint32_t)p_hs(P.n) * 64u;
-  if (nb == 0 || P.n_plane_batches != nb || P.halo_off.size() != nb + 1 || hs > (1u << kP2SlotBits)) return;
+  if (nb == 0 || P.n_plane_batches != nb || P.halo_off.size() != nb + 1 || hs > (1u << kP2SlotBits)) return false;
   for (size_t b = 0; b <= nb; ++b)
-    if (P.halo_off[b] != (uint64_t)b * hs) return;
+    if (P.halo_off[b] != (uint64_t)b * hs) return false;
   std::vector<std::vector<uint32_t>> owned(nb);
-  size_t expanded = 0;
-  for (size_t i = 0; i < P.sdofs.size(); ++i) {
-    const uint32_t k = P.s_off[i + 1] - P.s_off[i];
+  expanded = 0;
+  for (size_t i = 0; i < sdofs.size(); ++i) {
+    const uint32_t k = s_off[i + 1] - s_off[i];
     expanded += 1 + (k ? k : 1);
     if (k == 0) continue;
-    if (k > (uint32_t)kP2MaxK) return;
-    const uint32_t owner = P.s_idx[P.s_off[i]] / hs;
+    if (k > (uint32_t)kP2MaxK) return false;
+    const uint32_t owner = s_idx[s_off[i]] / hs;
     for (uint32_t t = 0; t < k; ++t) {
-      const uint32_t tb = P.s_idx[P.s_off[i] + t] / hs;
-      if (tb >= nb || tb < owner || tb - owner >= (1u << (32 - kP2SlotBits))) return;
+      const uint32_t tb = s_idx[s_off[i] + t] / hs;
+      if (tb >= nb || tb < owner || tb - owner >= (1u << (32 - kP2SlotBits))) return false;
     }
     owned[owner].push_back((uint32_t)i);
   }
-  P.sh_p2tab.assign(2 * nb, 0u);
+  p2tab.assign(2 * nb, 0u);
   std::unordered_multimap<uint64_t, std::pair<uint32_t, uint32_t>> seen;
   std::vector<uint32_t> rec;
   for (size_t b = 0; b < nb; ++b) {
     std::vector<uint32_t> &m = owned[b];
-    auto k_of = [&](uint32_t i) { return P.s_off[i + 1] - P.s_off[i]; };
+    auto k_of = [&](uint32_t i) { return s_off[i + 1] - s_off[i]; };
     std::stable_sort(m.begin(), m.end(), [&](uint32_t x, uint32_t y) { return k_of(x) > k_of(y); });
     const uint32_t base = P.sh_batch[b * kShBatchWords], ne = (uint32_t)m.size(), kmax = ne ? k_of(m[0]) : 0u;
     auto pad = [](uint32_t x) { return (x + 63u) & ~63u; };
@@ -783,7 +785,7 @@
     rec[1] = e0;
     rec[2] = kmax;
     rec.resize(kP2Header + 2 * (size_t)e0, 0u);
-    for (uint32_t e = 0; e < e0; ++e) rec[kP2Header + e] = e < ne ? P.sdofs[m[e]] - base : 0xffffffffu;
+    for (uint32_t e = 0; e < e0; ++e) rec[kP2Header + e] = e < ne ? sdofs[m[e]] - base : 0xffffffffu;
     for (uint32_t e = 0; e < ne; ++e) rec[kP2Header + e0 + e] = k_of(m[e]);
     for (uint32_t t = 0; t < kmax; ++t) {
       uint32_t cnt = 0;
@@ -791,7 +793,7 @@
       rec[3 + t] = (uint32_t)rec.size();
       rec.resize(rec.size() + pad(cnt), 0u);
       for (uint32_t e = 0; e < cnt; ++e) {
-        const uint32_t slot = P.s_idx[P.s_off[m[e]] + t], tb = slot / hs;
+        const uint32_t slot = s_idx[s_off[m[e]] + t], tb = slot / hs;
         rec[rec[3 + t] + e] = ((tb - (uint32_t)b) << kP2SlotBits) | (slot - tb * hs);
       }
     }
@@ -800,18 +802,171 @@
     const auto range = seen.equal_range(h);
     for (auto it = range.first; it != range.second && off == 0xffffffffu; ++it)
       if (it->second.second == rec.size() &&
-          !std::memcmp(P.sh_p2rec.data() + it->second.first, rec.data(), rec.size() * sizeof(uint32_t)))
+          !std::memcmp(p2rec.data() + it->second.first, rec.data(), rec.size() * sizeof(uint32_t)))
         off = it->second.first;
     if (off == 0xffffffffu) {
-      off = (uint32_t)P.sh_p2rec.size();
-      P.sh_p2rec.insert(P.sh_p2rec.end(), rec.begin(), rec.end());
+      off = (uint32_t)p2rec.size();
+      p2rec.insert(p2rec.end(), rec.begin(), rec.end());
       seen.emplace(h, std::make_pair(off, (uint32_t)rec.size()));
     }
-    P.sh_p2tab[2 * b] = base;
-    P.sh_p2tab[2 * b + 1] = off;
+    p2tab[2 * b] = base;
+    p2tab[2 * b + 1] = off;
+  }
+  return true;
+}
+}
+
+void share_pass2_records(Plan &P) {
+  size_t expanded = 0;
+  P.sh_p2_use = false;
+  if (!owner_batch_records(P, P.sdofs, P.s_off, P.s_idx, P.sh_p2rec, P.sh_p2tab, expanded)) {
+    P.sh_p2rec.clear();
+    P.sh_p2tab.clear();
+    return;
   }
   const size_t shared = P.sh_p2rec.size() + P.sh_p2tab.size();
   P.sh_p2_use = (double)shared <= kShareMaxFraction * (double)expanded;
+}
+
+int build_chain(const Plan &P, uint32_t G, uint32_t L, Chain &C) {
+  C = Chain();
+  const int n = P.n, NT = p_cells_per_wave(n) * n, NIW = (n * n + 1) / 2;
+  const uint32_t JI = (uint32_t)p_ji(n) * 64u, NB = (uint32_t)p_kgu(n) * 64u, HSL = (uint32_t)p_hs(n) * 64u;
+  const uint32_t JIC = JI + 64u, NBC = NB + 64u;
+  const uint32_t nb = P.n_plane_batches, NONE = 0xffffffffu;
+  if (!P.pr_hn.empty() || nb == 0 || nb != P.batch_cell_off.size() - 1 || P.sh_p2tab.size() != 2 * (size_t)nb ||
+      P.pr_idx.size() != (size_t)NIW * NT * nb || nb >= (1u << 24) || G == 0 || L == 0) {
+    set_error("the plan has no chained form (it needs plain plane batches only and owner-batch records of pass 2)");
+    return MFGPU_EUNSUPPORTED;
+  }
+  C.grid = G;
+  C.run = L;
+  std::vector<std::vector<uint32_t>> F(nb);
+  for (size_t i = 0; i < P.sdofs.size(); ++i) {
+    if (P.s_off[i + 1] - P.s_off[i] != 2 || (P.sdofs[i] >> 31)) continue;
+    const uint32_t b0 = P.s_idx[P.s_off[i]] / HSL, b1 = P.s_idx[P.s_off[i] + 1] / HSL;
+    if (b1 == b0 + 1) F[b0].push_back(P.sdofs[i]);
+  }
+  for (auto &f : F) std::sort(f.begin(), f.end());
+  auto n_pass2 = [&](uint32_t b) { return P.batch_dof_off[b + 1] - P.batch_dof_off[b] - P.batch_nint[b]; };
+  auto n_link = [&](uint32_t b) { return b < nb ? (uint32_t)F[b].size() : 0u; };
+  std::vector<uint8_t> eligible(nb, 0);
+  for (uint32_t b = 0; b + 1 < nb; ++b) {
+    const uint32_t f = n_link(b);
+    eligible[b] = f >= 1 && f <= 63 && n_pass2(b) - f <= HSL - 64u && n_pass2(b) > f + n_link(b - 1) &&
+                  n_pass2(b + 1) > f + n_link(b + 1);
+    if (eligible[b]) C.eligible.push_back(b);
+  }
+  C.order.resize(nb);
+  std::iota(C.order.begin(), C.order.end(), 0u);
+  struct Range {
+    uint32_t lo, hi, w;
+  };
+  std::vector<Range> ranges;
+  if (G >= 8 && nb >= G) {
+    const uint32_t q = G >> 3, rem = G & 7u;
+    for (uint32_t xcd = 0; xcd < 8; ++xcd) {
+      const uint32_t wlo = xcd * q + std::min(xcd, rem), w = q + (xcd < rem ? 1u : 0u);
+      ranges.push_back({(uint32_t)((uint64_t)nb * wlo / G), (uint32_t)((uint64_t)nb * (wlo + w) / G), w});
+    }
+  } else {
+    ranges.push_back({0u, nb, G});
+  }
+  std::vector<uint32_t> pos_of(nb), stride_of(nb);
+  for (const Range &r : ranges) {
+    uint32_t pos = r.lo;
+    while (r.hi - pos >= 2 * r.w) {
+      const uint32_t Lr = std::min(L, (r.hi - pos) / r.w);
+      for (uint32_t s2 = 0; s2 < r.w; ++s2)
+        for (uint32_t j = 0; j < Lr; ++j) C.order[pos + s2 + j * r.w] = pos + s2 * Lr + j;
+      pos += r.w * Lr;
+    }
+    for (uint32_t p2 = r.lo; p2 < r.hi; ++p2) {
+      pos_of[C.order[p2]] = p2;
+      stride_of[C.order[p2]] = r.w;
+    }
+  }
+  std::vector<uint8_t> kept(nb, 0);
+  std::vector<uint32_t> lane_of(P.n_dofs, NONE), link_of(P.n_dofs, NONE);
+  for (uint32_t b : C.eligible) {
+    if (pos_of[b + 1] != pos_of[b] + stride_of[b] || stride_of[b + 1] != stride_of[b]) continue;
+    bool same_range = false;
+    for (const Range &r : ranges) same_range = same_range || (pos_of[b] >= r.lo && pos_of[b + 1] < r.hi);
+    if (!same_range) continue;
+    kept[b] = 1;
+    C.links.push_back(b);
+    C.carried += F[b].size();
+    for (size_t l = 0; l < F[b].size(); ++l) {
+      lane_of[F[b][l]] = (uint32_t)l;
+      link_of[F[b][l]] = b;
+    }
+  }
+  std::vector<uint32_t> new_slot((size_t)nb * HSL, NONE);
+  std::unordered_multimap<uint64_t, uint32_t> seen_d, seen_x;
+  std::vector<uint32_t> list(NBC), map(NB), runs((size_t)NIW * NT), drec(nb), irec(nb), base_of(nb);
+  for (uint32_t b = 0; b < nb; ++b) {
+    const uint32_t d0 = P.batch_dof_off[b], ni = P.batch_nint[b], nps = n_pass2(b);
+    const bool out = kept[b], in = b > 0 && kept[b - 1];
+    for (uint32_t t = 0; t < NB; ++t) map[t] = t;
+    map[NB - 1] = NBC - 1;
+    uint32_t pad = NONE, ord = 0;
+    for (uint32_t q = 0; q < nps; ++q) {
+      const uint32_t e = P.bdofs[d0 + ni + q], g = e & 0x7fffffffu;
+      uint32_t slot;
+      if (link_of[g] == NONE) {
+        slot = JIC + ord++;
+        new_slot[(size_t)b * HSL + q] = slot - JIC;
+        if (pad == NONE) pad = e;
+      } else {
+        slot = (link_of[g] == b ? NBC - 64u : JI) + lane_of[g];
+        if (link_of[g] == b) new_slot[(size_t)b * HSL + q] = slot - JIC;
+      }
+      map[JI + q] = slot;
+      list[slot] = e;
+    }
+    if (pad == NONE || ord > (out ? HSL - 64u : HSL - 1u)) {
+      set_error("internal: chained record does not fit");
+      return MFGPU_EINVAL;
+    }
+    for (uint32_t t = 0; t < JI; ++t) list[t] = t < ni ? P.bdofs[d0 + t] : pad;
+    for (uint32_t l = in ? n_link(b - 1) : 0u; l < 64u; ++l) list[JI + l] = pad;
+    for (uint32_t t = JIC + ord; t < NBC; ++t)
+      if (!(out && t >= NBC - 64u && t < NBC - 64u + n_link(b))) list[t] = pad;
+    uint32_t base = 0x7fffffffu;
+    for (uint32_t t = 0; t < NBC; ++t) base = std::min(base, list[t] & 0x7fffffffu);
+    for (uint32_t t = 0; t < NBC; ++t) list[t] -= base;
+    const uint32_t *ix = P.pr_idx.data() + (size_t)b * NIW * NT;
+    for (size_t w = 0; w < runs.size(); ++w)
+      runs[w] = 8u * map[(ix[w] & 0xffffu) / 8u] | (8u * map[(ix[w] >> 16) / 8u]) << 16;
+    base_of[b] = base;
+    drec[b] = intern_record(C.dofs, seen_d, list.data(), NBC);
+    irec[b] = intern_record(C.idx, seen_x, runs.data(), runs.size());
+  }
+  C.tab.resize((size_t)nb * kShBatchWords);
+  for (uint32_t p2 = 0; p2 < nb; ++p2) {
+    const uint32_t b = C.order[p2];
+    uint32_t *e = C.tab.data() + (size_t)p2 * kShBatchWords;
+    e[0] = base_of[b];
+    e[1] = drec[b];
+    e[2] = irec[b];
+    e[3] = b | (b > 0 && kept[b - 1] ? n_link(b - 1) : 0u) << 24;
+  }
+  std::vector<uint32_t> sd, so(1, 0u), si;
+  for (size_t i = 0; i < P.sdofs.size(); ++i) {
+    if (link_of[P.sdofs[i] & 0x7fffffffu] != NONE) continue;
+    sd.push_back(P.sdofs[i]);
+    for (uint32_t t = P.s_off[i]; t < P.s_off[i + 1]; ++t) {
+      const uint32_t tb = P.s_idx[t] / HSL;
+      si.push_back(tb * HSL + new_slot[P.s_idx[t]]);
+    }
+    so.push_back((uint32_t)si.size());
+  }
+  size_t expanded = 0;
+  if (!owner_batch_records(P, sd, so, si, C.p2rec, C.p2tab, expanded)) {
+    set_error("internal: chained pass-2 records");
+    return MFGPU_EINVAL;
+  }
+  return 0;
 }
 
 int choose_kernel_and_plan(const mfgpu_desc &d, PlaneKernel &pk, BatchKernel &bk, Plan &plan) {
@@ -969,10 +1124,23 @@
     case 19: v = &p->plan.sh_batch; break;
     case 20: v = &p->plan.sh_p2rec; break;
     case 21: v = &p->plan.sh_p2tab; break;
+    case 22: v = &p->chain.order; break;
+    case 23: v = &p->chain.links; break;
+    case 24: v = &p->chain.dofs; break;
+    case 25: v = &p->chain.idx; break;
+    case 26: v = &p->chain.tab; break;
+    case 27: v = &p->chain.p2rec; break;
+    case 28: v = &p->chain.p2tab; break;
+    case 29: v = &p->chain.eligible; break;
     default: mfgpu::set_error("bad array id"); return MFGPU_EINVAL;
   }
   *ptr = v->data();
   return (int64_t)v->size();
+}
+
+int mfgpu_plan_chain(mfgpu_plan *p, uint32_t grid, uint32_t run_length) {
+  if (!p) return MFGPU_EINVAL;
+  return mfgpu::build_chain(p->plan, grid, run_length ? run_length : (uint32_t)mfgpu::kChainRun, p->chain);
 }
 
 int mfgpu_plan_shares_records(const mfgpu_plan *p) {
diff --git a/dealii-cuda_amd/pymfgpu/__init__.py b/dealii-cuda_amd/pymfgpu/__init__.py
--- a/dealii-cuda_amd/pymfgpu/__init__.py
+++ b/dealii-cuda_amd/pymfgpu/__init__.py
@@ -10,7 +10,7 @@
 
 F64, F32 = 0, 1
 OK, EINVAL = 0, -1
-UNIFORM_J0, HANGING_NODES, COLORED_SCATTER, NO_SHARED_RECORDS = 1, 2, 1 << 8, 1 << 9
+UNIFORM_J0, HANGING_NODES, COLORED_SCATTER, NO_SHARED_RECORDS, NO_CARRY = 1, 2, 1 << 8, 1 << 9, 1 << 10
 KERNEL_AUTO, KERNEL_PENCILS, KERNEL_PENCILS_X, KERNEL_PLANES, KERNEL_PLANES_2W = 0, 1, 2, 3, 4
 
 
@@ -38,7 +38,7 @@
     "mfgpu_vec_sadd", "mfgpu_vec_equ", "mfgpu_vec_scale", "mfgpu_vec_divide", "mfgpu_vec_invert", "mfgpu_vec_mul",
     "mfgpu_vec_dot", "mfgpu_vec_l2_norm", "mfgpu_vec_add_and_dot", "mfgpu_vec_all_zero", "mfgpu_profile_enable", "mfgpu_profile_read", "mfgpu_profile_read_pass2",
     "mfgpu_plan_create", "mfgpu_plan_destroy", "mfgpu_plan_array_u32", "mfgpu_plan_lmap", "mfgpu_plan_bflags",
-    "mfgpu_plan_shares_records", "mfgpu_record_stats",
+    "mfgpu_plan_shares_records", "mfgpu_record_stats", "mfgpu_carry_stats", "mfgpu_plan_chain",
     "mfgpu_vec_alloc", "mfgpu_vec_free", "mfgpu_vec_fill", "mfgpu_vec_from_host", "mfgpu_vec_to_host",
     "mfgpu_device_synchronize", "mfgpu_device_memory_info", "mfgpu_mesh_create_uniform", "mfgpu_mesh_create_adaptive", "mfgpu_mesh_create_ball", "mfgpu_mesh_create_from_leaves",
     "mfgpu_mesh_cell_levels", "mfgpu_mesh_destroy",
@@ -111,6 +111,9 @@
         L.mfgpu_plan_bflags.restype = C.c_int64
         L.mfgpu_plan_shares_records.argtypes = [C.c_void_p]
         L.mfgpu_record_stats.argtypes = [C.c_void_p, C.POINTER(C.c_uint64)]
+        if hasattr(L, "mfgpu_carry_stats"):
+            L.mfgpu_carry_stats.argtypes = [C.c_void_p, C.POINTER(C.c_uint64)]
+            L.mfgpu_plan_chain.argtypes = [C.c_void_p, C.c_uint32, C.c_uint32]
         L.mfgpu_vec_alloc.argtypes = [C.POINTER(C.c_void_p), C.c_size_t, C.c_int]
         L.mfgpu_vec_free.argtypes = [C.c_void_p]
         L.mfgpu_vec_fill.argtypes = [C.c_void_p, C.c_size_t, C.c_int, C.c_double, C.c_void_p]
@@ -410,6 +413,12 @@
     sh_p2tab = property(lambda s: s._u32(21).reshape(-1, 2))
     shares_pass2_records = property(lambda s: bool(lib().mfgpu_plan_shares_records(s._h) & 2))
 
+    def chain(self, grid, run_length=0):
+        _check(lib().mfgpu_plan_chain(self._h, grid, run_length))
+        return dict(order=self._u32(22), links=self._u32(23), dofs=self._u32(24), idx=self._u32(25),
+                    tab=self._u32(26).reshape(-1, 4), p2rec=self._u32(27), p2tab=self._u32(28).reshape(-1, 2),
+                    eligible=self._u32(29))
+
     @property
     def lmap(self):
         p = C.c_void_p()
@@ -543,6 +552,11 @@
         out.update(index_records="shared" if r[0] & 1 else "expanded",
                    pass2_records="shared" if r[0] & 2 else "expanded", distinct_dof_records=int(r[1]),
                    distinct_index_records=int(r[2]), index_record_bytes=int(r[3]))
+        c = (C.c_uint64 * 4)()
+        if hasattr(lib(), "mfgpu_carry_stats"):
+            _check(lib().mfgpu_carry_stats(self._h, c))
+        out.update(carry="on" if c[0] else "off", carry_run_length=int(c[1]), carry_kept_links=int(c[2]),
+                   carried_dofs=int(c[3]))
         return out
 
     def kernel_name(self):
diff --git a/include/mfgpu.h b/include/mfgpu.h
--- a/include/mfgpu.h
+++ b/include/mfgpu.h
@@ -23,6 +23,8 @@
 #define MFGPU_COLORED_SCATTER (1u << 8)
 
 #define MFGPU_NO_SHARED_RECORDS (1u << 9)
+
+#define MFGPU_NO_CARRY (1u << 10)
 
 typedef struct mfgpu_handle mfgpu_handle;
 
@@ -79,6 +81,8 @@
 
 int mfgpu_record_stats(const mfgpu_handle *h, uint64_t stats[4]);
 
+int mfgpu_carry_stats(const mfgpu_handle *h, uint64_t stats[4]);
+
 const char *mfgpu_kernel_name(const mfgpu_handle *h);
 
 int mfgpu_profile_enable(mfgpu_handle *h, int on);
@@ -90,6 +94,7 @@
 void mfgpu_plan_destroy(mfgpu_plan *p);
 int64_t mfgpu_plan_array_u32(const mfgpu_plan *p, int what, const uint32_t **ptr);
 int mfgpu_plan_shares_records(const mfgpu_plan *p);
+int mfgpu_plan_chain(mfgpu_plan *p, uint32_t grid, uint32_t run_length);
 int64_t mfgpu_plan_lmap(const mfgpu_plan *p, const uint16_t **ptr);
 int64_t mfgpu_plan_bflags(const mfgpu_plan *p, const uint8_t **ptr);
 
```
